# bark-simulator/planner-miqp

Measured on AMD Instinct MI355X. Metric: MIQP solves/sec to 1% gap, 2-agent x 20-step x 32-region, higher is better.
Workload: dtype f64

## Files before the change

### include/miqp_gpu.h

```cpp
#ifndef MIQP_GPU_H
#define MIQP_GPU_H

#include "miqp_types.h"

#ifdef __cplusplus
extern "C" {
#endif

typedef struct miqp_solver miqp_solver_t;

typedef struct miqp_solver_opts {
  int precision;
  int device;
  int nodes_per_round;
  int max_open_nodes;
  double gap_override;
  int verbose;
} miqp_solver_opts;

miqp_solver_t* miqp_solver_create(const miqp_solver_opts* opts);
void miqp_solver_destroy(miqp_solver_t* s);

int miqp_solver_set_params(miqp_solver_t* s, const miqp_model_params_c* p);

int miqp_solver_load_dat(miqp_solver_t* s, const char* path);

int miqp_solver_override_settings(miqp_solver_t* s, double max_solution_time, double relative_mip_gap_tolerance);

int miqp_solver_set_warmstart(miqp_solver_t* s, const miqp_raw_results_c* start, int warmstart_type);

int miqp_solver_solve(miqp_solver_t* s, double timestamp);

int miqp_solver_solve_batch(miqp_solver_t* const* solvers, int n, int* statuses);

int miqp_solver_solve_stream(miqp_solver_t* const* solvers, int n, int inflight, int* statuses);

int miqp_solver_solve_batch_multi(miqp_solver_t* const* solvers, int n, int gpus, int* statuses);

typedef int (*miqp_exchange_fn)(void* user, int op, void* buf, int count, int root);
int miqp_solver_solve_split(miqp_solver_t* s, double timestamp, int world, int rank, miqp_exchange_fn exchange, void* user);

int miqp_comm_unique_id(char* out128);
int miqp_comm_init(int world, int rank, const char* id128, int device);
int miqp_comm_finalize(void);
int miqp_solver_solve_split_rccl(miqp_solver_t* s, double timestamp);
int miqp_comm_selftest(miqp_exchange_fn exchange, void* user, int world, int rank);

int miqp_solver_split_roots(const miqp_solver_t* s, int world, int rank, int* root_of_pair, int* index, int* value, int cap, int* nroots_out, int* ncombos_out);

int miqp_solver_raw_sizes(const miqp_solver_t* s, int* out4);
int miqp_solver_lift_tables(const miqp_solver_t* s, double* out, int cap);

int miqp_solver_get_results(const miqp_solver_t* s, miqp_raw_results_c* out);

int miqp_solver_materialize_results(miqp_solver_t* const* solvers, int n, int threads);

int miqp_solver_get_properties(const miqp_solver_t* s, miqp_solution_properties_c* out);

int miqp_solver_get_dims(const miqp_solver_t* s, int* out6);

int miqp_solver_export_lp(const miqp_solver_t* s, const char* path);

int miqp_solver_write_dat(const miqp_solver_t* s, const char* path);

int miqp_solver_write_solution(const miqp_solver_t* s, const char* path);

int miqp_solver_write_mst(const miqp_solver_t* s, const char* path);

int miqp_solver_read_mst(miqp_solver_t* s, const char* path);

int miqp_solver_solve_fixed(miqp_solver_t* s, const miqp_raw_results_c* fixed, miqp_raw_results_c* out,
                            double* objective, int* iterations);

int miqp_solver_last_timing(const miqp_solver_t* s, double* out6);

int miqp_solver_last_active_set(const miqp_solver_t* s, double* out8);

int miqp_solver_last_fixed_route(const miqp_solver_t* s);

int miqp_solver_solve_fixed_batch(miqp_solver_t* s, const miqp_raw_results_c* const* fixed, int n, miqp_fixed_result_c* out, int* best);

int miqp_solver_fixed_batch_record(miqp_solver_t* s, int k, miqp_raw_results_c* out);

int miqp_gpu_fixed_result_size(void);
int miqp_gpu_fixed_batch_chunk(void);

int miqp_solver_set_pool(miqp_solver_t* s, int capacity);
int miqp_solver_pool_count(const miqp_solver_t* s);
int miqp_solver_pool_found(const miqp_solver_t* s, double* obj, int cap);
int miqp_solver_pool_solve(miqp_solver_t* s, miqp_fixed_result_c* out, int cap);
int miqp_solver_pool_record(miqp_solver_t* s, int k, miqp_raw_results_c* out);
int miqp_gpu_pool_max(void);

int miqp_solver_set_pool_filter(miqp_solver_t* s, int families);
int miqp_gpu_pool_signature(int cars, int steps, int obstacles, int families, const signed char* decisions, signed char* out, int len);
int miqp_solver_pool_signature(const miqp_solver_t* s, const miqp_raw_results_c* rec, int families, signed char* out, int cap);
int miqp_solver_pool_found_decisions(const miqp_solver_t* s, int k, signed char* out, int cap);

int miqp_solver_solve_fixed_multi(miqp_solver_t* const* solvers, int n, const miqp_raw_results_c* const* fixed, const int* first, miqp_fixed_result_c* out, int* best);
int miqp_solver_pool_solve_multi(miqp_solver_t* const* solvers, int n, miqp_fixed_result_c* out, int cap, int* counts);

int miqp_gpu_has_active_set(int num_cars, int num_steps);

int miqp_solver_launch_plan(const miqp_solver_t* s, int bc, int overlap, int par, const int* cls_n3, int cus, double free_gb, int flags, int* out, int cap);

int miqp_solver_last_setup(const miqp_solver_t* s, double* out3);

int miqp_solver_last_admission(const miqp_solver_t* s, double* out1);

const char* miqp_solver_last_error(const miqp_solver_t* s);


int miqp_fraction_parameters(int nr_regions, float max_velocity_fitting, double* out);
int miqp_fitting_polynomial_parameters(int nr_regions, float max_velocity_fitting, float min_velocity_fitting, double* out);
int miqp_mean_angles(const double* fraction_parameters, int nr_regions, double* out);
int miqp_limits_per_region(const double* fraction_parameters, int nr_regions, float long_min, float long_max, float lat_min, float lat_max,
                           double* min_x, double* max_x, double* min_y, double* max_y);
int miqp_calculate_region_idx(const double* fraction_parameters, int nr_regions, float vx, float vy, int* out);
int miqp_reserve_neighbor_regions(int* row, int nr_regions, int expansions);
int miqp_calculate_possible_regions(const double* fraction_parameters, int nr_regions, const double* theta_ref, int n, int* flags);
int miqp_reference_trajectory(const double* ref_xy, int n_ref, const double* state5, double dt, int num_points, double line_interp_inc, double vel_desired,
                              double delta_s_desired, double acc_lat_max, int vel_curve_dep, double* out);
int miqp_update_car(const double* settings12, const double* fraction_parameters, const double* initial_state6, const double* ref_xy, int n_ref, double desired_velocity,
                    double delta_s_desired, double timestep, int track_reference_positions, int is_ego, int num_cars, double* ref4N, int* possible_region, double* weights8);
int miqp_calculate_warmstart(const miqp_raw_results_c* last, miqp_raw_results_c* out, double ts, double minimum_region_change_speed);
int miqp_plan(miqp_solver_t* s, miqp_model_params_c* p, int* initial_region, int* possible_region, const miqp_raw_results_c* warmstart,
              int warmstart_type, double timestamp, int* status_out);

int miqp_initial_pose_check(const miqp_model_params_c* p);
int miqp_select_environment(const double* pieces_xy, const int* piece_off, int n_pieces, const double* traj_xy, const int* traj_off, int n_traj, int* selected);
int miqp_obstacle_intersects_environment(const double* pieces_xy, const int* piece_off, int n_pieces, const double* obstacle_xy, int n_steps, int is_static);
int miqp_bark_trajectory(const miqp_raw_results_c* results, int car, double start_time, double ts, double min_speed, double* out_rows5);
int miqp_obstacles_roi(double x, double y, double theta, double behind_distance, double front_distance, double side_distance, double* roi_xy);
int miqp_obstacle_intersects_environment_roi(const double* pieces_xy, const int* piece_off, int n_pieces, const double* obstacle_xy, int n_steps, int is_static, const double* roi_xy);
int miqp_environment_warmstart(const miqp_raw_results_c* last, miqp_raw_results_c* out, const int* ids_old, int n_old, const int* ids_new, int n_new);

int miqp_solver_certify(miqp_solver_t* s, const miqp_raw_results_c* candidate, miqp_certificate_c* out);
int miqp_solver_certify_batch(miqp_solver_t* const* solvers, int n, miqp_certificate_c* out);
int miqp_gpu_certificate_size(void);
int miqp_gpu_certify_last_timing(double* out4);

const char* miqp_gpu_version(void);

#ifdef __cplusplus
}
#endif
#endif
```

### planner_miqp_amd/csrc/as_onchip.hip

```cpp
namespace miqp {

#ifdef MIQP_PROFILE
#define ASP_T(var) const long long var = clock64()
#define ASP_ACC(k, t0, t1) asp_[k] += (unsigned long long)((t1) - (t0))
#else
#define ASP_T(var)
#define ASP_ACC(k, t0, t1)
#endif
constexpr int AS_MAXSTEP = 220;
constexpr double AS_VTOL = 1.0e-8;
constexpr double AS_DEP = 1.0e-8;
constexpr int AS_MT = 64;
constexpr int AS_MSTR = AS_MT * (AS_MT + 1) / 2;

__host__ __device__ constexpr bool as_shape_ok(int C, int N) { return (C == 1 || C == 2) && N >= 1 && N <= 2 * OC_NSL; }

template <int C> __device__ inline int as_col(int pq) { return C == 2 ? ((pq & 3) << 2) | (pq >> 2) : ((pq & 1) << 2) | (pq >> 1); }
template <int C> __device__ inline int as_pcol(int q) { return C == 2 ? ((q & 3) << 2) | (q >> 2) : ((q & 3) << 1) | (q >> 2); }
template <int C> struct AsDecode {
  static constexpr bool LANE_BOUNDS = true, ROW_IDENTITY = true, MARKS = true;
  static __device__ int col(int l) { return as_col<C>(oc_pcol<C, true>(l)); }
};

template <int C, int NSL, int GCAP = miqp::OC_GCAP>
__global__ void __launch_bounds__(64, (GCAP > 128 ? 1 : 2)) as_onchip_kernel(DevBuf B) {
  static_assert(C == 1 || C == 2, "a stage of 16 columns holds the chains of up to two cars");
  constexpr bool CM = true;
  constexpr bool BIG = GCAP > 128;
  constexpr int OC_GCAP = GCAP, OC_GSLOTS = OC_GCAP / 64, OC_GCOEF = oc_gcoef_of(OC_GCAP);
  constexpr int NX = 6 * C, NZ = 8 * C, NCH = 2 * C;
  const Layout& Y = B.Y;
  const int tid = threadIdx.x, lg = tid >> 4, lc = tid & 15;
  const int par = lg >> 1, side = lg & 1;
  const double bsgn = side ? -1.0 : 1.0;
  WAVE_DUMP(BIG ? 1 : 4);
  const int* const clist = BIG && B.cls_take ? B.cls_list + (size_t)(B.cls_take - 1) * B.batch_cap : nullptr;
  const int nbatch = clist ? (B.cls_count[B.cls_take - 1] < B.batch_cap ? B.cls_count[B.cls_take - 1] : B.batch_cap) : (*B.batch_count < B.batch_cap ? *B.batch_count : B.batch_cap);
  const int N = Y.N, NSLOT = Y.NSLOT;
  extern __shared__ double lds[];
  char* const L0 = (char*)lds;
  const OcLds LL = oc_lds_layout(N, Y.fixlen, OC_GCAP, !BIG);
  double* const Z = (double*)(L0 + LL.z);
  double* const scr = (double*)(L0 + LL.u);
  double* const V = (double*)(L0 + LL.u);
  unsigned long long* const bkey = (unsigned long long*)(L0 + LL.r);
  const int SPAN = LL.gmeta - LL.u;
  double* const kref = (double*)(L0 + LL.u + SPAN - N * 32);
  double* const kff = kref - N * 4;
  double* const KS = kff - N * 16;
  const int STG_CAP = (SPAN - N * 192) / 8;
  uint4* const gmeta = (uint4*)(L0 + LL.gmeta);
  double* const gcoef = (double*)(L0 + LL.gcoef);
  double* const grhs = (double*)(L0 + LL.grhs);
  double* const Wd = (double*)(L0 + LL.wd);
  int* const sstart = (int*)(L0 + LL.sstart);
  unsigned short* const cand = (unsigned short*)(L0 + LL.cand);
  signed char* const fix = (signed char*)(L0 + LL.fix);
  __shared__ int sh_node;
  __shared__ unsigned long long sh_stat[32];
  if (tid < 32) sh_stat[tid] = 0ull;
  const unsigned long long lt = (1ull << tid) - 1ull;

  const int chunk = B.as_chunk > 0 ? B.as_chunk : 1;
  int run_next = 0, run_end = 0;
  const int quota = BIG ? 0 : B.as_quota; int handed = 0;
#ifdef MIQP_PROFILE
  const unsigned long long wv_c0 = __builtin_amdgcn_s_memtime(), wv_r0 = __builtin_amdgcn_s_memrealtime();
  unsigned long long wv_first = 0; int wv_nodes = 0;
  if (!BIG && tid == 0) wv_first = atomicMin(&B.prof[120], wv_r0);
#endif
  for (;;) {
    __syncthreads();
    if (run_next >= run_end) {
      if (quota > 0 && handed >= quota) break;
      ++handed;
      if (tid == 0) sh_node = atomicAdd(B.work_counter, chunk);
      __syncthreads();
      run_next = __builtin_amdgcn_readfirstlane(sh_node); run_end = run_next + chunk;
      if (run_next >= nbatch) break;
    }
    const int slot_ = run_next++;
    if (slot_ >= nbatch) { run_next = run_end; continue; }
    const int node = clist ? __builtin_amdgcn_readfirstlane(clist[slot_]) : slot_;
    {
      const int cls = B.batch_large ? (int)B.batch_large[node] : (is_probe_word(B.batch_depth[node]) ? 1 : 0);
      if (cls != (BIG ? 1 : 0)) continue;
    }
    WAVE_DUMP_NODE();
    const int inst = __builtin_amdgcn_readfirstlane(B.batch_inst[node]);
    const double* D = B.inst_d + (size_t)inst * Y.dstride;
    const int* T = B.inst_i + (size_t)inst * Y.istride;
    const double ts = D[Y.d_glob + 7];
    const double aqs = 2.0 * D[Y.d_misc + 0];
    const double iaq = aqs > 0.0 ? 1.0 / aqs : 0.0;
    {
      const signed char* src = B.pool_fix + (size_t)B.batch_node[node] * Y.fixlen;
      for (int k = tid; k < Y.fixlen; k += 64) fix[k] = src[k];
      if (tid < 16) Wd[tid] = tid < NZ ? D[Y.d_wd + oc_lcol<C, CM>(as_pcol<C>(tid))] : 0.0;
      for (int k = tid; k < N * 32; k += 64) bkey[k] = ~0ull;
      for (int k = tid; k <= N + 1; k += 64) sstart[k] = 0;
    }
    __syncthreads();
    const double* Rf = D + Y.d_ref;
    double cutoff = 1e300;
    {
      const double inc0 = fmin(inc_from_key(*(volatile unsigned long long*)&B.inc_key[inst]), B.inc_ext[inst]);
      const double gap_ = is_probe_word(B.batch_depth[node]) ? 0.0 : B.inst_gap[inst];
      if (B.use_cutoff && inc0 < 1e300) cutoff = inc0 - gap_ * (1e-10 + fabs(inc0)) - B.inst_const[inst];
    }

#ifdef MIQP_PROFILE
    unsigned long long asp_[12] = {0, 0, 0, 0, 0, 0, 0, 0, 0, 0, 0, 0};
#endif
    ASP_T(ta0);
#define OC_DECODE_POLICY AsDecode<C>
#include "oc_decode_body.inc"
#undef OC_DECODE_POLICY
    if (overflow) {
      if (B.batch_A) B.batch_A[(size_t)node * 64 + tid] = 0xFFFFu;
      if (tid == 0) {
        if (B.ring_M) B.batch_Mtag[node] = 0ull;
        B.batch_ok[node] = 5; B.pool_big[B.batch_node[node]] |= (BIG ? 2 : 1); if (B.stats) { atomicAdd(&B.stats[3], 1ull); atomicAdd(&B.stats[8 + (ngen >= 512 ? 15 : ngen / 32)], 1ull); }
      }
      continue;
    }
    const int NM = sstart[N + 1];
    OC_WAVE_SYNC();

    ASP_T(ta1); ASP_ACC(0, ta0, ta1);
#ifdef MIQP_PROFILE
    asp_[9] += (unsigned long long)(ocd_t_sparse - ta0); asp_[11] += (unsigned long long)(ta1 - ocd_t_rows);
#endif
    double brhs[NSL];
    unsigned int bact = 0u, binA = 0u, ginA = 0u;
#pragma unroll
    for (int k = 0; k < NSL; ++k) {
      const int i = 2 * k + par;
      brhs[k] = 1e300;
      if (i < N && lc < NZ) {
        const unsigned long long key = bkey[(i * 2 + side) * 16 + lc];
        if (key != ~0ull) { brhs[k] = key2d(key); bact |= 1u << k; }
      }
    }
    OC_WAVE_SYNC();

    const double h1 = ts, h2 = 0.5 * ts * ts, h3 = ts * ts * ts / 6.0;
    const double* const tb = D + Y.d_astab;
    if constexpr (C == 2) {
      for (int k = tid; k < N * 16; k += 64) KS[k] = tb[k];
      for (int k = tid; k < N * 4; k += 64) kref[k] = tb[N * 16 + k];
    } else {
      for (int k = tid; k < N * 8; k += 64) KS[(k >> 3) * 16 + (k & 7)] = tb[k];
      for (int k = tid; k < N * 2; k += 64) kref[(k >> 1) * 4 + (k & 1)] = tb[N * 8 + k];
    }
    OC_WAVE_SYNC();
    typedef double d2_t __attribute__((ext_vector_type(2)));
    auto subst = [&](const bool fromx0, const int itop, const int iend, double* const out) {
      for (int k = tid; k < (N - 1) * 4; k += 64) if ((k >> 2) > itop) kff[k] = fromx0 ? kref[k] : 0.0;
      if (tid < NCH) {
        const int ch = tid;
        double p0 = 0.0, p1 = 0.0, p2 = 0.0;
        int i0 = itop;
        if (itop >= N - 1) { const d2_t a = *(const d2_t*)(V + (N - 1) * 16 + 4 * ch); p0 = a[0]; p1 = a[1]; p2 = V[(N - 1) * 16 + 4 * ch + 2]; i0 = N - 2; }
        if (i0 >= 0) {
          d2_t va = *(const d2_t*)(V + i0 * 16 + 4 * ch), vb = *(const d2_t*)(V + i0 * 16 + 4 * ch + 2);
          d2_t ka = *(const d2_t*)(KS + (i0 * 4 + ch) * 4), kb = *(const d2_t*)(KS + (i0 * 4 + ch) * 4 + 2);
          double kr = fromx0 ? kref[i0 * 4 + ch] : 0.0;
          for (int i = i0; i >= 0; --i) {
            const int j = i > 0 ? i - 1 : 0;
            const d2_t nva = *(const d2_t*)(V + j * 16 + 4 * ch), nvb = *(const d2_t*)(V + j * 16 + 4 * ch + 2);
            const d2_t nka = *(const d2_t*)(KS + (j * 4 + ch) * 4), nkb = *(const d2_t*)(KS + (j * 4 + ch) * 4 + 2);
            const double nkr = fromx0 ? kref[j * 4 + ch] : 0.0;
            const double su = vb[1] + h3 * p0 + h2 * p1 + h1 * p2;
            const double sx0 = va[0] + p0, sx1 = va[1] + h1 * p0 + p1, sx2 = vb[0] + h2 * p0 + h1 * p1 + p2;
            kff[i * 4 + ch] = fma(su, kb[1], kr);
            p0 = sx0 - ka[0] * su; p1 = sx1 - ka[1] * su; p2 = sx2 - kb[0] * su;
            va = nva; vb = nvb; ka = nka; kb = nkb; kr = nkr;
          }
        }
      }
      OC_WAVE_SYNC();
      if (tid < NCH) {
        const int ch = tid;
        double x0 = 0.0, x1 = 0.0, x2 = 0.0;
        if (fromx0) { const int c = ch >> 1, s = ch & 1; x0 = D[Y.d_x0 + 6 * c + 3 * s]; x1 = D[Y.d_x0 + 6 * c + 3 * s + 1]; x2 = D[Y.d_x0 + 6 * c + 3 * s + 2]; }
        const int ie = iend < N - 1 ? iend : N - 2;
        d2_t ka = *(const d2_t*)(KS + ch * 4), kb = *(const d2_t*)(KS + ch * 4 + 2);
        double kf = kff[ch];
        for (int i = 0; i <= ie; ++i) {
          const int j = i < N - 2 ? i + 1 : N - 2;
          const d2_t nka = *(const d2_t*)(KS + (j * 4 + ch) * 4), nkb = *(const d2_t*)(KS + (j * 4 + ch) * 4 + 2);
          const double nkf = kff[j * 4 + ch];
          const double u = -kf - (ka[0] * x0 + ka[1] * x1 + kb[0] * x2);
          d2_t oa, ob; oa[0] = x0; oa[1] = x1; ob[0] = x2; ob[1] = u;
          *(d2_t*)(out + i * 16 + 4 * ch) = oa; *(d2_t*)(out + i * 16 + 4 * ch + 2) = ob;
          const double n0 = x0 + h1 * x1 + h2 * x2 + h3 * u, n1 = x1 + h1 * x2 + h2 * u, n2 = x2 + h1 * u;
          x0 = n0; x1 = n1; x2 = n2;
          ka = nka; kb = nkb; kf = nkf;
        }
        if (iend >= N - 1 || ie == N - 2) { d2_t oa, ob; oa[0] = x0; oa[1] = x1; ob[0] = x2; ob[1] = 0.0; *(d2_t*)(out + (ie + 1) * 16 + 4 * ch) = oa; *(d2_t*)(out + (ie + 1) * 16 + 4 * ch + 2) = ob; }
      }
      OC_WAVE_SYNC();
    };
    auto row_dot = [&](int id, const double* vec) -> double {
      if (id < 1024) return (((id >> 4) & 1) ? -1.0 : 1.0) * vec[(id >> 5) * 16 + (id & 15)];
      const uint4 m4 = gmeta[id - 1024];
      const int off = (int)(m4.z & 0xFFFFu), nn = (int)((m4.z >> 16) & 7u), i = (int)((m4.z >> 20) & 0x7FFu);
      double a = 0.0;
#pragma unroll
      for (int k = 0; k < 6; ++k) if (k < nn) a += gcoef[off + k] * vec[i * 16 + ((m4.w >> (4 * k)) & 15u)];
      return a;
    };
    auto row_soft = [&](int id) -> bool { return id >= 1024 && (gmeta[id - 1024].z & 0x80000000u) != 0u; };
    auto zeroV = [&]() { for (int k = tid; k < N * 16; k += 64) V[k] = 0.0; OC_WAVE_SYNC(); };
    auto objective = [&]() -> double {
      double o = 0.0;
      for (int k = tid; k < N * 16; k += 64) { const int q = k & 15; if (q < NZ) { const double d = Z[k] - Rf[(k >> 4) * NZ + oc_lcol<C, CM>(as_pcol<C>(q))]; o += Wd[q] * d * d; } }
      return wave_sum(o);
    };

    int arow = -1, astage = -1; double alam = 0.0, arhs = 0.0;
    double M[64];
#pragma unroll
    for (int b = 0; b < 64; ++b) M[b] = 0.0;
    unsigned long long used = 0ull;
    auto rank1 = [&](const double u, const double alpha, const unsigned long long mask) {
#pragma unroll
      for (int g8 = 0; g8 < 8; ++g8) {
        if ((mask >> (8 * g8)) & 0xFFull) {
#pragma unroll
          for (int j = 0; j < 8; ++j) { const int b = 8 * g8 + j; M[b] = fma(u * readlane_d(u, b), alpha, M[b]); }
        }
      }
    };
    auto refresh = [&]() {
      zeroV();
      const double FX = 274877906944.0, IFX = 1.0 / 274877906944.0;
      if (arow >= 0 && alam != 0.0) {
        if (arow < 1024) atomicAdd((unsigned long long*)&V[(arow >> 5) * 16 + (arow & 15)], (unsigned long long)(long long)__double2ll_rn((((arow >> 4) & 1) ? -alam : alam) * FX));
        else {
          const uint4 m4 = gmeta[arow - 1024];
          const int off = (int)(m4.z & 0xFFFFu), nn = (int)((m4.z >> 16) & 7u), i = (int)((m4.z >> 20) & 0x7FFu);
#pragma unroll
          for (int k = 0; k < 6; ++k) if (k < nn) atomicAdd((unsigned long long*)&V[i * 16 + ((m4.w >> (4 * k)) & 15u)], (unsigned long long)(long long)__double2ll_rn(gcoef[off + k] * alam * FX));
        }
      }
      OC_WAVE_SYNC();
      for (int k = tid; k < N * 16; k += 64) V[k] = (double)(long long)__double_as_longlong(V[k]) * IFX;
      const int amax = (int)wave_max((double)astage);
      OC_WAVE_SYNC();
      subst(true, amax, N - 1, Z);
    };
    if constexpr (C == 2) { for (int k = tid; k < N * 16; k += 64) Z[k] = tb[N * 20 + k]; }
    else { for (int k = tid; k < N * 16; k += 64) Z[k] = (k & 15) < NZ ? tb[N * 10 + (k >> 4) * NZ + (k & 15)] : 0.0; }
    OC_WAVE_SYNC();
    ASP_T(ta2); ASP_ACC(1, ta1, ta2);
    int steps = 0, ndrop = 0, ok = 1, nwarm = 0, nfast = 0, ncold = 0;
    bool infeas = false, fail = false;
    int why = 0;
    if (B.pool_A && (B.batch_depth[node] >> 6) >= 1 && B.batch_node[node] < B.z_cap) {
      const int rec = B.batch_node[node];
      const unsigned int pa = B.pool_A[(size_t)rec * 64 + tid];
      int cid = -1;
      int ownl = 0;
      if (pa < 1024u) ownl = (int)((((pa >> 5) & 1u) * 2u + ((pa >> 4) & 1u)) << 4 | (pa & 15u));
      const unsigned int ob = (unsigned int)__shfl((int)bact, ownl);
      if (pa < 1024u) { if ((ob >> (pa >> 6)) & 1u) cid = (int)pa; }
      else if (pa != 0xFFFFu) {
        const int pc = (int)pa - 1024;
        int lo = 0, hi = NM;
        while (lo < hi) { const int mid = (lo + hi) >> 1; if ((int)cand[mid] < pc) lo = mid + 1; else hi = mid; }
        if (lo < NM && (int)cand[lo] == pc) cid = 1024 + lo;
      }
      const unsigned long long u0p = __ballot(pa != 0xFFFFu);
      const unsigned long long u0 = __ballot(cid >= 0);
      if (u0) {
        arow = cid;
        astage = cid < 0 ? -1 : (cid < 1024 ? (cid >> 5) : (int)((gmeta[cid - 1024].z >> 20) & 0x7FFu));
        int nmp = 0; unsigned long long moff = 0ull;
        if (B.ring_M) {
          const unsigned long long tg = B.pool_Mtag[rec];
          const unsigned long long c_ = tg >> 8;
          if (tg != 0ull && *(volatile unsigned long long*)B.ring_head - c_ < B.ring_doubles - B.ring_margin) { nmp = (int)(tg & 255ull); moff = c_ % B.ring_doubles; }
        }
        nmp = __builtin_amdgcn_readfirstlane(nmp);
        if (B.as_stats && tid == 0 && !(nmp > 0 && nmp == __popcll(u0p))) sh_stat[16 + (B.ring_M == nullptr ? 0 : (B.pool_Mtag[rec] == 0ull ? 1 : (nmp == 0 ? 2 : 3)))] += 1ull;
        if (nmp > 0 && nmp == __popcll(u0p)) {
          const double* const rm = B.ring_M; const unsigned long long rd_ = B.ring_doubles;
          const int ra = __popcll(u0p & lt);
          const bool mine = (u0p >> tid) & 1ull;
          const int len = nmp * (nmp + 1) / 2;
          for (int c0 = 0; c0 < len; c0 += STG_CAP) {
            const int c1 = c0 + STG_CAP < len ? c0 + STG_CAP : len;
            OC_WAVE_SYNC();
            for (int k = c0 + tid; k < c1; k += 64) { unsigned long long q_ = moff + (unsigned long long)k; if (q_ >= rd_) q_ -= rd_; V[k - c0] = rm[q_]; }
            OC_WAVE_SYNC();
#pragma unroll
            for (int b8 = 0; b8 < 64; ++b8) {
              if ((u0p >> b8) & 1ull) {
                const int rb = __popcll(u0p & ((1ull << b8) - 1ull));
                const int hi_ = ra > rb ? ra : rb, lo_ = ra > rb ? rb : ra;
                const int ix = hi_ * (hi_ + 1) / 2 + lo_;
                if (mine && ix >= c0 && ix < c1) M[b8] = V[ix - c0];
              }
            }
          }
          OC_WAVE_SYNC();
          used = u0p;
          for (unsigned long long um = u0p & ~u0; um; um &= um - 1ull) {
            const int kd = __builtin_amdgcn_readfirstlane(__ffsll((long long)um) - 1);
            double m = 0.0;
#pragma unroll
            for (int b = 0; b < 64; ++b) m = (b == kd) ? M[b] : m;
            const double mkk = readlane_d(m, kd);
            if (mkk > 0.0) rank1(m, -1.0 / mkk, used);
#pragma unroll
            for (int b = 0; b < 64; ++b) if (b == kd || tid == kd) M[b] = 0.0;
            used &= ~(1ull << kd);
          }
          nfast = 1;
        } else {
          used = u0;
          const int amax0 = (int)wave_max((double)astage);
          double sdiag = 1.0;
          for (unsigned long long um = u0; um; um &= um - 1ull) {
            const int a = __builtin_amdgcn_readfirstlane(__ffsll((long long)um) - 1);
            const int ida = __builtin_amdgcn_readlane(arow, a);
            zeroV();
            if (ida < 1024) { if (tid == 0) V[(ida >> 5) * 16 + (ida & 15)] = ((ida >> 4) & 1) ? -1.0 : 1.0; }
            else {
              const uint4 m4 = gmeta[ida - 1024];
              const int off = (int)(m4.z & 0xFFFFu), nn = (int)((m4.z >> 16) & 7u), i = (int)((m4.z >> 20) & 0x7FFu);
              if (tid < nn) V[i * 16 + ((m4.w >> (4 * tid)) & 15u)] = gcoef[off + tid];
            }
            const int sta = __builtin_amdgcn_readlane(astage, a);
            OC_WAVE_SYNC();
            subst(false, sta, amax0, V);
            double sv = arow >= 0 ? -row_dot(arow, V) : 0.0;
            if (tid == a && row_soft(ida)) sv += iaq;
            if (tid == a) sdiag = sv;
#pragma unroll
            for (int b = 0; b < 64; ++b) M[b] = (b == a) ? sv : M[b];
          }
          for (unsigned long long um = u0; um; um &= um - 1ull) {
            const int k = __builtin_amdgcn_readfirstlane(__ffsll((long long)um) - 1);
            double m = 0.0;
#pragma unroll
            for (int b = 0; b < 64; ++b) m = (b == k) ? M[b] : m;
            const double d = readlane_d(m, k);
            if (!(d > AS_DEP * readlane_d(sdiag, k))) {
#pragma unroll
              for (int b = 0; b < 64; ++b) if (b == k || tid == k) M[b] = 0.0;
              if (tid == k) { arow = -1; astage = -1; }
              used &= ~(1ull << k);
              continue;
            }
            const double invd = 1.0 / d;
#pragma unroll
            for (int g8 = 0; g8 < 8; ++g8) {
              if ((u0 >> (8 * g8)) & 0xFFull) {
#pragma unroll
                for (int j = 0; j < 8; ++j) { const int b = 8 * g8 + j; const double mb = readlane_d(m, b); M[b] = (tid == k) ? M[b] * invd : fma(m * mb, -invd, M[b]); }
              }
            }
#pragma unroll
            for (int b = 0; b < 64; ++b) M[b] = (b == k) ? ((tid == k) ? -invd : m * invd) : M[b];
          }
#pragma unroll
          for (int b = 0; b < 64; ++b) M[b] = (arow < 0) ? 0.0 : -M[b];
        }
        {
          int ol = 0, ok_ = -1;
          if (arow >= 0 && arow < 1024) { ol = (((arow >> 5) & 1) * 2 + ((arow >> 4) & 1)) << 4 | (arow & 15); ok_ = arow >> 6; }
          double rsel = arow >= 1024 ? grhs[arow - 1024] : 0.0;
#pragma unroll
          for (int k = 0; k < NSL; ++k) {
            const double rk = __shfl(brhs[k], ol);
            if (ok_ == k) rsel = rk;
          }
          arhs = rsel;
        }
        double cv = arow >= 0 ? row_dot(arow, Z) - arhs : 0.0;
        for (int guard = 0; guard < 64; ++guard) {
          double l0 = 0.0;
#pragma unroll
          for (int g8 = 0; g8 < 8; ++g8) {
            if ((used >> (8 * g8)) & 0xFFull) {
#pragma unroll
              for (int j = 0; j < 8; ++j) { const int b = 8 * g8 + j; l0 = fma(M[b], readlane_d(cv, b), l0); }
            }
          }
          if (arow < 0) l0 = 0.0;
          alam = l0;
          const double lmin = wave_min(arow >= 0 ? l0 : 1e300);
          if (!(lmin < -1e-10)) break;
          const int kd = __builtin_amdgcn_readfirstlane(__ffsll((long long)__ballot(arow >= 0 && l0 == lmin)) - 1);
          double m = 0.0;
#pragma unroll
          for (int b = 0; b < 64; ++b) m = (b == kd) ? M[b] : m;
          const double mkk = readlane_d(m, kd);
          if (!(mkk > 0.0)) { fail = true; break; }
          rank1(m, -1.0 / mkk, used);
#pragma unroll
          for (int b = 0; b < 64; ++b) if (b == kd || tid == kd) M[b] = 0.0;
          if (tid == kd) { arow = -1; astage = -1; alam = 0.0; cv = 0.0; }
          used &= ~(1ull << kd);
          ndrop++;
        }
        if (alam < 0.0) alam = 0.0;
        nwarm = __popcll(used);
        refresh();
        double resid = arow >= 0 ? fabs(row_dot(arow, Z) - arhs - ((arow >= 1024 && row_soft(arow)) ? alam * iaq : 0.0)) : 0.0;
        resid = wave_max(resid);
        if (!(resid <= 1e-7) || fail) {
          fail = false;
          arow = -1; astage = -1; alam = 0.0; arhs = 0.0; used = 0ull; nwarm = 0; nfast = 0; ncold = 1;
#pragma unroll
          for (int b = 0; b < 64; ++b) M[b] = 0.0;
          refresh();
        } else {
          unsigned int* const inab = C == 2 ? (unsigned int*)fix : (unsigned int*)V;
          inab[tid] = 0u;
          OC_WAVE_SYNC();
          if (arow >= 0) {
            if (arow < 1024) atomicOr(&inab[(((arow >> 5) & 1) * 2 + ((arow >> 4) & 1)) << 4 | (arow & 15)], 1u << (arow >> 6));
            else { const int rr_ = arow - 1024; atomicOr(&inab[rr_ & 63], 1u << (16 + (rr_ >> 6))); }
          }
          OC_WAVE_SYNC();
          { const unsigned int w_ = inab[tid]; binA = w_ & 0xFFFFu; ginA = w_ >> 16; }
        }
      }
    }
    ASP_T(ta3); ASP_ACC(8, ta2, ta3);
    double Dval = objective() + wave_sum((arow >= 1024 && row_soft(arow)) ? 0.5 * alam * alam * iaq : 0.0);

    for (; !fail;) {
      ASP_T(tb0);
      double bv = -1e300, brh = 0.0; int bid = -1;
#pragma unroll
      for (int k = 0; k < NSL; ++k) {
        const int i = 2 * k + par;
        if (((bact >> k) & 1u) && !((binA >> k) & 1u)) { const double v = bsgn * Z[i * 16 + lc] - brhs[k]; if (v > bv) { bv = v; brh = brhs[k]; bid = (i * 2 + side) * 16 + lc; } }
      }
#pragma unroll
      for (int q = 0; q < OC_GSLOTS; ++q) {
        const int r = q * 64 + tid;
        if (r < NM && !((ginA >> q) & 1u)) { const double rh_ = grhs[r]; const double v = row_dot(1024 + r, Z) - rh_; if (v > bv) { bv = v; brh = rh_; bid = 1024 + r; } }
      }
      const double vmax = wave_max(bv);
      if (!(vmax > AS_VTOL)) break;
      if (steps >= AS_MAXSTEP || used == ~0ull || !(vmax < 1e290)) { fail = true; why = used == ~0ull ? 1 : 2; break; }
      const int src = __builtin_amdgcn_readfirstlane(__ffsll((long long)__ballot(bv == vmax)) - 1);
      const int pid = __builtin_amdgcn_readlane(bid, src);
      const bool psoft = row_soft(pid);
      const double prhs = readlane_d(brh, src);
      ASP_T(tb1); ASP_ACC(2, tb0, tb1);
      zeroV();
      if (pid < 1024) { if (tid == 0) V[(pid >> 5) * 16 + (pid & 15)] = ((pid >> 4) & 1) ? -1.0 : 1.0; }
      else {
        const uint4 m4 = gmeta[pid - 1024];
        const int off = (int)(m4.z & 0xFFFFu), nn = (int)((m4.z >> 16) & 7u), i = (int)((m4.z >> 20) & 0x7FFu);
        if (tid < nn) V[i * 16 + ((m4.w >> (4 * tid)) & 15u)] = gcoef[off + tid];
      }
      const int pstage = pid < 1024 ? (pid >> 5) : (int)((gmeta[pid - 1024].z >> 20) & 0x7FFu);
      const int amax_ = (int)wave_max((double)astage);
      OC_WAVE_SYNC();
      subst(false, pstage, amax_ > pstage ? amax_ : pstage, V);
      ASP_T(tb2); ASP_ACC(3, tb1, tb2);
      double q = arow >= 0 ? -row_dot(arow, V) : 0.0;
      const double Spp = -row_dot(pid, V) + (psoft ? iaq : 0.0);
      double vp = vmax, lp = 0.0;
      steps++;
      ASP_T(tb3); ASP_ACC(4, tb2, tb3);
      for (;;) {
        double r = 0.0;
#pragma unroll
        for (int g8 = 0; g8 < 8; ++g8) {
          if ((used >> (8 * g8)) & 0xFFull) {
#pragma unroll
            for (int j = 0; j < 8; ++j) { const int b = 8 * g8 + j; r = fma(M[b], readlane_d(q, b), r); }
          }
        }
        if (arow < 0) r = 0.0;
        const double curv = Spp - wave_sum(q * r);
        const double ratio = (arow >= 0 && r > 1e-13) ? alam / r : 1e300;
        const double td = wave_min(ratio);
        const int kd = td < 1e299 ? __builtin_amdgcn_readfirstlane(__ffsll((long long)__ballot(ratio == td)) - 1) : -1;
        if (!(curv == curv) || !(Spp > 0.0)) { fail = true; why = 3; break; }
        const bool dep = !(curv > AS_DEP * Spp);
        double t; bool full;
        if (dep) { if (kd < 0) { infeas = true; break; } t = td; full = false; }
        else { const double tp = vp / curv; if (tp <= td) { t = tp; full = true; } else { t = td; full = false; } }
        if (arow >= 0) { alam = fma(-t, r, alam); if (alam < 0.0) alam = 0.0; }
        lp += t;
        Dval += t * (vp - 0.5 * t * (dep ? 0.0 : curv));
        if (lp > RHO_EL) { infeas = true; break; }
        if (full) {
          const int s = __builtin_amdgcn_readfirstlane(__ffsll((long long)~used) - 1);
          double u = arow >= 0 ? r : 0.0;
          if (tid == s) u = -1.0;
          const unsigned long long nmask = used | (1ull << s);
          rank1(u, 1.0 / curv, nmask);
          if (tid == s) { arow = pid; alam = lp; astage = pstage; arhs = prhs; }
          used = nmask;
          if (pid < 1024) { if (tid == ((((pid >> 5) & 1) * 2 + ((pid >> 4) & 1)) << 4 | (pid & 15))) binA |= 1u << (pid >> 6); }
          else { const int rr_ = pid - 1024; if (tid == (rr_ & 63)) ginA |= 1u << (rr_ >> 6); }
          break;
        }
        vp -= t * (dep ? 0.0 : curv);
        const int idk = __builtin_amdgcn_readlane(arow, kd);
        if (idk < 1024) { if (tid == ((((idk >> 5) & 1) * 2 + ((idk >> 4) & 1)) << 4 | (idk & 15))) binA &= ~(1u << (idk >> 6)); }
        else { const int rr_ = idk - 1024; if (tid == (rr_ & 63)) ginA &= ~(1u << (rr_ >> 6)); }
        double m = 0.0;
#pragma unroll
        for (int b = 0; b < 64; ++b) m = (b == kd) ? M[b] : m;
        const double mkk = readlane_d(m, kd);
        if (!(mkk > 0.0)) { fail = true; why = 4; break; }
        rank1(m, -1.0 / mkk, used);
#pragma unroll
        for (int b = 0; b < 64; ++b) if (b == kd || tid == kd) M[b] = 0.0;
        if (tid == kd) { arow = -1; astage = -1; alam = 0.0; q = 0.0; }
        used &= ~(1ull << kd);
        ndrop++; steps++;
        if (steps >= AS_MAXSTEP) { fail = true; why = 2; break; }
      }
      ASP_T(tb4); ASP_ACC(5, tb3, tb4);
      if (infeas || fail) break;
      refresh();
      ASP_T(tb5); ASP_ACC(6, tb4, tb5);
      if (Dval - 1e-9 * fabs(Dval) > cutoff + 1e-9 * fabs(cutoff)) { ok = 2; break; }
    }
    ASP_T(tc0);
    double viol = 0.0, scost = 0.0, lres = 0.0;
    if (!fail && !infeas && ok == 1) {
#pragma unroll
      for (int k = 0; k < NSL; ++k) { const int i = 2 * k + par; if ((bact >> k) & 1u) viol = fmax(viol, bsgn * Z[i * 16 + lc] - brhs[k]); }
#pragma unroll
      for (int q = 0; q < OC_GSLOTS; ++q) { const int r = q * 64 + tid; if (r < NM && !(gmeta[r].z & 0x80000000u)) viol = fmax(viol, row_dot(1024 + r, Z) - grhs[r]); }
      if (arow >= 0) {
        const bool sf = arow >= 1024 && row_soft(arow);
        const double res = row_dot(arow, Z) - arhs - (sf ? alam * iaq : 0.0);
        if (sf) { scost = 0.5 * alam * alam * iaq; viol = fmax(viol, res); }
        lres = alam * res;
      }
      viol = wave_max(viol); scost = wave_sum(scost);
      lres = fabs(wave_sum(lres));
    } else if (infeas) viol = 1.0;
    if (!fail && !infeas && ok == 1 && !(viol <= 5.0e-7)) { fail = true; why = 5; }
    if (BIG && infeas && B.as_probe_first && B.pump_max > 0 && is_probe_word(B.batch_depth[node]) && (cutoff > 1e299 || B.pump_inc)) fail = true;
    if (fail) {
      if (B.batch_A) B.batch_A[(size_t)node * 64 + tid] = 0xFFFFu;
      if (B.ring_M && tid == 0) B.batch_Mtag[node] = 0ull;
      if (tid == 0) { B.batch_ok[node] = 5; B.pool_big[B.batch_node[node]] |= 4; if (B.as_stats) { sh_stat[2] += 1ull; sh_stat[10 + (why < 6 ? why : 5)] += 1ull; } }
      continue;
    }
    const double obj = (infeas || ok == 2) ? Dval : objective() + scost;
    double* Zo = B.batch_Z + (size_t)node * N * NZ;
    for (int k = tid; k < N * 16; k += 64) { const int q = k & 15; if (q < NZ) Zo[(k >> 4) * NZ + oc_lcol<C, CM>(as_pcol<C>(q))] = Z[k]; }
    if (B.batch_A) {
      unsigned short enc = 0xFFFFu;
      if (!fail && !infeas && ok == 1 && arow >= 0) enc = arow < 1024 ? (unsigned short)arow : (unsigned short)(1024 + (int)cand[arow - 1024]);
      B.batch_A[(size_t)node * 64 + tid] = enc;
    }
    if (B.ring_M) {
      const int n_ = __popcll(used);
      unsigned long long tg_ = 0ull;
      OC_WAVE_SYNC();
      if (!fail && !infeas && ok == 1 && n_ >= 1 && n_ <= AS_MT && n_ * (n_ + 1) * 4 <= LL.total) {
        double* const stg = (double*)L0;
        const int ra = __popcll(used & lt);
#pragma unroll
        for (int b8 = 0; b8 < 64; ++b8) {
          if ((used >> b8) & 1ull) {
            const int rb = __popcll(used & ((1ull << b8) - 1ull));
            if (arow >= 0 && ra >= rb) stg[ra * (ra + 1) / 2 + rb] = M[b8];
          }
        }
        const int len = n_ * (n_ + 1) / 2;
        unsigned long long cnt_ = 0ull;
        if (tid == 0) cnt_ = atomicAdd(B.ring_head, (unsigned long long)len);
        cnt_ = ((unsigned long long)(unsigned int)__builtin_amdgcn_readfirstlane((int)(cnt_ >> 32)) << 32) | (unsigned int)__builtin_amdgcn_readfirstlane((int)cnt_);
        tg_ = (cnt_ << 8) | (unsigned long long)n_;
        OC_WAVE_SYNC();
        const unsigned long long o_ = cnt_ % B.ring_doubles, rd_ = B.ring_doubles;
        for (int k = tid; k < len; k += 64) { unsigned long long q_ = o_ + (unsigned long long)k; if (q_ >= rd_) q_ -= rd_; B.ring_M[q_] = stg[k]; }
      }
      if (tid == 0) B.batch_Mtag[node] = tg_;
    }
    if (tid == 0) {
      B.batch_obj[node] = obj; B.batch_viol[node] = viol; B.batch_ok[node] = ok;
      B.batch_bound[node] = lres + 1e-9 * (1.0 + fabs(obj));
      B.batch_it[node] = steps;
      atomicAdd((unsigned long long*)&B.inst_nodes[inst], 1ull);
      atomicAdd((unsigned long long*)&B.inst_iters[inst], (unsigned long long)steps);
#ifdef MIQP_PROFILE
      ++wv_nodes;
      { const long long tc1 = clock64(); asp_[7] += (unsigned long long)(tc1 - tc0);
        for (int q_ = 0; q_ < 9; ++q_) atomicAdd(&B.prof[80 + q_], asp_[q_]);
        atomicAdd(&B.prof[92], asp_[9]); atomicAdd(&B.prof[93], asp_[11]);
        atomicAdd(&B.prof[90], 1ull); atomicAdd(&B.prof[91], (unsigned long long)steps); }
#endif
      if (B.as_stats) {
        sh_stat[0] += 1ull; sh_stat[1] += (unsigned long long)steps; sh_stat[3] += (unsigned long long)ndrop;
        sh_stat[4] += infeas ? 1ull : 0ull; sh_stat[5] += ok == 2 ? 1ull : 0ull; sh_stat[6] += (unsigned long long)__popcll(used); sh_stat[7] += (unsigned long long)nwarm; sh_stat[8] += (unsigned long long)nfast; sh_stat[9] += (unsigned long long)ncold;
        if (BIG) { const int og_ = B.pool_origin ? (int)B.pool_origin[B.batch_node[node]] : 0; sh_stat[20] += 1ull; sh_stat[21] += (unsigned long long)steps; if (og_ == 14) { sh_stat[22] += 1ull; sh_stat[23] += (unsigned long long)steps; }
          sh_stat[24 + (ngen <= 64 ? 0 : ngen <= 96 ? 1 : ngen <= 128 ? 2 : ngen <= 192 ? 3 : 4)] += 1ull; if (is_probe_word(B.batch_depth[node]) && og_ != 14) sh_stat[29] += 1ull; }
      }
    }
  }
  __syncthreads();
  if (B.as_stats && tid < 32 && sh_stat[tid] != 0ull) atomicAdd(&B.as_stats[tid], sh_stat[tid]);
#ifdef MIQP_PROFILE
  if (!BIG && tid == 0) {
    const unsigned long long wv_c1 = __builtin_amdgcn_s_memtime(), wv_r1 = __builtin_amdgcn_s_memrealtime();
    atomicAdd(&B.prof[94], wv_c1 - wv_c0); atomicAdd(&B.prof[95], wv_r1 - wv_r0); atomicAdd(&B.prof[96], 1ull);
    atomicMin(&B.prof[122], wv_r1); atomicMax(&B.prof[121], wv_r1);
    const unsigned long long dl = wv_r0 > wv_first ? wv_r0 - wv_first : 0ull;
    const int hb = dl < 5000 ? 0 : dl < 20000 ? 1 : dl < 50000 ? 2 : dl < 100000 ? 3 : dl < 200000 ? 4 : dl < 400000 ? 5 : dl < 800000 ? 6 : 7;
    atomicAdd(&B.prof[128 + hb], 1ull);
    const int nb = wv_nodes == 0 ? 0 : wv_nodes <= 4 ? 1 : wv_nodes <= 16 ? 2 : wv_nodes <= 32 ? 3 : wv_nodes <= 64 ? 4 : 5;
    atomicAdd(&B.prof[136 + nb], 1ull);
    if (B.prof[125] == 300 && blockIdx.x < 4096) {
      unsigned int hw, xcc;
      asm volatile("s_getreg_b32 %0, hwreg(HW_REG_HW_ID)" : "=s"(hw));
      asm volatile("s_getreg_b32 %0, hwreg(HW_REG_XCC_ID)" : "=s"(xcc));
      unsigned long long* const w = B.prof + 160 + 4 * blockIdx.x;
      w[0] = wv_r0; w[1] = wv_r1; w[2] = ((unsigned long long)xcc << 32) | hw; w[3] = (unsigned long long)wv_nodes;
    }
  }
#endif
}

}
```

### planner_miqp_amd/csrc/miqp_gpu.hip

```cpp
#include <hip/hip_runtime.h>
#include <dlfcn.h>

#include <algorithm>
#include <chrono>
#include <cmath>
#include <cstdio>
#include <cstdlib>
#include <cstring>
#include <map>
#include <memory>
#include <atomic>
#include <mutex>
#include <string>
#include <thread>
#include <vector>

#include "../../include/miqp_gpu.h"
#include "kernels.hip"
#include "wire_formats.hpp"
#include "planner_core.hpp"
#include "lp_export.hpp"

__attribute__((constructor)) static void miqp_gpu_hw_queues() { setenv("GPU_MAX_HW_QUEUES", "8", 0); }

// ... 1122 lines not shown
    unsigned long long kinc = ~0ull; double lbl = 1e300;
    HIP_OK(hipMemcpy(&kinc, B.inc_key, 8, hipMemcpyDeviceToHost)); HIP_OK(hipMemcpy(&lbl, B.lower_bound, 8, hipMemcpyDeviceToHost));
    local_done = bc <= 0;
    unsigned long long w[4];
    w[0] = kinc >= 0xFFF0000000000000ull ? ~0ull : ((kinc & ~0xFFFFFull) | (unsigned long long)split->rank);
    w[1] = host_d2key(local_done && kinc >= 0xFFF0000000000000ull ? 1e300 : (local_done ? std::min(lbl, 1e300) : lbl));
    w[2] = local_done ? ~0ull : 0ull;
    w[3] = (wall_s() - t0 > tlim) ? 0ull : ~0ull;
    if (split->fn(split->user, 0, w, 4, 0) != 0) { std::fprintf(stderr, "[miqp_gpu] incumbent exchange failed\n"); return false; }
    sp.inc = w[0] >= 0xFFF0000000000000ull ? 1e300 : host_key2d(w[0] & ~0xFFFFFull); sp.owner = (int)(w[0] & 0xFFFFFull);
    sp.lb = host_key2d(w[1]); sp.timeup = w[3] == 0ull;
    HIP_OK(hipMemcpyAsync(B.inc_ext, &sp.inc, 8, hipMemcpyHostToDevice, st));
    const bool all_done = w[2] == ~0ull;
    const bool gap_ok = sp.inc < 1e299 && (sp.inc - sp.lb) <= H.h_gap[0] * (1e-10 + std::fabs(sp.inc));
    stop = all_done || sp.timeup || gap_ok;
    if (stop) sp.finished = all_done || gap_ok;
    return true;
  }

  void adapt_width() {
    if (kinc_now != width_key) { width_key = kinc_now; width_since = rounds; }
    else if (kinc_now < 0xFFF0000000000000ull && rounds - width_since >= 32 && demand_now >= 8 * width_now && width_now < sh.width_max) {
      const double io_ = host_key2d(kinc_now & ~0xFFFFFull);
      if (lb_now > -1e299 && io_ - lb_now <= 0.05 * std::fabs(io_)) { width_now *= 2; width_since = rounds; }
    }
  }

  bool run() {
    const ProcessSwitches& ps = process_switches(); const CallSwitches& sw = X.sw; const Layout& Y = X.Y;
    t0 = wall_s();
    for (int k = 0; k < n; ++k) tlim = std::max(tlim, H.h_tlim[k]);
    HIP_OK(hipEventRecord(X.ev0, st));
    if (!admit(0.0, 0)) return false;
    use_par = X.ctr && X.oc_grid > 0 && X.ocb_grid > 0 && X.concurrent_big && X.stream2 && X.probe_grid > 0 && !sw.memsets;
    if (use_par) HIP_OK(hipMemsetAsync(X.ctr, 0, 2 * CTR_SET * 4, st));
    use_cls = use_par && X.as_on && X.cls_list && sw.cls_lists;
    B.cls_list = use_cls ? X.cls_list : nullptr; B.cls_take = 0; X.cls_n[0] = X.cls_n[1] = X.cls_n[2] = -1;
    width_now = sh.adaptive_width ? sh.width0 : 0;
    const bool share_aside = B.lns_mode > 0 && NS >= 64 && X.stream2 && X.ev_sfork && !sw.debug_sync;
    for (;;) {
      const int par = rounds & 1;
      B.width_cap = width_now;
      if (use_par) { B.batch_count = X.ctr + CTR_SET * par; B.cls_count = B.batch_count + 8; } else HIP_OK(hipMemsetAsync(B.batch_count, 0, 4, st));
      B.open_sel = rounds & 1;
      B.prev_bc = prev_bc;
      hipLaunchKernelGGL(select_kernel, dim3(NS), dim3(SEL_THREADS), 0, st, B, rounds);
      if (share_aside) { (void)hipEventRecord(X.ev_sfork, st); (void)hipStreamWaitEvent(X.stream2, X.ev_sfork, 0); hipLaunchKernelGGL(share_kernel, dim3(1), dim3(1024), 0, X.stream2, B); (void)hipEventRecord(X.ev_sjoin, X.stream2); }
      if (B.lns_mode > 0) hipLaunchKernelGGL(lns_kernel, dim3(NS), dim3(64), 0, st, B);
      if (sw.debug_sync) debug_sync(st, rounds, "select");
      hipLaunchKernelGGL(roll_kernel, dim3(1), dim3(CTR_SET), 0, st, B, use_par ? X.ctr + CTR_SET * (par ^ 1) : (int*)nullptr);
      if (share_aside) (void)hipStreamWaitEvent(st, X.ev_sjoin, 0); else hipLaunchKernelGGL(share_kernel, dim3(1), dim3(1024), 0, st, B);
      int bc = 0; int hctr[CTR_SET] = {0};
      HIP_OK(hipMemcpyAsync(use_cls ? hctr : &bc, B.batch_count, use_cls ? CTR_SET * 4 : 4, hipMemcpyDeviceToHost, st));
      HIP_OK(hipMemcpyAsync(done_now.data(), B.inst_done, (size_t)n * 4, hipMemcpyDeviceToHost, st));
      if (sh.adaptive_width) { HIP_OK(hipMemcpyAsync(&kinc_now, B.inc_key, 8, hipMemcpyDeviceToHost, st)); HIP_OK(hipMemcpyAsync(&demand_now, B.slot_demand, 4, hipMemcpyDeviceToHost, st)); HIP_OK(hipMemcpyAsync(&lb_now, B.lower_bound, 8, hipMemcpyDeviceToHost, st)); }
      HIP_OK(hipStreamSynchronize(st));
      if (use_cls) { bc = hctr[0]; for (int q = 0; q < 3; ++q) X.cls_n[q] = std::min(hctr[8 + q], X.batch_cap); }
      if (sh.adaptive_width) adapt_width();
      const double tnow = wall_s() - t0;
      for (int sl = 0; sl < NS; ++sl) { const int k = slot_inst[sl]; if (k >= 0 && done_now[k] && t_done[k] < 0) t_done[k] = tnow - t_admit[k]; }
      if (split) {
        bool stop = false, local_done = false;
        if (!exchange(bc, stop, local_done)) return false;
        if (stop) break;
        if (local_done) { rounds++; continue; }
      } else {
        if (!kill_timed_out(tnow)) return false;
        if (!admit(tnow, 1 - (rounds & 1))) return false;
        if (in_flight == 0 && next_q >= n) break;
        if (tnow > tlim * (double)((n + NS - 1) / NS + 1) + 30.0) { abandoned = true; break; }
        if (bc <= 0) {
          if (!empty_round()) return false;
          if (abandoned) break;
          rounds++; prev_bc = 0; continue;
        }
        stuck_once = false;
        empty_rounds = 0;
      }
      if (bc > X.batch_cap) bc = X.batch_cap;
      if (sw.trace && bc > 0 && bc <= 256 && !trace_selection(X, rounds, bc)) return false;
      if (X.ipm_ev.size() < nev + 2) { hipEvent_t a, b; HIP_OK(hipEventCreate(&a)); HIP_OK(hipEventCreate(&b)); X.ipm_ev.push_back(a); X.ipm_ev.push_back(b); }
      if (ps.launch_trace && !X.ev_mid) HIP_OK(hipEventCreate(&X.ev_mid));
      if (X.std_ev.size() < nev / 2 + 1) { hipEvent_t a_; HIP_OK(hipEventCreate(&a_)); X.std_ev.push_back(a_); }
      HIP_OK(hipEventRecord(X.ipm_ev[nev], st));
      launch_ipm_batch(X, B, bc, st, true, use_par ? par : -1, X.std_ev[nev / 2]);
      HIP_OK(hipEventRecord(X.ipm_ev[nev + 1], st));
      if (ps.launch_trace && !trace_launches(X, rounds, bc, nev)) return false;
      nev += 2;
      if (bc >= X.batch_cap / 2 && rounds >= ps.replay_round && !replay_batch(X, bc)) return false;
      if (sw.debug_sync) debug_sync(st, rounds, "ipm", bc);
      if (sw.trace && !trace_batch(X, rounds, bc)) return false;
      { DevBuf Be = B; Be.open_sel = 1 - (rounds & 1); launch_eval_c(Y.C, Be, bc, l_eval, st); }
      if (X.pool.on && !pool_capture(X, bc)) return false;
      if (sw.debug_sync) debug_sync(st, rounds, "eval");
      launched_nodes += bc; rounds++; prev_bc = bc;
      if (ps.round_log) round_bc.push_back(bc);
      if (verbose > 1) std::fprintf(stderr, "[miqp_gpu] round %d: %d nodes\n", rounds, bc);
      if (verbose == 1 && rounds % 25 == 0 && !print_progress(X, wall_s() - t0, rounds, launched_nodes, H.h_const[0])) return false;
    }
    return true;
  }
};

struct Polished { std::vector<double> obj, viol; std::vector<int> ok, it; };
bool polish(DevCtx& X, int n, Polished& P, float& ms_all) {
  const DevBuf& B = X.B; const Layout& Y = X.Y; hipStream_t st = X.stream;
  P.obj.assign(n, 0.0); P.viol.assign(n, 1.0); P.ok.assign(n, 0); P.it.assign(n, 0);
  HIP_OK(hipMemcpyAsync(B.pool_fix, B.inc_fix, (size_t)n * Y.fixlen, hipMemcpyDeviceToDevice, st));
  std::vector<int> ids(n); for (int k = 0; k < n; ++k) ids[k] = k;
  HIP_OK(hipMemcpyAsync(B.batch_node, ids.data(), n * 4, hipMemcpyHostToDevice, st));
  HIP_OK(hipMemcpyAsync(B.batch_inst, ids.data(), n * 4, hipMemcpyHostToDevice, st));
  HIP_OK(hipMemcpyAsync(B.batch_count, &n, 4, hipMemcpyHostToDevice, st));
  HIP_OK(hipStreamSynchronize(st));
  DevBuf Bp = B; Bp.qp_tol = QP_TOL_FINAL; Bp.use_cutoff = 0; Bp.batch_cap = X.batch_alloc;
  Bp.ws_on = (B.ws_on && !X.sw.polish_cold) ? 2 : 0; Bp.ws_mu = X.sw.polish_mu; Bp.ws_delta = X.sw.polish_delta;
  int nb = std::min(n, X.batch_alloc);
  launch_ipm_batch(X, Bp, nb, st);
  HIP_OK(hipMemcpyAsync(P.obj.data(), B.batch_obj, nb * 8, hipMemcpyDeviceToHost, st));
  HIP_OK(hipMemcpyAsync(P.viol.data(), B.batch_viol, nb * 8, hipMemcpyDeviceToHost, st));
  HIP_OK(hipMemcpyAsync(P.ok.data(), B.batch_ok, nb * 4, hipMemcpyDeviceToHost, st));
  HIP_OK(hipMemcpyAsync(P.it.data(), B.batch_it, nb * 4, hipMemcpyDeviceToHost, st));
  HIP_OK(hipEventRecord(X.ev1, st));
  HIP_OK(hipStreamSynchronize(st));
  HIP_OK(hipGetLastError());
  HIP_OK(hipEventElapsedTime(&ms_all, X.ev0, X.ev1));
  return true;
}

struct Results {
  std::vector<double> inc, lb, Z; std::vector<int> flags, ninc, oc, dn; std::vector<long long> nodes, iters;
  std::vector<signed char> fix; unsigned long long rowiters = 0, as[32] = {0};
};
bool read_back(const DevCtx& X, int n, Results& R) {
  const DevBuf& B = X.B; const Layout& Y = X.Y;
  R.inc.resize(n); R.lb.resize(n); R.flags.resize(n); R.ninc.resize(n); R.oc.resize(n); R.dn.resize(n); R.nodes.resize(n); R.iters.resize(n);
  HIP_OK(hipMemcpy(R.inc.data(), B.inc_obj, n * 8, hipMemcpyDeviceToHost));
  HIP_OK(hipMemcpy(R.lb.data(), B.lower_bound, n * 8, hipMemcpyDeviceToHost));
  HIP_OK(hipMemcpy(R.flags.data(), B.inst_flags, n * 4, hipMemcpyDeviceToHost));
  HIP_OK(hipMemcpy(R.ninc.data(), B.inst_ninc, n * 4, hipMemcpyDeviceToHost));
  HIP_OK(hipMemcpy(R.oc.data(), B.open_count, n * 4, hipMemcpyDeviceToHost));
  HIP_OK(hipMemcpy(R.dn.data(), B.inst_done, n * 4, hipMemcpyDeviceToHost));
  HIP_OK(hipMemcpy(R.nodes.data(), B.inst_nodes, n * 8, hipMemcpyDeviceToHost));
  HIP_OK(hipMemcpy(R.iters.data(), B.inst_iters, n * 8, hipMemcpyDeviceToHost));
  HIP_OK(hipMemcpy(&R.rowiters, B.stat_rowiters, 8, hipMemcpyDeviceToHost));
  HIP_OK(hipMemcpy(R.as, B.as_stats, 256, hipMemcpyDeviceToHost));
  if (B.stats && R.as[0] + R.as[2] > 0) print_as_stats(R.as);
  R.fix.resize((size_t)n * Y.fixlen); R.Z.resize((size_t)n * Y.N * Y.nz);
  HIP_OK(hipMemcpy(R.fix.data(), B.inc_fix, R.fix.size(), hipMemcpyDeviceToHost));
  HIP_OK(hipMemcpy(R.Z.data(), B.inc_Z, R.Z.size() * 8, hipMemcpyDeviceToHost));
  return true;
}
bool take_polished(const DevCtx& X, miqp_solver_t* const* S, int n, const HostTables& H, const Polished& P, Results& R) {
  const DevBuf& B = X.B; const Layout& Y = X.Y;
  std::vector<double> h_pZ((size_t)n * Y.N * Y.nz);
  HIP_OK(hipMemcpy(h_pZ.data(), B.batch_Z, h_pZ.size() * 8, hipMemcpyDeviceToHost));
  for (int k = 0; k < n; ++k) {
    if (!(R.inc[k] < 1e299)) continue;
    if (P.viol[k] <= FEAS_TOL && (P.ok[k] || P.it[k] >= 10)) {
      int nign = 0; for (int q = 0; q < Y.C * Y.O * Y.N * 5; ++q) nign += R.fix[(size_t)k * Y.fixlen + Y.f_obs + q] >= Y.L;
      R.inc[k] = P.obj[k] + H.h_const[k] + nign * S[k]->inst.w_slack_obs;
      std::copy(h_pZ.begin() + (size_t)k * Y.N * Y.nz, h_pZ.begin() + (size_t)(k + 1) * Y.N * Y.nz, R.Z.begin() + (size_t)k * Y.N * Y.nz);
    }
  }
  return true;
}

bool split_broadcast(const SplitCtx* split, const SplitState& sp, Results& R) {
  std::vector<unsigned char> buf(8 + R.Z.size() * 8 + R.fix.size());
  unsigned long long w[2] = {R.inc[0] < 1e299 ? ((host_d2key(R.inc[0]) & ~0xFFFFFull) | (unsigned long long)split->rank) : ~0ull, ~0ull};
  if (split->fn(split->user, 0, w, 2, 0) != 0) { std::fprintf(stderr, "[miqp_gpu] incumbent exchange failed\n"); return false; }
  if (w[0] < 0xFFF0000000000000ull) {
    const int owner = (int)(w[0] & 0xFFFFFull);
    if (owner == split->rank) { std::memcpy(buf.data(), &R.inc[0], 8); std::memcpy(buf.data() + 8, R.Z.data(), R.Z.size() * 8); std::memcpy(buf.data() + 8 + R.Z.size() * 8, R.fix.data(), R.fix.size()); }
    if (split->fn(split->user, 1, buf.data(), (int)buf.size(), owner) != 0) { std::fprintf(stderr, "[miqp_gpu] solution broadcast failed\n"); return false; }
    std::memcpy(&R.inc[0], buf.data(), 8); std::memcpy(R.Z.data(), buf.data() + 8, R.Z.size() * 8); std::memcpy(R.fix.data(), buf.data() + 8 + R.Z.size() * 8, R.fix.size());
    R.lb[0] = std::min(sp.lb, R.inc[0]);
  }
  R.flags[0] = sp.finished ? 0 : 1; R.oc[0] = 0; R.dn[0] = 1;
  return true;
}

struct CallTimes { double t_setup = 0, t_ctx = 0, t_tables = 0, t_solve = 0, ms_ipm = 0, ms_std = 0; float ms_all = 0; bool ctx_built = false, std_timed = false; };

void report(miqp_solver_t* const* S, int* statuses, const Layout& Y, const HostTables& H, const Rounds& L, const Results& R, const CallTimes& T, bool split) {
  const int n = L.n;
  long long tot_iters = 0; for (int k = 0; k < n; ++k) tot_iters += R.iters[k];
  for (int k = 0; k < n; ++k) {
    miqp_solver* s = S[k];
    bool have = R.inc[k] < 1e299;
    bool unfinished = (R.flags[k] & 3) || R.oc[k] > 0 || !R.dn[k];
    if (!split && k >= L.next_q && !H.h_done[k]) {
      s->status = MIQP_STATUS_FAILED_SEG_FAULT; s->has_sol = false; s->props.objective = NAN; s->props.gap = NAN; s->props.best_bound = NAN; s->props.status = 0; s->props.time = 0.0;
      s->err = "the queue was abandoned before this instance was admitted";
      statuses[k] = s->status; continue;
    }
    s->props.time = L.t_done[k] >= 0 ? L.t_done[k] : std::max(0.0, T.t_solve - L.t_admit[k]);
    s->admit_s = L.t_admit[k];
    s->props.NrIterations = (int)std::min<long long>(R.iters[k], 2147483647LL); s->props.nodes = R.nodes[k];
    s->props.NrSolutionPool = R.ninc[k];
    s->timing[0] = T.ms_all * 1e-3; s->timing[1] = T.ms_ipm * 1e-3; s->timing[2] = (double)(L.nev / 2); s->timing[3] = (double)L.launched_nodes;
    s->timing[4] = (double)tot_iters; s->timing[5] = (double)R.rowiters;
    s->as_timing[0] = (double)R.as[0]; s->as_timing[1] = (double)R.as[1]; s->as_timing[2] = (double)R.as[2]; s->as_timing[3] = (double)R.as[3];
    s->as_timing[4] = (double)R.as[6]; s->as_timing[5] = (double)R.as[7]; s->as_timing[6] = T.ms_std * 1e-3; s->as_timing[7] = T.std_timed ? (double)(L.nev / 2) : 0.0;
    s->setup[0] = T.t_setup; s->setup[1] = T.t_ctx; s->setup[2] = T.ctx_built ? 1.0 : 0.0;
    s->err.clear();
    if (L.stalled[k] && unfinished) s->err = "retired without a proof: no progress for 64 branch-and-bound rounds (not a time-limit verdict)";
    if (have) {
      s->status = MIQP_STATUS_SUCCESS; s->has_sol = true;
      s->props.objective = R.inc[k];
      double lb = std::min(R.lb[k], R.inc[k]);
      const double lb_tol = R.inc[k] - H.h_gap[k] * std::fabs(R.inc[k]);
      lb = std::min(lb, lb_tol);
      s->props.best_bound = lb; s->props.gap = std::fabs(lb - R.inc[k]) / (1e-10 + std::fabs(R.inc[k]));
      if (lb == lb_tol && s->props.gap > H.h_gap[k]) s->props.gap = H.h_gap[k];
      s->props.status = unfinished ? MIQP_CPX_STAT_TIME_LIM_FEAS : (s->props.gap <= 1e-9 ? MIQP_CPX_STAT_OPTIMAL : MIQP_CPX_STAT_OPTIMAL_TOL);
      s->Z.assign(R.Z.begin() + (size_t)k * Y.N * Y.nz, R.Z.begin() + (size_t)(k + 1) * Y.N * Y.nz);
      s->comp.assign(R.fix.begin() + (size_t)k * Y.fixlen, R.fix.begin() + (size_t)(k + 1) * Y.fixlen);
    } else {
      s->status = unfinished ? (L.stalled[k] ? MIQP_STATUS_FAILED_SEG_FAULT : MIQP_STATUS_FAILED_TIMEOUT) : MIQP_STATUS_FAILED_NO_SOLUT;
      s->props.objective = NAN; s->props.gap = NAN; s->props.best_bound = R.lb[k];
      s->props.status = unfinished ? MIQP_CPX_STAT_TIME_LIM_INFEAS : MIQP_CPX_STAT_INFEASIBLE;
    }
    statuses[k] = s->status;
  }
  if (L.abandoned) std::fprintf(stderr, "[miqp_gpu] the round loop was abandoned with %d of %d instances never admitted: they report FAILED_SEG_FAULT, the call fails\n", n - L.next_q, n);
}

bool pool_prepare(DevCtx& X, miqp_solver_t* const* S, int n);
bool pool_read_back(const DevCtx& X, miqp_solver_t* const* S, int n, const Results& R);

bool solve_batch_impl(miqp_solver_t* const* S, int n, int* statuses, const SplitCtx* split = nullptr, int inflight = 0, int lane = 0, int lanes = 1) {
  for (int k = 0; k < n; ++k) { statuses[k] = MIQP_STATUS_FAILED_SEG_FAULT; if (S[k]) { S[k]->status = MIQP_STATUS_FAILED_SEG_FAULT; S[k]->has_sol = false; S[k]->rescache.reset(); S[k]->drop_pool(); } }
  if (split && n != 1) return false;
  BatchShape bs = batch_layout(S, n);
  if (!bs.ok) { for (int k = 0; k < n; ++k) { if (S[k]) S[k]->err = bs.err; statuses[k] = MIQP_STATUS_FAILED_SEG_FAULT; } std::fprintf(stderr, "[miqp_gpu] %s\n", bs.err.c_str()); return false; }
  const Layout& Y = bs.Y;
  const miqp_solver_opts& O0 = S[0]->opts;
  auto fail_all = [&](const char* why) { if (why) std::fprintf(stderr, "[miqp_gpu] %s\n", why); for (int k = 0; k < n; ++k) statuses[k] = MIQP_STATUS_FAILED_SEG_FAULT; return false; };
  for (int k = 1; k < n; ++k) if (S[k]->opts.device != O0.device) return fail_all("instances of one batch must name the same device (use miqp_solver_solve_batch_multi to span devices)");
  const double t_enter = wall_s();
  DevCtx* Xp = ctx_for_device(O0.device, lane);
  if (!Xp) return fail_all(nullptr);
  warn_ignored_switches();
  DevCtx& X = *Xp;
  std::lock_guard<std::mutex> ctx_lock(X.mu);
  if (hipSetDevice(X.device) != hipSuccess) return fail_all("hipSetDevice failed");
  const CallSwitches sw = read_call_switches();
  const CallShape sh = plan_call(Y, O0, n, inflight, lanes, split != nullptr, sw);
  const size_t l_ipm = ipm_lds_bytes(Y), l_eval = eval_lds_bytes(Y, sw.seq_kinds);
  CallTimes T;
  {
    bool setup_ok = ctx_prepare(X, Y, n, sh.NS, sh.open_cap, sh.npr, sh.MAXR, sh.clamp_open, lanes, &T.ctx_built);
    if (setup_ok && (l_ipm > 160 * 1024 || l_eval > 160 * 1024)) { std::fprintf(stderr, "[miqp_gpu] instance too large for LDS (%zu bytes)\n", l_ipm); setup_ok = false; }
    if (setup_ok && !set_kernel_lds(Y, l_ipm, l_eval)) setup_ok = false;
    if (setup_ok && !pool_prepare(X, S, n)) setup_ok = false;
    if (split) {
      unsigned long long w = setup_ok ? 1ull : 0ull;
      if (split->fn(split->user, 0, &w, 1, 0) != 0) return fail_all("set-up exchange failed");
      if (setup_ok && w == 0ull) return fail_all("another rank of the tree split failed its set-up");
    }
    if (!setup_ok) return fail_all(nullptr);
  }
  T.t_ctx = wall_s() - t_enter;
  HostTables H;
  prepare_instances(S, Y, sh, split, H);
  T.t_tables = wall_s() - t_enter - T.t_ctx;
  apply_call_switches(X, sh, sw, H.h_gap);
  if (!upload_and_reset(X, H, sh)) return fail_all(nullptr);

  Rounds L(X, sh, H, split, O0.verbose, l_eval);
  if (!L.run()) return fail_all(nullptr);
  T.t_setup = L.t0 - t_enter;
  if (sw.dump_open && !dump_open_list(X, sw.dump_open, L.rounds, sh.NS, H.h_const[0])) return fail_all(nullptr);

  Polished P;
  if (!polish(X, n, P, T.ms_all)) return fail_all(nullptr);
#ifdef MIQP_PROFILE
  if (!print_profile(X)) return fail_all(nullptr);
#endif
  if (X.B.stats && !print_stats(X)) return fail_all(nullptr);
  if (process_switches().round_log) { std::fprintf(stderr, "[rounds]"); for (int v : L.round_bc) std::fprintf(stderr, " %d", v); std::fprintf(stderr, "\n"); }
  for (size_t e = 0; e + 1 < L.nev; e += 2) { float ms = 0; HIP_OK(hipEventElapsedTime(&ms, X.ipm_ev[e], X.ipm_ev[e + 1])); T.ms_ipm += ms; }
  T.std_timed = L.use_par;
  if (T.std_timed) for (size_t e = 0; e + 1 < L.nev; e += 2) { float ms = 0; if (hipEventElapsedTime(&ms, X.ipm_ev[e], X.std_ev[e / 2]) == hipSuccess) T.ms_std += ms; }
  T.t_solve = wall_s() - L.t0;

  Results R;
  if (!read_back(X, n, R) || !take_polished(X, S, n, H, P, R)) return fail_all(nullptr);
  if (X.pool.on && !pool_read_back(X, S, n, R)) return fail_all(nullptr);
  if (split && !split_broadcast(split, L.sp, R)) return fail_all(nullptr);
  report(S, statuses, Y, H, L, R, T, split != nullptr);
  for (int k = 0; k < n; ++k) if (!S[k]->has_sol) S[k]->drop_pool();
  if (sw.stats) std::fprintf(stderr, "[miqp_gpu stats] reachable-set diameter (L1) of instance 0: %.1f\n", H.D[Y.d_misc + 2]);
  if (sw.stats) std::fprintf(stderr, "[miqp_gpu stats] host: setup %.3f s (device context %.3f, instance tables and presolve %.3f, upload %.3f), rounds %.3f s (%d), results %.3f s\n", T.t_setup, T.t_ctx, T.t_tables, T.t_setup - T.t_ctx - T.t_tables, T.t_solve, L.rounds, wall_s() - L.t0 - T.t_solve);
  return !L.abandoned;
}

}

#include "certify.hip"
#include "fixed_batch.hip"
#include "solution_pool.hip"
#include "fixed_multi.hip"

extern "C" {

const char* miqp_gpu_version(void) { return "miqp_gpu 0.1 (gfx950)"; }

miqp_solver_t* miqp_solver_create(const miqp_solver_opts* opts) {
  miqp_solver* s = new miqp_solver();
  if (opts) s->opts = *opts; else { s->opts.precision = 12; s->opts.device = -1; s->opts.gap_override = -1; }
  if (s->opts.precision <= 0) s->opts.precision = 12;
  return s;
}

void miqp_solver_destroy(miqp_solver_t* s) { delete s; }

int miqp_solver_set_params(miqp_solver_t* s, const miqp_model_params_c* p) {
  if (!s || !p) return -1;
  s->has_inst = inst_from_params(p, s->opts.precision - 2, s->inst, s->err);
  s->rescache.reset(); s->drop_fixed_batch(); s->drop_pool();
  s->has_sol = false;
  if (!s->has_inst) std::fprintf(stderr, "[miqp_gpu] %s\n", s->err.c_str());
  return s->has_inst ? 0 : -2;
}

int miqp_solver_load_dat(miqp_solver_t* s, const char* path) {
  if (!s || !path) return -1;
  s->has_inst = inst_from_dat(path, s->inst, s->err);
  s->has_sol = false; s->rescache.reset(); s->drop_fixed_batch(); s->drop_pool();
  if (!s->has_inst) std::fprintf(stderr, "[miqp_gpu] %s\n", s->err.c_str());
  return s->has_inst ? 0 : -2;
}

int miqp_solver_override_settings(miqp_solver_t* s, double max_solution_time, double relative_mip_gap_tolerance) {
  if (!s || !s->has_inst) return -1;
  s->inst.tilim = max_solution_time; s->inst.gap = relative_mip_gap_tolerance;
  return 0;
}

int miqp_solver_get_dims(const miqp_solver_t* s, int* o) {
  if (!s || !s->has_inst) return -1;
  o[0] = s->inst.C; o[1] = s->inst.N; o[2] = s->inst.R; o[3] = s->inst.E; o[4] = s->inst.O; o[5] = s->inst.L;
  return 0;
}

int miqp_solver_set_warmstart(miqp_solver_t* s, const miqp_raw_results_c* start, int warmstart_type) {
  if (!s) return -1;
  if (warmstart_type == MIQP_WARMSTART_NONE || !start) { s->ws[0].reset(); s->ws[1].reset(); return 0; }
  const int slot = warmstart_type == MIQP_WARMSTART_LAST_SOLUTION ? 1 : 0;
  if (start->N < 2 || start->NrCars < 1 || start->NrRegions < 1 || start->NrEnvironments < 0 || start->NrObstacles < 0 || start->MaxLinesObstacles < 0 ||
      start->NrCarToCarCollisions != start->NrCars - 1) return -2;
  if (s->has_inst && !dims_match(*start, s->inst)) { s->ws[slot].reset(); return -3; }
  s->ws[slot].reset(new OwnedResults(start->NrCars, start->N, start->NrRegions, start->NrEnvironments, start->NrObstacles, start->MaxLinesObstacles));
  s->ws[slot]->copy_from(*start);
  return 0;
}

int miqp_solver_solve_batch(miqp_solver_t* const* solvers, int n, int* statuses) {
  if (!solvers || n < 1 || !statuses) return -1;
  return solve_batch_impl(solvers, n, statuses) ? 0 : -2;
}

int miqp_solver_solve_stream(miqp_solver_t* const* solvers, int n, int inflight, int* statuses) {
  if (!solvers || n < 1 || !statuses) return -1;
  int lanes = knob_int(KNOB_P("MIQP_LANES"), 1);
  if (lanes > 8) lanes = 8;
  while (lanes > 1 && (inflight <= 0 || inflight >= n || inflight / lanes < 128)) lanes--;
  if (lanes <= 1) return solve_batch_impl(solvers, n, statuses, nullptr, inflight) ? 0 : -2;
  for (int b = 0; b < n; ++b) { if (!solvers[b]) return -1; if (solvers[b]->opts.device != solvers[0]->opts.device) lanes = 1; }
  if (lanes <= 1) return solve_batch_impl(solvers, n, statuses, nullptr, inflight) ? 0 : -2;
  std::vector<std::vector<miqp_solver_t*>> sub(lanes); std::vector<std::vector<int>> st(lanes);
  for (int b = 0; b < n; ++b) sub[b % lanes].push_back(solvers[b]);
  std::vector<char> ok(lanes, 0);
  std::vector<std::thread> th;
  for (int l = 0; l < lanes; ++l) {
    st[l].assign(sub[l].size(), MIQP_STATUS_FAILED_SEG_FAULT);
    const int infl = (inflight + lanes - 1 - l) / lanes;
    th.emplace_back([&, l, infl] { ok[l] = solve_batch_impl(sub[l].data(), (int)sub[l].size(), st[l].data(), nullptr, infl, l, lanes) ? 1 : 0; });
  }
  for (auto& t : th) t.join();
  int rc = 0;
  for (int b = 0; b < n; ++b) statuses[b] = st[b % lanes][b / lanes];
  for (int l = 0; l < lanes; ++l) if (!ok[l]) rc = -2;
  return rc;
}

int miqp_solver_solve_batch_multi(miqp_solver_t* const* solvers, int n, int gpus, int* statuses) {
  if (!solvers || n < 1 || !statuses) return -1;
  int ndev = 0;
  if (hipGetDeviceCount(&ndev) != hipSuccess || ndev < 1) { std::fprintf(stderr, "[miqp_gpu] no HIP device: the solver has no CPU path\n"); for (int k = 0; k < n; ++k) statuses[k] = MIQP_STATUS_FAILED_SEG_FAULT; return -2; }
  if (gpus <= 0 || gpus > ndev) gpus = ndev;
  if (gpus > n) gpus = n;
  std::vector<std::vector<miqp_solver_t*>> shard(gpus); std::vector<std::vector<int>> st(gpus);
  for (int b = 0; b < n; ++b) { if (!solvers[b]) return -1; solvers[b]->opts.device = b % gpus; shard[b % gpus].push_back(solvers[b]); }
  std::vector<char> ok(gpus, 0);
  std::vector<std::thread> th;
  for (int g = 0; g < gpus; ++g) {
    st[g].assign(shard[g].size(), MIQP_STATUS_FAILED_SEG_FAULT);
    th.emplace_back([&, g] { ok[g] = solve_batch_impl(shard[g].data(), (int)shard[g].size(), st[g].data()) ? 1 : 0; });
  }
  for (auto& t : th) t.join();
  int rc = 0;
  for (int b = 0; b < n; ++b) statuses[b] = st[b % gpus][b / gpus];
  for (int g = 0; g < gpus; ++g) if (!ok[g]) rc = -2;
  return rc;
}

int miqp_solver_solve_split(miqp_solver_t* s, double timestamp, int world, int rank, miqp_exchange_fn exchange, void* user) {
  (void)timestamp;
  if (!s || !s->has_inst || world < 1 || rank < 0 || rank >= world || !exchange) return MIQP_STATUS_FAILED_SEG_FAULT;
  SplitCtx sc{world, rank, exchange, user};
  miqp_solver_t* one[1] = {s}; int st = MIQP_STATUS_FAILED_SEG_FAULT;
  if (!solve_batch_impl(one, 1, &st, &sc)) return MIQP_STATUS_FAILED_SEG_FAULT;
  return st;
}

int miqp_solver_split_roots(const miqp_solver_t* s, int world, int rank, int* root_of_pair, int* index, int* value, int cap, int* nroots_out, int* ncombos_out) {
  if (!s || !s->has_inst || world < 1 || rank < 0 || rank >= world) return -1;
  miqp_solver_t* one[1] = {const_cast<miqp_solver_t*>(s)};
  BatchShape bs = batch_layout(one, 1);
  if (!bs.ok) return -2;
  std::vector<double> D(bs.Y.dstride); std::vector<int> T(bs.Y.istride);
  compile_instance(s->inst, bs.Y, D.data(), T.data());
  std::vector<std::vector<std::pair<int, int>>> combos; split_roots(bs.Y, T.data(), combos, world);
  int np = 0, nr = 0;
  for (size_t q = 0; q < combos.size(); ++q) {
    if ((int)(q % (size_t)world) != rank) continue;
    for (auto& d : combos[q]) { if (np < cap) { if (root_of_pair) root_of_pair[np] = nr; if (index) index[np] = d.first; if (value) value[np] = d.second; } np++; }
    nr++;
  }
  if (nroots_out) *nroots_out = nr;
  if (ncombos_out) *ncombos_out = (int)combos.size();
  return np;
}

struct Id128 { char b[128]; };
namespace {
struct Rccl {
  void* lib = nullptr; void* comm = nullptr; int world = 0, rank = 0, device = -1; void* dbuf = nullptr; size_t dcap = 0; hipStream_t stream = nullptr;
  int (*GetUniqueId)(void*) = nullptr;
  int (*CommInitRank)(void**, int, Id128, int) = nullptr;
  int (*CommDestroy)(void*) = nullptr;
  int (*AllReduce)(const void*, void*, size_t, int, int, void*, hipStream_t) = nullptr;
  int (*Broadcast)(const void*, void*, size_t, int, int, void*, hipStream_t) = nullptr;
};
Rccl g_rccl; std::mutex g_rccl_mu;
bool rccl_load() {
  if (g_rccl.lib) return true;
  for (const char* nm : {"librccl.so.1", "librccl.so", "/opt/rocm/lib/librccl.so.1"}) { g_rccl.lib = dlopen(nm, RTLD_NOW | RTLD_LOCAL); if (g_rccl.lib) break; }
  if (!g_rccl.lib) { std::fprintf(stderr, "[miqp_gpu] librccl not found: %s\n", dlerror()); return false; }
  g_rccl.GetUniqueId = (int (*)(void*))dlsym(g_rccl.lib, "ncclGetUniqueId");
  g_rccl.CommInitRank = (int (*)(void**, int, Id128, int))dlsym(g_rccl.lib, "ncclCommInitRank");
  g_rccl.CommDestroy = (int (*)(void*))dlsym(g_rccl.lib, "ncclCommDestroy");
  g_rccl.AllReduce = (int (*)(const void*, void*, size_t, int, int, void*, hipStream_t))dlsym(g_rccl.lib, "ncclAllReduce");
  g_rccl.Broadcast = (int (*)(const void*, void*, size_t, int, int, void*, hipStream_t))dlsym(g_rccl.lib, "ncclBroadcast");
  return g_rccl.GetUniqueId && g_rccl.CommInitRank && g_rccl.CommDestroy && g_rccl.AllReduce && g_rccl.Broadcast;
}
int rccl_exchange(void*, int op, void* buf, int count, int root) {
  Rccl& R = g_rccl;
  if (!R.comm) return -1;
  const size_t bytes = op == 0 ? (size_t)count * 8 : (size_t)count;
  if (hipSetDevice(R.device) != hipSuccess) return -2;
  if (bytes > R.dcap) { if (R.dbuf) (void)hipFree(R.dbuf); R.dcap = std::max<size_t>(bytes, 1 << 16); if (hipMalloc(&R.dbuf, R.dcap) != hipSuccess) { R.dbuf = nullptr; R.dcap = 0; return -2; } }
  if (hipMemcpyAsync(R.dbuf, buf, bytes, hipMemcpyHostToDevice, R.stream) != hipSuccess) return -2;
  const int rc = op == 0 ? R.AllReduce(R.dbuf, R.dbuf, (size_t)count,  5,  3, R.comm, R.stream)
                         : R.Broadcast(R.dbuf, R.dbuf, bytes,  1, root, R.comm, R.stream);
  if (rc != 0) return -3;
  if (hipMemcpyAsync(buf, R.dbuf, bytes, hipMemcpyDeviceToHost, R.stream) != hipSuccess) return -2;
  return hipStreamSynchronize(R.stream) == hipSuccess ? 0 : -2;
}
}

int miqp_comm_unique_id(char* out128) {
  std::lock_guard<std::mutex> lk(g_rccl_mu);
  if (!out128 || !rccl_load()) return -1;
  return g_rccl.GetUniqueId(out128) == 0 ? 0 : -2;
}
int miqp_comm_init(int world, int rank, const char* id128, int device) {
  std::lock_guard<std::mutex> lk(g_rccl_mu);
  if (!id128 || world < 1 || rank < 0 || rank >= world || !rccl_load()) return -1;
  if (g_rccl.comm) return -4;
  int ndev = 0; if (hipGetDeviceCount(&ndev) != hipSuccess || ndev < 1) { std::fprintf(stderr, "[miqp_gpu] no HIP device\n"); return -2; }
  if (device < 0) { if (hipGetDevice(&device) != hipSuccess) device = 0; }
  if (hipSetDevice(device) != hipSuccess) return -2;
  Id128 id; std::memcpy(id.b, id128, 128);
  if (g_rccl.CommInitRank(&g_rccl.comm, world, id, rank) != 0) { g_rccl.comm = nullptr; return -3; }
  if (hipStreamCreate(&g_rccl.stream) != hipSuccess) return -2;
  g_rccl.world = world; g_rccl.rank = rank; g_rccl.device = device;
  return 0;
}
int miqp_comm_finalize(void) {
  std::lock_guard<std::mutex> lk(g_rccl_mu);
  if (g_rccl.comm) { g_rccl.CommDestroy(g_rccl.comm); g_rccl.comm = nullptr; }
  if (g_rccl.dbuf) { (void)hipFree(g_rccl.dbuf); g_rccl.dbuf = nullptr; g_rccl.dcap = 0; }
  if (g_rccl.stream) { (void)hipStreamDestroy(g_rccl.stream); g_rccl.stream = nullptr; }
  return 0;
}
int miqp_comm_selftest(miqp_exchange_fn exchange, void* user, int world, int rank) {
  if (!exchange) { if (!g_rccl.comm) return -1; exchange = rccl_exchange; world = g_rccl.world; rank = g_rccl.rank; }
  unsigned long long w[3] = {1000ull - (unsigned long long)rank, 5ull + (unsigned long long)rank, 0x8000000000000000ull + (unsigned long long)(world - rank)};
  if (exchange(user, 0, w, 3, 0) != 0) return -2;
  if (w[0] != 1000ull - (unsigned long long)(world - 1) || w[1] != 5ull || w[2] != 0x8000000000000001ull) return -3;
  for (int root = 0; root < world; ++root) {
    unsigned char b[37]; for (int k = 0; k < 37; ++k) b[k] = (unsigned char)(rank == root ? (7 * k + root) & 255 : 0xEE);
    if (exchange(user, 1, b, 37, root) != 0) return -4;
    for (int k = 0; k < 37; ++k) if (b[k] != (unsigned char)((7 * k + root) & 255)) return -5;
  }
  return 0;
}
int miqp_solver_solve_split_rccl(miqp_solver_t* s, double timestamp) {
  if (!g_rccl.comm || !s) return MIQP_STATUS_FAILED_SEG_FAULT;
  s->opts.device = g_rccl.device;
  return miqp_solver_solve_split(s, timestamp, g_rccl.world, g_rccl.rank, rccl_exchange, nullptr);
}

int miqp_solver_raw_sizes(const miqp_solver_t* s, int* out4) {
  if (!s || !s->has_inst || !out4) return -1;
  raw_sizes(s->inst, out4[0], out4[1], out4[2], out4[3]);
  return 0;
}

int miqp_solver_lift_tables(const miqp_solver_t* s, double* out, int cap) {
  if (!s || !s->has_inst || !out) return -1;
  miqp_solver_t* one[1] = {const_cast<miqp_solver_t*>(s)};
  BatchShape bs = batch_layout(one, 1);
  if (!bs.ok) return -2;
  const int n = bs.Y.C * 2 * bs.Y.N * 16;
  if (cap < n) return -3;
  std::vector<double> D(bs.Y.dstride, 0.0);
  lift_tables(s->inst, bs.Y, D.data());
  std::copy(D.begin() + bs.Y.d_lift, D.begin() + bs.Y.d_lift + n, out);
  return n;
}

int miqp_solver_solve(miqp_solver_t* s, double timestamp) {
  (void)timestamp;
  if (!s || !s->has_inst) return MIQP_STATUS_FAILED_SEG_FAULT;
  miqp_solver_t* one[1] = {s}; int st = MIQP_STATUS_FAILED_SEG_FAULT;
  if (!solve_batch_impl(one, 1, &st)) return MIQP_STATUS_FAILED_SEG_FAULT;
  return st;
}

int miqp_solver_last_admission(const miqp_solver_t* s, double* out1) { if (!s || !out1) return -1; out1[0] = s->admit_s; return 0; }

const char* miqp_solver_last_error(const miqp_solver_t* s) { return s ? s->err.c_str() : "null handle"; }

int miqp_solver_get_results(const miqp_solver_t* s, miqp_raw_results_c* out) {
  if (!s || !out || !s->has_sol) return -1;
  if (!dims_match(*out, s->inst)) return -2;
  if (s->rescache) { out->N = s->rescache->r.N; out->NrEnvironments = s->rescache->r.NrEnvironments; out->NrRegions = s->rescache->r.NrRegions; out->NrObstacles = s->rescache->r.NrObstacles;
                     out->MaxLinesObstacles = s->rescache->r.MaxLinesObstacles; out->NrCarToCarCollisions = s->rescache->r.NrCarToCarCollisions; out->NrCars = s->rescache->r.NrCars;
                     s->rescache->copy_to(*out); return 0; }
  std::vector<double> D(s->lay.dstride); std::vector<int> T(s->lay.istride);
  compile_instance(s->inst, s->lay, D.data(), T.data());
  fill_results(s->inst, s->lay, D.data(), T.data(), s->comp.data(), s->Z.data(), out);
  return 0;
}

int miqp_solver_materialize_results(miqp_solver_t* const* solvers, int n, int threads) {
  if (!solvers || n < 0) return -1;
  int nth = threads > 0 ? threads : std::min((int)std::thread::hardware_concurrency(), 32);
  nth = std::max(1, std::min(nth, std::max(1, n / 4)));
  std::atomic<int> next{0}, made{0};
  auto work = [&] {
    std::vector<double> D; std::vector<int> T;
    for (int k = next.fetch_add(1); k < n; k = next.fetch_add(1)) {
      miqp_solver* s = solvers[k];
      if (!s || !s->has_sol || s->rescache) continue;
      std::unique_ptr<OwnedResults> R(new OwnedResults(s->inst));
      D.resize(s->lay.dstride); T.resize(s->lay.istride);
      compile_instance(s->inst, s->lay, D.data(), T.data());
      fill_results(s->inst, s->lay, D.data(), T.data(), s->comp.data(), s->Z.data(), &R->r);
      s->rescache = std::move(R); made.fetch_add(1);
    }
  };
  if (nth <= 1) work();
  else { std::vector<std::thread> th; for (int t = 0; t < nth; ++t) th.emplace_back(work); for (auto& t : th) t.join(); }
  return made.load();
}

int miqp_solver_get_properties(const miqp_solver_t* s, miqp_solution_properties_c* out) {
  if (!s || !out) return -1;
  *out = s->props;
  return 0;
}

int miqp_solver_last_timing(const miqp_solver_t* s, double* out6) {
  if (!s || !out6) return -1;
  for (int k = 0; k < 6; ++k) out6[k] = s->timing[k];
  return 0;
}

int miqp_solver_last_active_set(const miqp_solver_t* s, double* out8) {
  if (!s || !out8) return -1;
  for (int k = 0; k < 8; ++k) out8[k] = s->as_timing[k];
  return 0;
}

int miqp_solver_last_fixed_route(const miqp_solver_t* s) { return s ? s->fixed_route : -1; }

int miqp_gpu_has_active_set(int num_cars, int num_steps) { return miqp::as_shape_ok(num_cars, num_steps) ? 1 : 0; }

int miqp_solver_launch_plan(const miqp_solver_t* s, int bc, int overlap, int par, const int* cls_n3, int cus, double free_gb, int flags, int* out, int cap) {
  if (!s || !s->has_inst || !cls_n3 || !out || bc < 1 || cus < 1 || free_gb <= 0) return -1;
  miqp_solver_t* one[1] = {const_cast<miqp_solver_t*>(s)};
// ... 238 lines not shown
```

### planner_miqp_amd/csrc/oc_decode.hip

```cpp
namespace miqp {

constexpr int OC_GCAP = 128;
constexpr int OC_SCR = 32;
constexpr int OC_SSTR = 17;
constexpr int OC_KL0 = 6;

struct OcLds { int z, u, r, gmeta, gcoef, grhs, wd, sstart, cand, fix, total; };
constexpr int OC_GCAP_BIG = 320;
__host__ __device__ constexpr int oc_gcoef_of(int gcap) { return gcap == 128 ? 432 : gcap * 7 / 2; }
__host__ __device__ inline OcLds oc_lds_layout(int N, int fixlen, int OC_GCAP = miqp::OC_GCAP, bool as_std = false) {
  const int OC_GCOEF = oc_gcoef_of(OC_GCAP);
  OcLds L; int o = 0;
  L.z = o; o += N * 16 * 8;
  L.u = o; { int a = as_std ? N * 16 * 8 : N * 32 * 8, b = OC_SCR * OC_SSTR * 8; o += a > b ? a : b; }
  L.r = o; { int a = N * 32 * 8, b = as_std ? 0 : OC_GCAP * 16 + OC_KL0 * 64 * 8; o += a > b ? a : b; }
  L.gmeta = o; o += OC_GCAP * 16;
  L.gcoef = o; o += OC_GCOEF * 8;
  L.grhs = o; o += OC_GCAP * 8;
  L.wd = o; o += 16 * 8;
  L.sstart = o; o += ((N + 2) * 4 + 7) & ~7;
  L.cand = o; o += (OC_GCAP + 64) * 2;
  L.fix = o; o += (fixlen + 15) & ~15;
  L.total = (o + 15) & ~15;
  return L;
}

#define OC_WAVE_SYNC() do { __builtin_amdgcn_fence(__ATOMIC_RELEASE, "wavefront"); __builtin_amdgcn_wave_barrier(); __builtin_amdgcn_fence(__ATOMIC_ACQUIRE, "wavefront"); } while (0)

template <int C>
__device__ inline bool box_of_slot(const Layout& Y, const double* D, const int* T, const signed char* fix, int i, int slot, int& col, double& sgn, double& rhs) {
  if (slot >= C * Y.SC) return false;
  const int N = Y.N;
  const double* G = D + Y.d_glob;
  const int c = slot / Y.SC, rr = slot - c * Y.SC;
  const int code = i >= 1 ? (int)fix[Y.f_reg + c * N + i] : -1;
  const double* rt = code >= 0 ? D + Y.d_reg + (c * Y.P + (code >> 2)) * REGSZ : nullptr;
  if (rr < 7) {
    const double* Hc = (rt || rr < 3) ? D : region_hull(Y, D, T, fix, c, i);
    switch (rr) {
      case 0: col = 6 * c + 1; sgn = -1; rhs = -G[0]; break;
      case 1: col = 6 * c + 4; sgn = -1; rhs = -G[0]; break;
      case 2: col = 6 * c + 1; sgn = 1; rhs = G[1]; break;
      case 3: col = 6 * c + 2; sgn = 1; rhs = rt ? rt[12] : Hc[1]; break;
      case 4: col = 6 * c + 2; sgn = -1; rhs = -(rt ? rt[11] : Hc[0]); break;
      case 5: col = 6 * c + 5; sgn = 1; rhs = rt ? rt[14] : Hc[3]; break;
      default: col = 6 * c + 5; sgn = -1; rhs = -(rt ? rt[13] : Hc[2]); break;
    }
    return true;
  }
  if (rr < 11) {
    const int s = (rr - 7) >> 1; const bool up = ((rr - 7) & 1) == 0;
    double lo, hi;
    if (i == 0) { lo = D[Y.d_u0box + c * 4 + 2 * s]; hi = D[Y.d_u0box + c * 4 + 2 * s + 1]; }
    else if (rt) { lo = rt[15 + 2 * s]; hi = rt[16 + 2 * s]; }
    else { const double* Hc = region_hull(Y, D, T, fix, c, i); lo = Hc[4 + 2 * s]; hi = Hc[5 + 2 * s]; }
    col = 6 * C + 2 * c + s; sgn = up ? 1.0 : -1.0; rhs = up ? hi : -lo;
    return true;
  }
  if (rr < 16) {
    if (code < 0) return false;
    const int h = code & 3, k = rr - 11;
    if (h == 3) { col = 6 * c + (k < 2 ? 1 : 4); sgn = (k & 1) ? -1.0 : 1.0; rhs = G[6]; return true; }
    if (k == 2) {
      const int* hs = T + Y.i_hs + ((c * Y.P + (code >> 2)) * 2 + h) * 2;
      col = 6 * c + (hs[0] == 0 ? 1 : 4); sgn = -(double)hs[1]; rhs = -G[6];
      return true;
    }
    return false;
  }
  int q = rr - 16;
  const double* ed;
  if (q < 5 * Y.EL) {
    const int pt = q / Y.EL, k = q - pt * Y.EL;
    if (pt != 0) return false;
    const int e = Y.E == 1 ? 0 : (int)fix[Y.f_env + (c * N + i) * 5];
    ed = D + Y.d_env + (e * Y.EL + k) * 3;
  } else {
    q -= 5 * Y.EL;
    const int o = q / 5, pt = q - o * 5;
    if (pt != 0) return false;
    const int kk = (int)fix[Y.f_obs + ((c * Y.O + o) * N + i) * 5];
    ed = D + Y.d_obs + ((o * N + i) * Y.L + kk) * 3;
  }
  if (ed[1] == 0.0 && fabs(ed[0]) == 1.0) { col = 6 * c; sgn = ed[0]; rhs = ed[2]; return true; }
  if (ed[0] == 0.0 && fabs(ed[1]) == 1.0) { col = 6 * c + 3; sgn = ed[1]; rhs = ed[2]; return true; }
  return false;
}

template <int C>
__device__ inline bool slot_maybe(const Layout& Y, const signed char* fix, int i, int slot) {
  const int N = Y.N;
  if (slot < C * Y.SC) {
    const int c = slot / Y.SC, rr = slot - c * Y.SC;
    if (rr < 11) return true;
    if (i < 1) return false;
    const int code = (int)fix[Y.f_reg + c * N + i];
    if (rr < 16) return code >= 0 ? ((code & 3) != 3 || rr - 11 <= 3) : rr - 11 <= 1;
    int q = rr - 16;
    if (q < 5 * Y.EL) {
      if (Y.E < 1) return false;
      const int pt = q / Y.EL;
      const int e = Y.E == 1 ? 0 : (int)fix[Y.f_env + (c * N + i) * 5 + pt];
      return e >= 0 && (pt == 0 || code >= 0);
    }
    q -= 5 * Y.EL;
    const int o = q / 5, pt = q - o * 5;
    const int kk = (int)fix[Y.f_obs + ((c * Y.O + o) * N + i) * 5 + pt];
    return kk >= 0 && kk < Y.L && (pt == 0 || code >= 0);
  }
  if (C < 2 || i < 1) return false;
  const int q = slot - C * Y.SC;
  if (q < Y.NP * 8) { const int p = q >> 3, grp = (q & 7) >> 1; return (int)fix[Y.f_c2c + (p * N + i) * 4 + grp] >= 0; }
  const int q2 = q - Y.NP * 8, p = q2 >> 4, grp = (q2 >> 2) & 3, alt = q2 & 3;
  const int m = (int)fix[Y.f_c2n + (p * N + i) * 4 + grp];
  return m > 0 && ((m >> alt) & 1);
}

}
```

### planner_miqp_amd/csrc/solve_diag.hpp

```cpp
#pragma once

inline void debug_sync(hipStream_t st, int round, const char* stage, int nodes = -1) {
  hipError_t e_ = hipStreamSynchronize(st);
  if (nodes >= 0) std::fprintf(stderr, "[dbg] round %d %s (%d nodes): %s\n", round, stage, nodes, hipGetErrorString(e_));
  else std::fprintf(stderr, "[dbg] round %d %s: %s\n", round, stage, hipGetErrorString(e_));
}

inline bool trace_selection(const DevCtx& X, int rounds, int bc) {
  const DevBuf& B = X.B;
  std::vector<double> sb(bc); std::vector<int> sd(bc); double io_ = 0; int md_ = 0;
  HIP_OK(hipMemcpy(sb.data(), B.batch_bound, (size_t)bc * 8, hipMemcpyDeviceToHost)); HIP_OK(hipMemcpy(sd.data(), B.batch_depth, (size_t)bc * 4, hipMemcpyDeviceToHost));
  HIP_OK(hipMemcpy(&io_, B.inc_obj, 8, hipMemcpyDeviceToHost)); HIP_OK(hipMemcpy(&md_, B.inst_mode, 4, hipMemcpyDeviceToHost));
  std::vector<int> ord(bc); for (int k = 0; k < bc; ++k) ord[k] = k;
  std::sort(ord.begin(), ord.end(), [&](int a, int b) { return sd[a] != sd[b] ? sd[a] > sd[b] : sb[a] < sb[b]; });
  std::fprintf(stderr, "[sel] r%d mode %d incumbent %a:", rounds, md_, io_);
  for (int k : ord) std::fprintf(stderr, " %d.%d/%a", sd[k] >> 6, sd[k] & 63, sb[k]);
  std::fprintf(stderr, "\n");
  return true;
}

inline bool trace_batch(const DevCtx& X, int rounds, int bc) {
  const DevBuf& B = X.B; hipStream_t st = X.stream;
  HIP_OK(hipStreamSynchronize(st));
  if (X.stream2) HIP_OK(hipStreamSynchronize(X.stream2));
  std::vector<int> hd(bc), hi(bc), hk(bc); std::vector<double> ho(bc), hb(bc), hv(bc);
  HIP_OK(hipMemcpy(hd.data(), B.batch_depth, bc * 4, hipMemcpyDeviceToHost)); HIP_OK(hipMemcpy(hi.data(), B.batch_it, bc * 4, hipMemcpyDeviceToHost));
  HIP_OK(hipMemcpy(hk.data(), B.batch_ok, bc * 4, hipMemcpyDeviceToHost)); HIP_OK(hipMemcpy(ho.data(), B.batch_obj, bc * 8, hipMemcpyDeviceToHost));
  HIP_OK(hipMemcpy(hb.data(), B.batch_bound, bc * 8, hipMemcpyDeviceToHost)); HIP_OK(hipMemcpy(hv.data(), B.batch_viol, bc * 8, hipMemcpyDeviceToHost));
  std::vector<int> ord(bc); for (int k = 0; k < bc; ++k) ord[k] = k;
  std::sort(ord.begin(), ord.end(), [&](int a, int b) { return hd[a] != hd[b] ? hd[a] < hd[b] : (ho[a] != ho[b] ? ho[a] < ho[b] : hi[a] < hi[b]); });
  { int oc_ = 0, fc_ = 0, tk_ = 0, dm_ = 0; double nt_ = 0;
    HIP_OK(hipMemcpy(&oc_, B.open_count, 4, hipMemcpyDeviceToHost)); if (B.far_cap > 0) HIP_OK(hipMemcpy(&fc_, B.far_count, 4, hipMemcpyDeviceToHost));
    HIP_OK(hipMemcpy(&nt_, B.near_thr, 8, hipMemcpyDeviceToHost)); HIP_OK(hipMemcpy(&tk_, B.slot_take, 4, hipMemcpyDeviceToHost)); HIP_OK(hipMemcpy(&dm_, B.slot_demand, 4, hipMemcpyDeviceToHost));
    std::fprintf(stderr, "[lists] r%d batch %d: near list after selection %d, far tier %d, near_thr %g, share of the next round %d, demand %d\n", rounds, bc, oc_, fc_, nt_, tk_, dm_); }
  for (int k : ord) std::fprintf(stderr, "[trace] r%d depth %d.%d ok %d it %d obj %a bound %a viol %.3e\n", rounds, hd[k] >> 6, hd[k] & 63, hk[k], hi[k], ho[k], hb[k], hv[k]);
  return true;
}

inline bool trace_launches(const DevCtx& X, int rounds, int bc, size_t nev) {
  const DevBuf& B = X.B; hipStream_t st = X.stream;
  HIP_OK(hipStreamSynchronize(st));
  float m1 = 0, m2 = 0; HIP_OK(hipEventElapsedTime(&m1, X.ipm_ev[nev], X.ev_mid)); HIP_OK(hipEventElapsedTime(&m2, X.ev_mid, X.ipm_ev[nev + 1]));
  int oc = 0; HIP_OK(hipMemcpy(&oc, B.ovf_count, 4, hipMemcpyDeviceToHost));
  std::vector<int> ol(std::max(oc, 1)), hit(bc), hdw(bc), hok(bc);
  if (oc > 0) HIP_OK(hipMemcpy(ol.data(), B.ovf_list, (size_t)oc * 4, hipMemcpyDeviceToHost));
  HIP_OK(hipMemcpy(hit.data(), B.batch_it, (size_t)bc * 4, hipMemcpyDeviceToHost)); HIP_OK(hipMemcpy(hdw.data(), B.batch_depth, (size_t)bc * 4, hipMemcpyDeviceToHost));
  HIP_OK(hipMemcpy(hok.data(), B.batch_ok, (size_t)bc * 4, hipMemcpyDeviceToHost));
  int np = 0, mxp = 0, mxo = 0, mxc = 0; long long sp = 0, so = 0, sc = 0;
  for (int q = 0; q < oc; ++q) { const int k = ol[q]; if ((hdw[k] & 63) == 63 && (hdw[k] >> 6) >= 1) { np++; sp += hit[k]; mxp = std::max(mxp, hit[k]); } else { so += hit[k]; mxo = std::max(mxo, hit[k]); } }
  std::vector<char> isov(bc, 0); for (int q = 0; q < oc; ++q) isov[ol[q]] = 1;
  for (int k = 0; k < bc; ++k) if (!isov[k]) { sc += hit[k]; mxc = std::max(mxc, hit[k]); }
  std::fprintf(stderr, "[launch] round %d nodes %d: on-chip %.2f ms (%d nodes, mean it %.1f, max %d); behind it %.2f ms: %d probes (mean it %.1f, max %d), %d others (mean it %.1f, max %d)\n",
               rounds, bc, m1, bc - oc, (double)sc / std::max(1, bc - oc), mxc, m2, np, (double)sp / std::max(1, np), mxp, oc - np, (double)so / std::max(1, oc - np), mxo);
  return true;
}

inline bool replay_batch(DevCtx& X, int bc) {
  static int replay = process_switches().replay;
  if (replay <= 0) return true;
  const DevBuf& B = X.B; hipStream_t st = X.stream; const Layout& Y = X.Y; (void)Y;
  hipEvent_t e0, e1; HIP_OK(hipEventCreate(&e0)); HIP_OK(hipEventCreate(&e1));
  HIP_OK(hipEventRecord(e0, st));
  for (int r = 0; r < replay; ++r) launch_ipm_batch(X, B, bc, st);
  HIP_OK(hipEventRecord(e1, st)); HIP_OK(hipStreamSynchronize(st));
  float ms = 0; HIP_OK(hipEventElapsedTime(&ms, e0, e1));
  std::vector<int> its(bc); HIP_OK(hipMemcpy(its.data(), B.batch_it, (size_t)bc * 4, hipMemcpyDeviceToHost));
  long long tot = 0; for (int v : its) tot += v;
  std::fprintf(stderr, "[miqp_gpu replay] %d nodes, %lld node-iterations: %.3f ms per pass, %.1f ns per node-iteration\n", bc, tot, ms / replay, 1e6 * ms / replay / (double)tot);
#ifdef MIQP_ABLATE
  if (X.oc_grid > 0 && Y.C == 2) {
    const size_t l_oc = (size_t)oc_lds_layout(Y.N, Y.fixlen).total;
    auto run = [&](auto kern, int mask) {
      HIP_OK(hipFuncSetAttribute((const void*)kern, hipFuncAttributeMaxDynamicSharedMemorySize, (int)l_oc));
      auto once = [&] { (void)hipMemsetAsync(B.work_counter, 0, 4, st); (void)hipMemsetAsync(B.ovf_count, 0, 4, st); hipLaunchKernelGGL(kern, dim3(std::min(bc, X.oc_grid)), dim3(64), l_oc, st, B); };
      once(); HIP_OK(hipEventRecord(e0, st)); for (int r = 0; r < 3; ++r) once(); HIP_OK(hipEventRecord(e1, st)); HIP_OK(hipStreamSynchronize(st));
      float m2 = 0; HIP_OK(hipEventElapsedTime(&m2, e0, e1));
      std::fprintf(stderr, "[miqp_gpu ablate] mask %4d: %.3f ms per pass of %d nodes x 15 iterations = %.1f ns per node-iteration\n", mask, m2 / 3, bc, 1e6 * m2 / 3 / (bc * 15.0));
      return true;
    };
    run(ipm_onchip_kernel<2, OC_NSL, 1>, 1); run(ipm_onchip_kernel<2, OC_NSL, 3>, 3); run(ipm_onchip_kernel<2, OC_NSL, 5>, 5); run(ipm_onchip_kernel<2, OC_NSL, 9>, 9);
    run(ipm_onchip_kernel<2, OC_NSL, 17>, 17); run(ipm_onchip_kernel<2, OC_NSL, 33>, 33); run(ipm_onchip_kernel<2, OC_NSL, 65>, 65); run(ipm_onchip_kernel<2, OC_NSL, 129>, 129);
    run(ipm_onchip_kernel<2, OC_NSL, 257>, 257); run(ipm_onchip_kernel<2, OC_NSL, 513>, 513); run(ipm_onchip_kernel<2, OC_NSL, 1023>, 1023);
    run(ipm_onchip_kernel<2, OC_NSL, 1025>, 1025);
    launch_ipm_batch(X, B, bc, st);
  }
#endif
  replay = 0;
  return true;
}

inline bool print_progress(const DevCtx& X, double t, int rounds, long long launched_nodes, double const0) {
  const DevBuf& B = X.B; hipStream_t st = X.stream;
  double lb0 = 0, io0 = 0; int oc0 = 0; unsigned long long k0 = 0;
  HIP_OK(hipMemcpyAsync(&lb0, B.lower_bound, 8, hipMemcpyDeviceToHost, st)); HIP_OK(hipMemcpyAsync(&io0, B.inc_obj, 8, hipMemcpyDeviceToHost, st));
  HIP_OK(hipMemcpyAsync(&oc0, B.open_count, 4, hipMemcpyDeviceToHost, st)); HIP_OK(hipMemcpyAsync(&k0, B.inc_key, 8, hipMemcpyDeviceToHost, st));
  int fc0 = 0; HIP_OK(hipMemcpyAsync(&fc0, B.far_count, 4, hipMemcpyDeviceToHost, st));
  HIP_OK(hipStreamSynchronize(st));
  std::fprintf(stderr, "[miqp_gpu] t %.2f s round %d nodes %lld: instance 0 bound %.4f incumbent %.4f open %d + %d\n", t, rounds, launched_nodes, lb0, k0 >= 0xFFF0000000000000ull ? INFINITY : io0 + const0, oc0, fc0);
  return true;
}

inline bool dump_open_list(const DevCtx& X, const char* dp, int rounds, int NS, double const0) {
  const DevBuf& B = X.B; const Layout& Y = X.Y; const int open_cap = X.open_cap;
  int oc0 = 0; HIP_OK(hipMemcpy(&oc0, B.open_count, 4, hipMemcpyDeviceToHost)); oc0 = std::min(oc0, open_cap);
  const size_t src = ((size_t)(rounds & 1) * NS + 0) * open_cap;
  std::vector<double> hb(oc0); std::vector<int> hn(oc0), hd(oc0);
  if (oc0 > 0) { HIP_OK(hipMemcpy(hb.data(), B.open_bound + src, (size_t)oc0 * 8, hipMemcpyDeviceToHost)); HIP_OK(hipMemcpy(hn.data(), B.open_node + src, (size_t)oc0 * 4, hipMemcpyDeviceToHost));
    HIP_OK(hipMemcpy(hd.data(), B.open_depth + src, (size_t)oc0 * 4, hipMemcpyDeviceToHost)); }
  std::vector<int> ord(oc0); for (int k = 0; k < oc0; ++k) ord[k] = k;
  std::sort(ord.begin(), ord.end(), [&](int x, int y) { return hb[x] < hb[y]; });
  if (FILE* f = std::fopen(dp, "w")) {
    std::fprintf(f, "%d %d %d %d %d %d %d\n", oc0, Y.fixlen, Y.f_reg, Y.f_env, Y.f_obs, Y.f_c2c, Y.N);
    std::vector<signed char> rec(Y.fixlen);
    for (int q = 0; q < std::min(oc0, 400); ++q) {
      int k = ord[q]; HIP_OK(hipMemcpy(rec.data(), B.pool_fix + (size_t)hn[k] * Y.fixlen, Y.fixlen, hipMemcpyDeviceToHost));
      std::fprintf(f, "%.9g %d", hb[k] + const0, hd[k] >> 6); for (int x = 0; x < Y.fixlen; ++x) std::fprintf(f, " %d", (int)rec[x]); std::fprintf(f, "\n");
    }
    std::fclose(f);
  }
  return true;
}

#ifdef MIQP_PROFILE
inline bool print_profile(const DevCtx& X) {
  const DevBuf& B = X.B;
  { unsigned long long pf[64]; HIP_OK(hipMemcpy(pf, B.prof + 64, 64 * 8, hipMemcpyDeviceToHost));
    const char* nm[10] = {"decode", "rowpass", "bw.phi", "bw.TS+p", "bw.readlane+LDL", "bw.Ksolve", "bw.update", "forward", "step", "update"};
    double tot = 0; for (int q = 0; q < 10; ++q) tot += (double)pf[q];
    { unsigned long long po[16]; HIP_OK(hipMemcpy(po, B.prof, 16 * 8, hipMemcpyDeviceToHost));
      const char* no[9] = {"build", "bw.rows/assemble", "bw.mfma", "bw.TS", "bw.cholK", "bw.P", "forward", "step", "update"};
      double to = 0; for (int q = 0; q < 9; ++q) to += (double)po[q];
      if (po[10]) { std::fprintf(stderr, "[miqp_gpu profile] memory-backed kernel nodes %llu iters %llu cycles/node-iter %.0f :", po[10], po[9], to / std::max(1ull, po[9]));
        for (int q = 0; q < 9; ++q) std::fprintf(stderr, " %s %.1f%% (%.0f)", no[q], 100.0 * po[q] / to, (double)po[q] / std::max(1ull, po[9]));
        std::fprintf(stderr, "; inside bw.TS, the stage-Hessian chain: weights + staging %.0f, single-entry rows %.0f, MFMA loop %.0f, reductions + diagonal %.0f", (double)po[12] / std::max(1ull, po[9]), (double)po[13] / std::max(1ull, po[9]), (double)po[14] / std::max(1ull, po[9]), (double)po[15] / std::max(1ull, po[9]));
        std::fprintf(stderr, "\n"); } }
    std::fprintf(stderr, "[miqp_gpu profile] on-chip nodes %llu iters %llu cycles/node-iter %.0f :", pf[11], pf[10], tot / std::max(1ull, pf[10]));
    for (int q = 0; q < 10; ++q) std::fprintf(stderr, " %s %.1f%% (%.0f)", nm[q], 100.0 * pf[q] / tot, (double)pf[q] / std::max(1ull, pf[10]));
    std::fprintf(stderr, "\n");
    { unsigned long long pa[14]; HIP_OK(hipMemcpy(pa, B.prof + 80, 14 * 8, hipMemcpyDeviceToHost));
      const char* na[9] = {"decode", "gains + first iterate", "scan", "response of the row", "q", "directions + ratio test + M update", "iterate refresh", "results", "warm start"};
      double ta = 0; for (int q = 0; q < 9; ++q) ta += (double)pa[q];
      if (pa[10]) { std::fprintf(stderr, "[miqp_gpu profile] active-set kernel nodes %llu steps %llu cycles/node %.0f :", pa[10], pa[11], ta / (double)pa[10]);
        for (int q = 0; q < 9; ++q) std::fprintf(stderr, " %s %.1f%% (%.0f)", na[q], 100.0 * pa[q] / ta, (double)pa[q] / (double)pa[10]);
        std::fprintf(stderr, "; inside the decode: bound classes %.0f, general-row pass %.0f", (double)pa[12] / (double)pa[10], (double)pa[13] / (double)pa[10]);
        std::fprintf(stderr, "\n");
        unsigned long long pw[3], pl[6]; HIP_OK(hipMemcpy(pw, B.prof + 94, 3 * 8, hipMemcpyDeviceToHost)); HIP_OK(hipMemcpy(pl, B.prof + 120, 6 * 8, hipMemcpyDeviceToHost));
        if (pw[2] && pw[1] && pl[5]) std::fprintf(stderr, "[miqp_gpu profile] standard active-set launches: %llu wavefronts resident %.0f shader cycles = %.1f us each (shader clock %.0f MHz); per launch (%llu folded): span %.3f ms, from the first wavefront out of work to the last end %.3f ms, wavefronts %.0f, resident wavefront time / (span x wavefronts) %.3f\n",
          pw[2], (double)pw[0] / pw[2], (double)pw[1] / pw[2] / 100.0, 100.0 * (double)pw[0] / (double)pw[1], pl[5], (double)pl[3] / pl[5] / 1e5, (double)pl[4] / pl[5] / 1e5, (double)pw[2] / pl[5], ((double)pw[1]) / ((double)pl[3] * ((double)pw[2] / pl[5])));
        unsigned long long ph[16]; HIP_OK(hipMemcpy(ph, B.prof + 128, 16 * 8, hipMemcpyDeviceToHost));
        if (pw[2]) { std::fprintf(stderr, "[miqp_gpu profile] standard active-set wavefronts by their start after the launch's first (< 0.05 / 0.2 / 0.5 / 1 / 2 / 4 / 8 ms / later), %% :");
          for (int q = 0; q < 8; ++q) std::fprintf(stderr, " %.1f", 100.0 * ph[q] / pw[2]);
          std::fprintf(stderr, "; by the nodes they solved (0 / <= 4 / <= 16 / <= 32 / <= 64 / more), %% :");
          for (int q = 8; q < 14; ++q) std::fprintf(stderr, " %.1f", 100.0 * ph[q] / pw[2]);
          std::fprintf(stderr, "\n"); }
        if (const char* wd = X.sw.wave_dump) {
          std::vector<unsigned long long> w(4 * 4 * 4096); HIP_OK(hipMemcpy(w.data(), B.prof + 160, w.size() * 8, hipMemcpyDeviceToHost));
          if (FILE* f = std::fopen(wd, "w")) { for (int q = 0; q < 4 * 4096; ++q) if (w[4 * q]) std::fprintf(f, "%d %llu %llu %u %u %llu %d\n", q & 4095, w[4 * q], w[4 * q + 1], (unsigned)(w[4 * q + 2] >> 32), (unsigned)w[4 * q + 2], w[4 * q + 3], q >> 12); std::fclose(f); } } } }
    { unsigned long long pe[8]; HIP_OK(hipMemcpy(pe, B.prof + 100, 8 * 8, hipMemcpyDeviceToHost));
      const char* ne[6] = {"load", "regions", "leaf disjunctions", "branching", "lifting + reservation", "records"};
      double te = 0; for (int q = 0; q < 6; ++q) te += (double)pe[q];
      if (pe[6]) { std::fprintf(stderr, "[miqp_gpu profile] eval_kernel, %llu branched nodes, cycles/node %.0f :", pe[6], te / (double)pe[6]);
        for (int q = 0; q < 6; ++q) std::fprintf(stderr, " %s %.1f%% (%.0f)", ne[q], 100.0 * pe[q] / te, (double)pe[q] / (double)pe[6]);
        std::fprintf(stderr, "\n"); } }
    { unsigned long long ps[10]; HIP_OK(hipMemcpy(ps, B.prof + 110, 10 * 8, hipMemcpyDeviceToHost));
      const char* ns[8] = {"incumbent copy / kill", "setup", "pass 1 (prune, keys)", "far refill", "bound reduce + spill select", "focus + window + share", "radix select + ties", "pass 3 (emit, compact)"};
      double ts = 0; for (int q = 0; q < 8; ++q) ts += (double)ps[q];
      if (ps[8]) { std::fprintf(stderr, "[miqp_gpu profile] select_kernel, %llu workgroups that reached the end (thread 0's clock), mean list %.0f entries, cycles each %.0f :", ps[8], (double)ps[9] / (double)ps[8], ts / (double)ps[8]);
        for (int q = 0; q < 8; ++q) std::fprintf(stderr, " %s %.1f%% (%.0f)", ns[q], 100.0 * ps[q] / ts, (double)ps[q] / (double)ps[8]);
        std::fprintf(stderr, "\n"); } }
    HIP_OK(hipMemset(B.prof, 0, 160 * 8)); }
  return true;
}
#endif

inline bool print_stats(const DevCtx& X) {
  const DevBuf& B = X.B; const Layout& Y = X.Y;
  unsigned long long hs[256]; HIP_OK(hipMemcpy(hs, B.stats, sizeof(hs), hipMemcpyDeviceToHost)); HIP_OK(hipMemset(B.stats, 0, sizeof(hs)));
  const double nn_ = (double)std::max(1ull, hs[0]);
  std::fprintf(stderr, "[miqp_gpu stats] on-chip nodes %llu (general rows %.1f, coefficients %.1f, box keys %.1f, iterations %.1f per node), handed over %llu; general rows / 32 histogram:", hs[0], hs[1] / nn_, hs[4] / nn_, hs[2] / nn_, hs[5] / nn_, hs[3]);
  for (int q = 0; q < 16; ++q) std::fprintf(stderr, " %llu", hs[8 + q]);
  std::fprintf(stderr, "\n");
  std::fprintf(stderr, "[miqp_gpu stats] node outcomes: infeasible %llu (%.1f it), cut off %llu (%.1f it), not converged %llu (%.1f it), solved %llu (%.1f it) of which: bound >= incumbent %llu, within gap %llu, integer feasible %llu, branched %llu (%.2f children; by kind region/env/obstacle/car-car: %llu x %.1f, %llu x %.1f, %llu x %.1f, %llu x %.1f)\n",
               hs[32], hs[36] / (double)std::max(1ull, hs[32]), hs[33], hs[37] / (double)std::max(1ull, hs[33]), hs[34], hs[38] / (double)std::max(1ull, hs[34]), hs[35], hs[39] / (double)std::max(1ull, hs[35]),
               hs[40], hs[41], hs[42], hs[43], hs[44] / (double)std::max(1ull, hs[43]), hs[48], hs[52] / (double)std::max(1ull, hs[48]), hs[49], hs[53] / (double)std::max(1ull, hs[49]),
               hs[50], hs[54] / (double)std::max(1ull, hs[50]), hs[51], hs[55] / (double)std::max(1ull, hs[51]));
  std::fprintf(stderr, "[miqp_gpu stats] region sets: tightened at %llu (car, step) sites, %llu nodes closed because a step had no region left; children not created because of their lifted bound %llu (multi-row lift larger than the single-row one: %llu), car/car sets tightened at %llu groups\n", hs[58], hs[59], hs[56], hs[57], hs[61]);
  std::fprintf(stderr, "[miqp_gpu stats] region branchings flagged by: own rows %llu (worst class acc box %llu, jerk box %llu, sector %llu, half-plane %llu, curvature %llu, slow square %llu), environment front rows %llu, obstacle front rows %llu, car/car front rows %llu; by step:",
               hs[64], hs[70], hs[71], hs[72], hs[73], hs[74], hs[75], hs[65], hs[66], hs[67]);
  for (int q = 0; q < 32 && q < Y.N; ++q) std::fprintf(stderr, " %llu", hs[160 + q]);
  std::fprintf(stderr, "\n[miqp_gpu stats] node outcomes by origin (processed: infeasible / cut off / not converged / solved):");
  const char* on_[16] = {"root|reg-ref", "reg-adjacent", "reg-other", "reg-slow", "env-ref", "env-other", "-", "-", "obs-ref", "obs-other", "-", "-", "c2c-ref", "c2c-other", "-", "probe"};
  for (int q = 0; q < 16; ++q) if (hs[80 + q]) std::fprintf(stderr, " %s %llu: %llu / %llu / %llu / %llu;", on_[q], hs[80 + q], hs[96 + q], hs[112 + q], hs[128 + q], hs[144 + q]);
  std::fprintf(stderr, "\n[miqp_gpu stats] infeasible rounding probes re-rounded: %llu", hs[62]);
  std::fprintf(stderr, "\n[miqp_gpu stats] handed-over nodes with >= 480 general rows: %llu, mean %.0f, most %llu general rows", hs[7], (double)hs[6] / std::max(1ull, hs[7]), hs[5]);
  std::fprintf(stderr, "\n[miqp_gpu stats] rounding probes by iterations / 3 (0-2, 3-5, ..., 45+):");
  { const char* oc_n[4] = {"infeasible", "cut off", "not converged", "solved"};
    for (int o = 0; o < 4; ++o) { std::fprintf(stderr, " %s", oc_n[o]); for (int q = 0; q < 16; ++q) std::fprintf(stderr, " %llu", hs[192 + 16 * o + q]); std::fprintf(stderr, ";"); } }
  std::fprintf(stderr, "\n");
  return true;
}

inline void print_as_stats(const unsigned long long* h_as) {
  std::fprintf(stderr, "[miqp_gpu stats] active-set launch: %llu nodes (%.1f steps, %.1f drops, %.1f rows from the parent's active set, %.1f active rows at the end per node; %llu infeasible, %llu cut off; %llu started from the parent's M, %llu fell back to a cold start), %llu handed to the interior point (no free slot %llu, step cap %llu, curvature %llu, down-date pivot %llu, rows off their equalities %llu, other %llu); M rebuilt because: the parent left none %llu, the ring had come round %llu, another row count %llu; in the larger block %llu nodes (%.1f steps), of them leaves of the local search %llu (%.1f steps), rounding probes %llu; by their general rows (<= 64 / 96 / 128 / 192 / more) %llu / %llu / %llu / %llu / %llu\n",
               h_as[0], h_as[1] / (double)std::max(1ull, h_as[0]), h_as[3] / (double)std::max(1ull, h_as[0]), h_as[7] / (double)std::max(1ull, h_as[0]), h_as[6] / (double)std::max(1ull, h_as[0]), h_as[4], h_as[5], h_as[8], h_as[9], h_as[2], h_as[11], h_as[12], h_as[13], h_as[14], h_as[15], h_as[10], h_as[17], h_as[18], h_as[19], h_as[20], h_as[21] / (double)std::max(1ull, h_as[20]), h_as[22], h_as[23] / (double)std::max(1ull, h_as[22]), h_as[29], h_as[24], h_as[25], h_as[26], h_as[27], h_as[28]);
}
```

### planner_miqp_amd/wrapper.py

```python
import ctypes as C
import enum
import os
import subprocess

import numpy as np

os.environ.setdefault("GPU_MAX_HW_QUEUES", "8")

from .ctypes_types import (Certificate, CertificateC, FixedResultC, ModelParameters, ModelParamsC, RawResults, RawResultsC, SolutionPropertiesC, SolverOptsC,
                           c_double_p)

_HERE = os.path.dirname(os.path.abspath(__file__))
_LIB = None
EXCHANGE_FN = C.CFUNCTYPE(C.c_int, C.c_void_p, C.c_int, C.c_void_p, C.c_int, C.c_int)


def library_path():
    return os.environ.get("MIQP_GPU_LIB", os.path.join(_HERE, "libmiqp_gpu.so"))


def build_library(force=False):
    src = os.path.join(_HERE, "csrc", "miqp_gpu.hip")
    out = library_path()
    deps = [os.path.join(_HERE, "csrc", f) for f in os.listdir(os.path.join(_HERE, "csrc"))]
    deps += [os.path.join(_HERE, "..", "include", f) for f in ("miqp_gpu.h", "miqp_types.h")]
    if not force and os.path.exists(out) and all(os.path.getmtime(out) >= os.path.getmtime(d) for d in deps):
        return out
    hipcc = os.environ.get("HIPCC", "/opt/rocm/bin/hipcc")
    cmd = [hipcc, "--offload-arch=gfx950", "-O3", "-fno-math-errno", "-fno-trapping-math",
           "-Xarch_device", "-freciprocal-math", "-Xarch_device", "-fno-signed-zeros",
           "-fPIC", "-shared", "-std=c++17", "-o", out, src]
    subprocess.check_call(cmd)
    return out


def load_library():
    global _LIB
    if _LIB is not None:
        return _LIB
    path = library_path()
    if not os.path.exists(path):
        raise RuntimeError("libmiqp_gpu.so is not built (run __graft_entry__.build()); the solver has no CPU fallback")
    L = C.CDLL(path)
    vp = C.c_void_p
    L.miqp_solver_create.restype = vp; L.miqp_solver_create.argtypes = [C.POINTER(SolverOptsC)]
    L.miqp_solver_destroy.restype = None; L.miqp_solver_destroy.argtypes = [vp]
    L.miqp_solver_set_params.restype = C.c_int; L.miqp_solver_set_params.argtypes = [vp, C.POINTER(ModelParamsC)]
    L.miqp_solver_load_dat.restype = C.c_int; L.miqp_solver_load_dat.argtypes = [vp, C.c_char_p]
    L.miqp_solver_override_settings.restype = C.c_int; L.miqp_solver_override_settings.argtypes = [vp, C.c_double, C.c_double]
    L.miqp_solver_set_warmstart.restype = C.c_int; L.miqp_solver_set_warmstart.argtypes = [vp, C.POINTER(RawResultsC), C.c_int]
    L.miqp_solver_solve.restype = C.c_int; L.miqp_solver_solve.argtypes = [vp, C.c_double]
    L.miqp_solver_solve_batch.restype = C.c_int; L.miqp_solver_solve_batch.argtypes = [C.POINTER(vp), C.c_int, C.POINTER(C.c_int)]
    L.miqp_solver_solve_stream.restype = C.c_int; L.miqp_solver_solve_stream.argtypes = [C.POINTER(vp), C.c_int, C.c_int, C.POINTER(C.c_int)]
    L.miqp_solver_solve_batch_multi.restype = C.c_int; L.miqp_solver_solve_batch_multi.argtypes = [C.POINTER(vp), C.c_int, C.c_int, C.POINTER(C.c_int)]
    L.miqp_solver_raw_sizes.restype = C.c_int; L.miqp_solver_raw_sizes.argtypes = [vp, C.POINTER(C.c_int)]
    L.miqp_solver_lift_tables.restype = C.c_int; L.miqp_solver_lift_tables.argtypes = [vp, c_double_p, C.c_int]
    L.miqp_solver_solve_split.restype = C.c_int; L.miqp_solver_solve_split.argtypes = [vp, C.c_double, C.c_int, C.c_int, EXCHANGE_FN, vp]
    L.miqp_solver_solve_split_rccl.restype = C.c_int; L.miqp_solver_solve_split_rccl.argtypes = [vp, C.c_double]
    L.miqp_solver_split_roots.restype = C.c_int
    L.miqp_solver_split_roots.argtypes = [vp, C.c_int, C.c_int, C.POINTER(C.c_int), C.POINTER(C.c_int), C.POINTER(C.c_int), C.c_int, C.POINTER(C.c_int), C.POINTER(C.c_int)]
    L.miqp_comm_unique_id.restype = C.c_int; L.miqp_comm_unique_id.argtypes = [C.c_char_p]
    L.miqp_comm_init.restype = C.c_int; L.miqp_comm_init.argtypes = [C.c_int, C.c_int, C.c_char_p, C.c_int]
    L.miqp_comm_finalize.restype = C.c_int; L.miqp_comm_finalize.argtypes = []
    L.miqp_comm_selftest.restype = C.c_int; L.miqp_comm_selftest.argtypes = [EXCHANGE_FN, vp, C.c_int, C.c_int]
    L.miqp_solver_get_results.restype = C.c_int; L.miqp_solver_get_results.argtypes = [vp, C.POINTER(RawResultsC)]
    L.miqp_solver_materialize_results.restype = C.c_int; L.miqp_solver_materialize_results.argtypes = [C.POINTER(vp), C.c_int, C.c_int]
    L.miqp_solver_get_properties.restype = C.c_int; L.miqp_solver_get_properties.argtypes = [vp, C.POINTER(SolutionPropertiesC)]
    L.miqp_solver_get_dims.restype = C.c_int; L.miqp_solver_get_dims.argtypes = [vp, C.POINTER(C.c_int)]
    L.miqp_solver_export_lp.restype = C.c_int; L.miqp_solver_export_lp.argtypes = [vp, C.c_char_p]
    for fn in (L.miqp_solver_write_dat, L.miqp_solver_write_solution, L.miqp_solver_write_mst, L.miqp_solver_read_mst):
        fn.restype = C.c_int; fn.argtypes = [vp, C.c_char_p]
    L.miqp_solver_solve_fixed.restype = C.c_int
    L.miqp_solver_solve_fixed.argtypes = [vp, C.POINTER(RawResultsC), C.POINTER(RawResultsC), C.POINTER(C.c_double), C.POINTER(C.c_int)]
    L.miqp_solver_last_timing.restype = C.c_int; L.miqp_solver_last_timing.argtypes = [vp, C.POINTER(C.c_double)]
    L.miqp_solver_last_setup.restype = C.c_int; L.miqp_solver_last_setup.argtypes = [vp, C.POINTER(C.c_double)]
    L.miqp_solver_last_active_set.restype = C.c_int; L.miqp_solver_last_active_set.argtypes = [vp, C.POINTER(C.c_double)]
    L.miqp_solver_last_fixed_route.restype = C.c_int; L.miqp_solver_last_fixed_route.argtypes = [vp]
    L.miqp_solver_last_error.restype = C.c_char_p; L.miqp_solver_last_error.argtypes = [vp]
    L.miqp_solver_last_admission.restype = C.c_int; L.miqp_solver_last_admission.argtypes = [vp, C.POINTER(C.c_double)]
    L.miqp_solver_certify.restype = C.c_int; L.miqp_solver_certify.argtypes = [vp, C.POINTER(RawResultsC), C.POINTER(CertificateC)]
    L.miqp_solver_certify_batch.restype = C.c_int; L.miqp_solver_certify_batch.argtypes = [C.POINTER(vp), C.c_int, C.POINTER(CertificateC)]
    L.miqp_gpu_certificate_size.restype = C.c_int; L.miqp_gpu_certificate_size.argtypes = []
    L.miqp_gpu_certify_last_timing.restype = C.c_int; L.miqp_gpu_certify_last_timing.argtypes = [C.POINTER(C.c_double)]
    L.miqp_gpu_has_active_set.restype = C.c_int; L.miqp_gpu_has_active_set.argtypes = [C.c_int, C.c_int]
    L.miqp_solver_launch_plan.restype = C.c_int
    L.miqp_solver_launch_plan.argtypes = [vp, C.c_int, C.c_int, C.c_int, C.POINTER(C.c_int), C.c_int, C.c_double, C.c_int, C.POINTER(C.c_int), C.c_int]
    L.miqp_solver_solve_fixed_batch.restype = C.c_int
    L.miqp_solver_solve_fixed_batch.argtypes = [vp, C.POINTER(C.POINTER(RawResultsC)), C.c_int, C.POINTER(FixedResultC), C.POINTER(C.c_int)]
    L.miqp_solver_fixed_batch_record.restype = C.c_int; L.miqp_solver_fixed_batch_record.argtypes = [vp, C.c_int, C.POINTER(RawResultsC)]
    L.miqp_gpu_fixed_result_size.restype = C.c_int; L.miqp_gpu_fixed_result_size.argtypes = []
    L.miqp_gpu_fixed_batch_chunk.restype = C.c_int; L.miqp_gpu_fixed_batch_chunk.argtypes = []
    L.miqp_solver_set_pool.restype = C.c_int; L.miqp_solver_set_pool.argtypes = [vp, C.c_int]
    L.miqp_solver_pool_count.restype = C.c_int; L.miqp_solver_pool_count.argtypes = [vp]
    L.miqp_solver_pool_found.restype = C.c_int; L.miqp_solver_pool_found.argtypes = [vp, c_double_p, C.c_int]
    L.miqp_solver_pool_solve.restype = C.c_int; L.miqp_solver_pool_solve.argtypes = [vp, C.POINTER(FixedResultC), C.c_int]
    L.miqp_solver_pool_record.restype = C.c_int; L.miqp_solver_pool_record.argtypes = [vp, C.c_int, C.POINTER(RawResultsC)]
    L.miqp_gpu_pool_max.restype = C.c_int; L.miqp_gpu_pool_max.argtypes = []
    L.miqp_solver_set_pool_filter.restype = C.c_int; L.miqp_solver_set_pool_filter.argtypes = [vp, C.c_int]
    L.miqp_gpu_pool_signature.restype = C.c_int
    L.miqp_gpu_pool_signature.argtypes = [C.c_int, C.c_int, C.c_int, C.c_int, C.POINTER(C.c_byte), C.POINTER(C.c_byte), C.c_int]
    L.miqp_solver_pool_signature.restype = C.c_int; L.miqp_solver_pool_signature.argtypes = [vp, C.POINTER(RawResultsC), C.c_int, C.POINTER(C.c_byte), C.c_int]
    L.miqp_solver_pool_found_decisions.restype = C.c_int; L.miqp_solver_pool_found_decisions.argtypes = [vp, C.c_int, C.POINTER(C.c_byte), C.c_int]
    L.miqp_solver_solve_fixed_multi.restype = C.c_int
    L.miqp_solver_solve_fixed_multi.argtypes = [C.POINTER(vp), C.c_int, C.POINTER(C.POINTER(RawResultsC)), C.POINTER(C.c_int), C.POINTER(FixedResultC), C.POINTER(C.c_int)]
    L.miqp_solver_pool_solve_multi.restype = C.c_int
    L.miqp_solver_pool_solve_multi.argtypes = [C.POINTER(vp), C.c_int, C.POINTER(FixedResultC), C.c_int, C.POINTER(C.c_int)]
    if L.miqp_gpu_fixed_result_size() != C.sizeof(FixedResultC):
        raise RuntimeError("libmiqp_gpu.so and ctypes_types.FixedResultC disagree on miqp_fixed_result_c (%d / %d bytes): rebuild the library"
                           % (L.miqp_gpu_fixed_result_size(), C.sizeof(FixedResultC)))
    L.miqp_gpu_version.restype = C.c_char_p
    _LIB = L
    return L


EXPORTED_SYMBOLS = ["miqp_solver_create", "miqp_solver_destroy", "miqp_solver_set_params", "miqp_solver_load_dat",
                    "miqp_solver_override_settings", "miqp_solver_set_warmstart", "miqp_solver_solve",
                    "miqp_solver_solve_batch", "miqp_solver_get_results", "miqp_solver_get_properties",
                    "miqp_solver_get_dims", "miqp_solver_export_lp", "miqp_solver_solve_fixed",
                    "miqp_solver_last_timing", "miqp_solver_last_active_set", "miqp_solver_last_setup", "miqp_solver_last_error", "miqp_solver_last_admission", "miqp_gpu_version", "miqp_solver_write_dat", "miqp_solver_write_solution",
                    "miqp_solver_write_mst", "miqp_solver_read_mst", "miqp_fraction_parameters", "miqp_mean_angles",
                    "miqp_limits_per_region", "miqp_calculate_region_idx", "miqp_reserve_neighbor_regions",
                    "miqp_calculate_possible_regions", "miqp_calculate_warmstart", "miqp_plan",
                    "miqp_solver_solve_batch_multi", "miqp_solver_raw_sizes", "miqp_solver_lift_tables", "miqp_reference_trajectory", "miqp_update_car", "miqp_fitting_polynomial_parameters",
                    "miqp_solver_solve_split", "miqp_solver_solve_split_rccl", "miqp_solver_split_roots", "miqp_comm_unique_id",
                    "miqp_comm_init", "miqp_comm_finalize", "miqp_comm_selftest", "miqp_solver_solve_stream", "miqp_solver_materialize_results",
                    "miqp_initial_pose_check", "miqp_select_environment", "miqp_obstacle_intersects_environment", "miqp_obstacles_roi", "miqp_bark_trajectory", "miqp_obstacle_intersects_environment_roi", "miqp_environment_warmstart",
                    "miqp_solver_certify", "miqp_solver_certify_batch", "miqp_gpu_certificate_size", "miqp_gpu_certify_last_timing",
                    "miqp_gpu_has_active_set", "miqp_solver_last_fixed_route", "miqp_solver_launch_plan",
                    "miqp_solver_solve_fixed_batch", "miqp_solver_fixed_batch_record", "miqp_gpu_fixed_result_size", "miqp_gpu_fixed_batch_chunk",
                    "miqp_solver_set_pool", "miqp_solver_pool_count", "miqp_solver_pool_found", "miqp_solver_pool_solve", "miqp_solver_pool_record", "miqp_gpu_pool_max",
                    "miqp_solver_solve_fixed_multi", "miqp_solver_pool_solve_multi",
                    "miqp_solver_set_pool_filter", "miqp_gpu_pool_signature", "miqp_solver_pool_signature", "miqp_solver_pool_found_decisions"]


LAUNCH_PLAN_FIELDS = ("kernel", "stream", "grid", "lds", "ovf_mode", "cls_take", "as_split", "skip_probes", "bounce", "work", "from_ovf2", "bufs", "zero")


_FIXED_RESULT_DTYPE = np.dtype([("status", "<i4"), ("route", "<i4"), ("iterations", "<i4"), ("reserved", "<i4"), ("objective", "<f8"), ("violation", "<f8")])


POOL_BY_REGION, POOL_BY_ENVIRONMENT, POOL_BY_OBSTACLE, POOL_BY_CAR_CAR, POOL_EXACT_TIMING = 1, 2, 4, 8, 16


def _decision_len(cars, steps, obstacles):
    return cars * steps * 6 + cars * obstacles * steps * 5 + cars * (cars - 1) // 2 * steps * 4


def pool_signature(cars, steps, obstacles, families, decisions):
    d = np.ascontiguousarray(decisions, dtype=np.int8)
    D = _decision_len(int(cars), int(steps), int(obstacles))
    if d.ndim != 1 or d.size < D or D <= 0:
        raise ValueError("%d decision bytes given, the shape has %d" % (d.size, D))
    out = np.empty(D, dtype=np.int8)
    bp = C.POINTER(C.c_byte)
    rc = load_library().miqp_gpu_pool_signature(int(cars), int(steps), int(obstacles), int(families), d.ctypes.data_as(bp), out.ctypes.data_as(bp), D)
    if rc != D:
        raise ValueError("miqp_gpu_pool_signature refused the arguments (%d)" % rc)
    return out


def pool_max():
    return int(load_library().miqp_gpu_pool_max())


def fixed_batch_chunk():
    return int(load_library().miqp_gpu_fixed_batch_chunk())


def has_active_set(cars, steps):
    return int(load_library().miqp_gpu_has_active_set(int(cars), int(steps)))


class OptimizationStatus(enum.IntEnum):
    SUCCESS = 0
    FAILED_NO_SOLUT = 1
    FAILED_SEG_FAULT = 2
    FAILED_TIMEOUT = 3


class WarmstartType(enum.IntEnum):
    NO_WARMSTART = 0
    RECEDING_HORIZON_WARMSTART = 1
    LAST_SOLUTION_WARMSTART = 2
    BOTH_WARMSTART_STRATEGIES = 3


class ParameterSource(enum.IntEnum):
    DATFILE = 0
    CPPINPUTS = 1
    MIXED = 2


class SolutionProperties:
    def __init__(self, c=None):
        for n, _ in SolutionPropertiesC._fields_:
            setattr(self, n, getattr(c, n) if c is not None else 0)

    def __repr__(self):
        return "SolutionProperties(" + ", ".join("%s=%r" % (n, getattr(self, n)) for n, _ in SolutionPropertiesC._fields_) + ")"


class CplexWrapper:

    def __init__(self, modfile="cplexmodel.mod", parameterSource=ParameterSource.CPPINPUTS, precision=12, modpath="cplexmodel/",
                 nodes_per_round=0, max_open_nodes=0, gap_override=-1.0, verbose=0, device=-1):
        self._L = load_library()
        self._opts = SolverOptsC(int(precision), int(device), int(nodes_per_round), int(max_open_nodes), float(gap_override), int(verbose))
        self._h = self._L.miqp_solver_create(C.byref(self._opts))
        self.parameterSource_ = ParameterSource(parameterSource)
        self.modfile_ = modpath + modfile
        self.datfile_ = ""
        self._params = None
        self._keep = None
        self._results = None
        self._warm = None
        self.useSpecialOrderedSets_ = False
        self.useBranchingPriorities_ = False
        self.doWarmstart_ = WarmstartType.NO_WARMSTART
        self.debugOutputFilePath_ = ""
        self.debugOutputFilePrefix_ = ""
        self.print_debug_outputs_ = False
        self.debugOutputParameterFilePath_ = ""
        self.tmpWarmstartFile_ = "/tmp/warmstart_debug_res.mst"

    def __del__(self):
        try:
            if self._h:
                self._L.miqp_solver_destroy(self._h)
                self._h = None
        except Exception:
            pass

    def setParameterDatFileRelative(self, datfile):
        self.datfile_ = "cplexmodel/" + datfile

    def setParameterDatFileAbsolute(self, datfile):
        self.datfile_ = datfile

    def resetParameters(self, parameters: ModelParameters):
        self._params = parameters

    def overrideSolverSettingsDataSource(self, parameters: ModelParameters):
        if self._params is not None:
            for n in ["max_solution_time", "relative_mip_gap_tolerance", "mipdisplay", "mipemphasis", "relobjdif", "cutpass",
                      "probe", "repairtries", "rinsheur", "varsel", "mircuts", "parallelmode"]:
                setattr(self._params, n, getattr(parameters, n))

    def setSpecialOrderedSets(self, v):
        self.useSpecialOrderedSets_ = bool(v)

    def setUseBranchingPriorities(self, v):
        self.useBranchingPriorities_ = bool(v)

    def setBranchingPriorityValueExtent(self, value, extent):
        self.branchingPriority_ = (value, extent)

    def setBufferCplexOutputsToStream(self, v):
        pass

    def setDebugOutputPrint(self, v):
        self.print_debug_outputs_ = bool(v)

    def setDebugOutputFilePath(self, p):
        self.debugOutputFilePath_ = p

    def setDebugOutputFilePrefix(self, p):
        self.debugOutputFilePrefix_ = p

    def addRecedingHorizonWarmstart(self, warmstart: RawResults, wt=WarmstartType.RECEDING_HORIZON_WARMSTART):
        self.doWarmstart_ = wt if wt == WarmstartType.RECEDING_HORIZON_WARMSTART else WarmstartType.BOTH_WARMSTART_STRATEGIES
        self._warm = warmstart

    def setLastSolutionWarmstart(self, wt=WarmstartType.LAST_SOLUTION_WARMSTART):
        self.doWarmstart_ = wt if wt == WarmstartType.LAST_SOLUTION_WARMSTART else WarmstartType.BOTH_WARMSTART_STRATEGIES

    def deleteLastSolutionWarmstartFile(self):
        self._last = None
        if os.path.exists(self.tmpWarmstartFile_):
            os.remove(self.tmpWarmstartFile_)

    def _push_inputs(self):
        if self.parameterSource_ == ParameterSource.DATFILE:
            rc = self._L.miqp_solver_load_dat(self._h, self.datfile_.encode())
        elif self.parameterSource_ == ParameterSource.MIXED and self._params is None:
            rc = self._L.miqp_solver_load_dat(self._h, self.datfile_.encode())
        else:
            if self._params is None:
                return -1
            s, self._keep = self._params.to_c()
            rc = self._L.miqp_solver_set_params(self._h, C.byref(s))
        if rc != 0:
            return rc
        self._L.miqp_solver_set_warmstart(self._h, None, int(WarmstartType.NO_WARMSTART))
        if self.doWarmstart_ in (WarmstartType.RECEDING_HORIZON_WARMSTART, WarmstartType.BOTH_WARMSTART_STRATEGIES) and self._warm is not None:
            wc = self._warm.to_c()
            self._L.miqp_solver_set_warmstart(self._h, C.byref(wc), int(WarmstartType.RECEDING_HORIZON_WARMSTART))
        if self.doWarmstart_ in (WarmstartType.LAST_SOLUTION_WARMSTART, WarmstartType.BOTH_WARMSTART_STRATEGIES):
            if os.path.exists(self.tmpWarmstartFile_):
                self._L.miqp_solver_read_mst(self._h, self.tmpWarmstartFile_.encode())
        return 0

    def _stamp(self, timestamp):
        return "%.15g" % float(timestamp)

    def _debug_before(self, timestamp):
        if not self.print_debug_outputs_:
            return
        base = os.path.join(self.debugOutputFilePath_, self.debugOutputFilePrefix_)
        self.debugOutputParameterFilePath_ = base + "parameters_" + self._stamp(timestamp) + ".txt"
        self._L.miqp_solver_write_dat(self._h, self.debugOutputParameterFilePath_.encode())
        self._L.miqp_solver_export_lp(self._h, (base + "lpexport_" + self._stamp(timestamp) + ".lp").encode())

    def _debug_after(self, timestamp, status):
        if status != OptimizationStatus.SUCCESS:
            return
        last = self.doWarmstart_ in (WarmstartType.LAST_SOLUTION_WARMSTART, WarmstartType.BOTH_WARMSTART_STRATEGIES)
        if last:
            self._L.miqp_solver_write_mst(self._h, self.tmpWarmstartFile_.encode())
        if self.print_debug_outputs_:
            base = os.path.join(self.debugOutputFilePath_, self.debugOutputFilePrefix_)
            self._L.miqp_solver_write_solution(self._h, (base + "solution_" + self._stamp(timestamp) + ".txt").encode())
            if last:
                self._L.miqp_solver_write_mst(self._h, (base + "warmstartsolution_" + self._stamp(timestamp) + ".mst").encode())

    def _collect(self, status, lazy=False):
        self._stale = status == OptimizationStatus.SUCCESS
        if not self._stale:
            return OptimizationStatus(status)
        if not lazy:
            self._fetch()
        return OptimizationStatus(status)

    def _fetch(self):
        if getattr(self, "_stale", False):
            d = (C.c_int * 6)()
            self._L.miqp_solver_get_dims(self._h, d)
            res = RawResults(*list(d))
            rc = res.to_c()
            if self._L.miqp_solver_get_results(self._h, C.byref(rc)) != 0:
                raise RuntimeError("miqp_solver_get_results failed: the library holds no solution for this handle")
            self._results = res
            self._last = res
            self._stale = False

    def callCplex(self, timestamp=0.0):
        if self._push_inputs() != 0:
            return OptimizationStatus.FAILED_SEG_FAULT
        self._debug_before(timestamp)
        st = self._collect(self._L.miqp_solver_solve(self._h, float(timestamp)))
        self._debug_after(timestamp, st)
        return st

    def callCplexSplit(self, world, rank, exchange=None, timestamp=0.0):
        if self._push_inputs() != 0:
            return OptimizationStatus.FAILED_SEG_FAULT
        if exchange is None:
            st = self._L.miqp_solver_solve_split_rccl(self._h, float(timestamp))
        else:
            st = self._L.miqp_solver_solve_split(self._h, float(timestamp), int(world), int(rank), exchange, None)
        return self._collect(st)

    def splitRoots(self, world, rank):
        if self._push_inputs() != 0:
            return None
        cap = 4096
        ro, ix, va = (C.c_int * cap)(), (C.c_int * cap)(), (C.c_int * cap)()
        nr, nc = C.c_int(0), C.c_int(0)
        n = self._L.miqp_solver_split_roots(self._h, int(world), int(rank), ro, ix, va, cap, C.byref(nr), C.byref(nc))
        if n < 0:
            return None
        roots = [[] for _ in range(nr.value)]
        for k in range(min(n, cap)):
            roots[ro[k]].append((ix[k], va[k]))
        return roots, nc.value

    def getRawResults(self):
        self._fetch()
        return self._results

    def getSolutionProperties(self):
        p = SolutionPropertiesC()
        self._L.miqp_solver_get_properties(self._h, C.byref(p))
        return SolutionProperties(p)

    def getTmpWarmstartFile(self):
        return self.tmpWarmstartFile_

    def getDebugOutputParameterFilePath(self):
        return self.debugOutputParameterFilePath_

    def writeDat(self, path):
        if self._push_inputs() != 0:
            return -1
        return self._L.miqp_solver_write_dat(self._h, path.encode())

    def solveFixed(self, fixed: RawResults):
        if self._push_inputs() != 0:
            return None
        d = (C.c_int * 6)()
        self._L.miqp_solver_get_dims(self._h, d)
        out = RawResults(*list(d))
        oc = out.to_c()
        fc = fixed.to_c()
        obj = C.c_double(0)
        it = C.c_int(0)
        rc = self._L.miqp_solver_solve_fixed(self._h, C.byref(fc), C.byref(oc), C.byref(obj), C.byref(it))
        return rc, out, obj.value, it.value

    def lastFixedRoute(self):
        return int(self._L.miqp_solver_last_fixed_route(self._h))

    def launchPlan(self, bc, overlap=0, par=-1, cls_n=(-1, -1, -1), cus=256, free_gb=256.0, as_on=1, concurrent=True):
        if self._push_inputs() != 0:
            return None
        out = (C.c_int * (5 * len(LAUNCH_PLAN_FIELDS)))()
        n = self._L.miqp_solver_launch_plan(self._h, int(bc), int(overlap), int(par), (C.c_int * 3)(*cls_n), int(cus), float(free_gb),
                                            (1 if as_on else 0) | (0 if concurrent else 2), out, len(out))
        if n < 0:
            raise RuntimeError("miqp_solver_launch_plan failed (%d)" % n)
        k = len(LAUNCH_PLAN_FIELDS)
        return [tuple(out[i * k:(i + 1) * k]) for i in range(n)]

    def solveFixedBatch(self, records):
        if self._push_inputs() != 0:
            raise RuntimeError("invalid parameters")
        n = len(records)
        keep = [r.to_c() if r is not None else None for r in records]
        ptrs = (C.POINTER(RawResultsC) * max(n, 1))(*[C.pointer(c) if c is not None else None for c in keep])
        out = (FixedResultC * max(n, 1))()
        best = C.c_int(-1)
        rc = self._L.miqp_solver_solve_fixed_batch(self._h, ptrs, n, out, C.byref(best))
        if rc != 0:
            raise RuntimeError("miqp_solver_solve_fixed_batch failed (%d)" % rc)
        a = np.frombuffer(out, dtype=np.dtype([("status", "<i4"), ("route", "<i4"), ("iterations", "<i4"), ("reserved", "<i4"),
                                               ("objective", "<f8"), ("violation", "<f8")]), count=n)
        return (a["status"].copy(), a["objective"].copy(), a["violation"].copy(), a["iterations"].copy(), a["route"].copy(), best.value)

    def fixedBatchRecord(self, k):
        d = (C.c_int * 6)()
        if self._L.miqp_solver_get_dims(self._h, d) != 0:
            return -1, None
        out = RawResults(*list(d))
        oc = out.to_c()
        rc = self._L.miqp_solver_fixed_batch_record(self._h, int(k), C.byref(oc))
        return rc, (out if rc == 0 else None)

    def setSolutionPool(self, capacity):
        return int(self._L.miqp_solver_set_pool(self._h, int(capacity)))

    def setSolutionPoolFilter(self, families):
        return int(self._L.miqp_solver_set_pool_filter(self._h, int(families)))

    def solutionPoolFoundDecisions(self, k):
        d = (C.c_int * 6)()
        if self._L.miqp_solver_get_dims(self._h, d) != 0:
            return None
        out = np.empty(_decision_len(d[0], d[1], d[4]), dtype=np.int8)
        rc = self._L.miqp_solver_pool_found_decisions(self._h, int(k), out.ctypes.data_as(C.POINTER(C.c_byte)), out.size)
        return out if rc == out.size else None

    def poolSignature(self, record, families):
        d = (C.c_int * 6)()
        if self._L.miqp_solver_get_dims(self._h, d) != 0 and (self._push_inputs() != 0 or self._L.miqp_solver_get_dims(self._h, d) != 0):
            raise ValueError("invalid parameters")
        out = np.empty(_decision_len(d[0], d[1], d[4]), dtype=np.int8)
        rc = self._L.miqp_solver_pool_signature(self._h, C.byref(record.to_c()), int(families), out.ctypes.data_as(C.POINTER(C.c_byte)), out.size)
        if rc != out.size:
            raise ValueError("miqp_solver_pool_signature refused the arguments (%d)" % rc)
        return out

    def solutionPoolCount(self):
        return int(self._L.miqp_solver_pool_count(self._h))

    def solutionPoolFound(self):
        n = self.solutionPoolCount()
        o = np.zeros(max(n, 1))
        m = self._L.miqp_solver_pool_found(self._h, o.ctypes.data_as(c_double_p), n)
        return o[:max(m, 0)].copy()

    def solveSolutionPool(self):
        n = max(self.solutionPoolCount(), 1)
        out = (FixedResultC * n)()
        m = self._L.miqp_solver_pool_solve(self._h, out, n)
        if m < 0:
            raise RuntimeError("miqp_solver_pool_solve failed (%d)" % m)
        a = np.frombuffer(out, dtype=np.dtype([("status", "<i4"), ("route", "<i4"), ("iterations", "<i4"), ("reserved", "<i4"),
                                               ("objective", "<f8"), ("violation", "<f8")]), count=m)
        return (a["status"].copy(), a["objective"].copy(), a["violation"].copy(), a["iterations"].copy(), a["route"].copy())

    def solutionPoolRecord(self, k):
        d = (C.c_int * 6)()
        if self._L.miqp_solver_get_dims(self._h, d) != 0:
            return -1, None
        out = RawResults(*list(d))
        oc = out.to_c()
        rc = self._L.miqp_solver_pool_record(self._h, int(k), C.byref(oc))
        return rc, (out if rc == 0 else None)

    def liftTables(self):
        if self._push_inputs() != 0:
            raise RuntimeError("invalid parameters")
        p = self._params
        out = np.zeros((p.NumCars, 2, p.NumSteps, 4, 4))
        n = self._L.miqp_solver_lift_tables(self._h, out.ctypes.data_as(c_double_p), out.size)
        if n != out.size:
            raise RuntimeError("miqp_solver_lift_tables failed (%d)" % n)
        return out

    def rawSizes(self):
        if self._push_inputs() != 0:
            return None
        o = (C.c_int * 4)()
        if self._L.miqp_solver_raw_sizes(self._h, o) != 0:
            return None
        return dict(rows=o[0], bin=o[1], cont=o[2], nnz=o[3])

    def certify(self, candidate: RawResults = None, use_real_slack=True):
        out = CertificateC()
        if candidate is None:
            rc = self._L.miqp_solver_certify(self._h, None, C.byref(out))
        else:
            d = (C.c_int * 6)()
            if self._L.miqp_solver_get_dims(self._h, d) != 0 and self._push_inputs() != 0:
                raise RuntimeError("invalid parameters")
            cc = candidate.to_c()
            if not use_real_slack:
                cc.slackvars_real = None
            rc = self._L.miqp_solver_certify(self._h, C.byref(cc), C.byref(out))
        if rc != 0:
            raise RuntimeError("miqp_solver_certify failed (%d): %s" % (rc, self.lastError()))
        return Certificate(out)

    def lastAdmission(self):
        o = (C.c_double * 1)()
        self._L.miqp_solver_last_admission(self._h, o)
        return o[0]

    def lastError(self):
        return (self._L.miqp_solver_last_error(self._h) or b"").decode()

    def lastTiming(self):
        t = (C.c_double * 6)()
        self._L.miqp_solver_last_timing(self._h, t)
        u = (C.c_double * 3)()
        self._L.miqp_solver_last_setup(self._h, u)
        v = (C.c_double * 8)()
        self._L.miqp_solver_last_active_set(self._h, v)
        return dict(solve_s=t[0], ipm_s=t[1], ipm_launches=int(t[2]), nodes=int(t[3]), ipm_iters=int(t[4]), row_iters=int(t[5]),
                    setup_s=u[0], context_s=u[1], context_built=bool(u[2]),
                    as_nodes=int(v[0]), as_steps=int(v[1]), as_unfinished=int(v[2]), as_drops=int(v[3]), as_rows_end=int(v[4]), as_rows_parent=int(v[5]),
                    std_launch_s=v[6], std_launches=int(v[7]))


def prepare_batch(wrappers):
    for w in wrappers:
        if w._push_inputs() != 0:
            raise RuntimeError("invalid parameters")


def solve_batch(wrappers, gpus=None, inflight=None, prepared=False):
    L = load_library()
    if not prepared:
        prepare_batch(wrappers)
    n = len(wrappers)
    hs = (C.c_void_p * n)(*[w._h for w in wrappers])
    st = (C.c_int * n)(*([int(OptimizationStatus.FAILED_SEG_FAULT)] * n))
    if inflight is not None and gpus is None:
        rc = L.miqp_solver_solve_stream(hs, n, int(inflight), st)
    else:
        rc = L.miqp_solver_solve_batch(hs, n, st) if gpus is None else L.miqp_solver_solve_batch_multi(hs, n, int(gpus), st)
    if rc not in (0, -2):
        return [OptimizationStatus.FAILED_SEG_FAULT] * n
    return [w._collect(st[k], lazy=True) for k, w in enumerate(wrappers)]


def certify_batch(wrappers):
    L = load_library()
    n = len(wrappers)
    if n == 0:
        return []
    hs = (C.c_void_p * n)(*[w._h for w in wrappers])
    out = (CertificateC * n)()
    rc = L.miqp_solver_certify_batch(hs, n, out)
    if rc != 0:
        raise RuntimeError("miqp_solver_certify_batch failed (%d): %s" % (rc, wrappers[0].lastError()))
    return [Certificate(out[k]) for k in range(n)]


def solve_fixed_multi(wrappers, records_per_wrapper):
    L = load_library()
    n = len(wrappers)
    if n != len(records_per_wrapper):
        raise ValueError("one list of records per wrapper")
    d = (C.c_int * 6)()
    for w in wrappers:
        if L.miqp_solver_get_dims(w._h, d) != 0 and w._push_inputs() != 0:
            raise RuntimeError("invalid parameters")
    first = [0]
    for recs in records_per_wrapper:
        first.append(first[-1] + len(recs))
    total = first[-1]
    keep = [r.to_c() if r is not None else None for recs in records_per_wrapper for r in recs]
    ptrs = (C.POINTER(RawResultsC) * max(total, 1))(*[C.pointer(c) if c is not None else None for c in keep])
    out = (FixedResultC * max(total, 1))()
    best = (C.c_int * max(n, 1))(*([-1] * max(n, 1)))
    hs = (C.c_void_p * max(n, 1))(*[w._h for w in wrappers])
    rc = L.miqp_solver_solve_fixed_multi(hs, n, ptrs, (C.c_int * (n + 1))(*first), out, best)
    if rc != 0:
        raise RuntimeError("miqp_solver_solve_fixed_multi failed (%d)%s" % (rc, ": " + wrappers[0].lastError() if n and rc == -2 else ""))
    a = np.frombuffer(out, dtype=_FIXED_RESULT_DTYPE, count=total)
    return [(a["status"][first[h]:first[h + 1]].copy(), a["objective"][first[h]:first[h + 1]].copy(), a["violation"][first[h]:first[h + 1]].copy(),
             a["iterations"][first[h]:first[h + 1]].copy(), a["route"][first[h]:first[h + 1]].copy(), int(best[h])) for h in range(n)]


def solve_solution_pools(wrappers):
    L = load_library()
    n = len(wrappers)
    cap = max([w.solutionPoolCount() for w in wrappers] + [1])
    out = (FixedResultC * (max(n, 1) * cap))()
    counts = (C.c_int * max(n, 1))()
    hs = (C.c_void_p * max(n, 1))(*[w._h for w in wrappers])
    m = L.miqp_solver_pool_solve_multi(hs, n, out, cap, counts)
    if m < 0:
        raise RuntimeError("miqp_solver_pool_solve_multi failed (%d)%s" % (m, ": " + wrappers[0].lastError() if n and m == -2 else ""))
    a = np.frombuffer(out, dtype=_FIXED_RESULT_DTYPE, count=n * cap)
    res = []
    for h in range(n):
        b = a[h * cap:h * cap + counts[h]]
        res.append((b["status"].copy(), b["objective"].copy(), b["violation"].copy(), b["iterations"].copy(), b["route"].copy()))
    return res


def certify_last_timing():
    t = (C.c_double * 4)()
    load_library().miqp_gpu_certify_last_timing(t)
    return dict(pack_s=t[0], upload_s=t[1], kernel_s=t[2], call_s=t[3])


def materialize_results(wrappers, threads=0):
    L = load_library()
    n = len(wrappers)
    hs = (C.c_void_p * n)(*[w._h for w in wrappers])
    return L.miqp_solver_materialize_results(hs, n, int(threads))
```

Measured before the change: 1091.

## Replace active-set decode with compacted candidate-list enumeration and bitmap prefix

The active-set kernel now uses a new decode body. Bound classes are written directly with atomicMin. Sparse row candidates are compacted into an LDS list via wavefront ballots, then classified in batched flushes, and survivors go into a bitmap that a prefix scan turns into the candidate array. This is meant to avoid classifying every slot of every step, cutting decode cycles per node. It also adds a decode-compare kernel and API that check the new decode against the old one, plus profiling counters, at the cost of more code and LDS pressure for the list.

```diff
diff --git a/include/miqp_gpu.h b/include/miqp_gpu.h
--- a/include/miqp_gpu.h
+++ b/include/miqp_gpu.h
@@ -104,6 +104,9 @@
 
 int miqp_solver_launch_plan(const miqp_solver_t* s, int bc, int overlap, int par, const int* cls_n3, int cus, double free_gb, int flags, int* out, int cap);
 
+int miqp_solver_decode_compare(miqp_solver_t* s, const signed char* fix, int n, int gcap, int* out, int* layout16, signed char* fix_out);
+int miqp_gpu_decode_compare_words(void);
+
 int miqp_solver_last_setup(const miqp_solver_t* s, double* out3);
 
 int miqp_solver_last_admission(const miqp_solver_t* s, double* out1);
diff --git a/planner_miqp_amd/csrc/as_decode_body.inc b/planner_miqp_amd/csrc/as_decode_body.inc
--- /dev/null
+++ b/planner_miqp_amd/csrc/as_decode_body.inc
@@ -0,0 +1,215 @@
+#ifdef MIQP_PROFILE
+    long long ocd_t_sparse = 0, ocd_t_rows = 0, ocd_c_class = 0, ocd_c_prefix = 0, ocd_c_build = 0;
+#endif
+    int ngen = 0;
+    {
+      unsigned long long* const bmp = (unsigned long long*)scr;
+      const int nw = (N * NSLOT + 63) >> 6;
+      unsigned short* const pre = (unsigned short*)(bmp + nw);
+      for (int k = tid; k < nw; k += 64) bmp[k] = 0ull;
+      OC_WAVE_SYNC();
+      const unsigned int nslot_magic = oc_magic16(NSLOT);
+      unsigned short* const plist = pre + ((nw + 1 + 3) & ~3);
+      const int LCAP = (int)(((char*)(L0 + LL.r) - (char*)plist) / 2) - 64;
+      int nlist = 0;
+      auto flush = [&]() {
+        OC_WAVE_SYNC();
+#ifdef MIQP_PROFILE
+        const long long tf0 = clock64();
+#endif
+        for (int j0 = 0; j0 < nlist; j0 += 64) if (j0 + tid < nlist) {
+          const int pc = plist[j0 + tid]; const int i = oc_div16(pc, nslot_magic);
+          int col; double sg, rh;
+          const int kind = as_classify<C>(Y, D, T, fix, i, pc - i * NSLOT, col, sg, rh);
+          if (kind == 1) atomicMin(&bkey[(i * 2 + (sg < 0.0 ? 1 : 0)) * 16 + OC_DECODE_POLICY::col(col)], d2key(rh));
+          else if (kind == 2) atomicOr(&bmp[pc >> 6], 1ull << (pc & 63));
+        }
+        OC_WAVE_SYNC();
+#ifdef MIQP_PROFILE
+        ocd_c_class += clock64() - tf0;
+#endif
+        nlist = 0;
+      };
+      for (int e0 = 0; e0 < C * N; e0 += 64) {
+        const int e = e0 + tid;
+        if (e < C * N) {
+          const int c = e / N, i = e - c * N;
+          const double* G = D + Y.d_glob;
+          const int code = i >= 1 ? (int)fix[Y.f_reg + c * N + i] : -1;
+          const unsigned int skip = i >= 1 ? (unsigned int)T[Y.i_boxskip + c * N + i] : 0x7Fu;
+          const double* rt = code >= 0 ? D + Y.d_reg + (c * Y.P + (code >> 2)) * REGSZ : nullptr;
+          const double* Hc = (!rt && i >= 1) ? region_hull(Y, D, T, fix, c, i) : nullptr;
+          auto put = [&](int col, bool neg, double rh) { atomicMin(&bkey[(i * 2 + (neg ? 1 : 0)) * 16 + OC_DECODE_POLICY::col(col)], d2key(rh)); };
+          if (i >= 1) {
+            const double a_lo_x = rt ? rt[11] : Hc[0], a_hi_x = rt ? rt[12] : Hc[1], a_lo_y = rt ? rt[13] : Hc[2], a_hi_y = rt ? rt[14] : Hc[3];
+            if (!(skip & 1u)) put(6 * c + 1, true, -G[0]);
+            if (!(skip & 2u)) put(6 * c + 4, true, -G[0]);
+            if (!(skip & 4u)) put(6 * c + 1, false, G[1]);
+            if (!(skip & 8u)) put(6 * c + 2, false, a_hi_x);
+            if (!(skip & 16u)) put(6 * c + 2, true, -a_lo_x);
+            if (!(skip & 32u)) put(6 * c + 5, false, a_hi_y);
+            if (!(skip & 64u)) put(6 * c + 5, true, -a_lo_y);
+          }
+          if (i <= N - 2) {
+#pragma unroll
+            for (int s_ = 0; s_ < 2; ++s_) {
+              double lo, hi;
+              if (i == 0) { lo = D[Y.d_u0box + c * 4 + 2 * s_]; hi = D[Y.d_u0box + c * 4 + 2 * s_ + 1]; }
+              else if (rt) { lo = rt[15 + 2 * s_]; hi = rt[16 + 2 * s_]; }
+              else { lo = Hc[4 + 2 * s_]; hi = Hc[5 + 2 * s_]; }
+              put(6 * C + 2 * c + s_, false, hi); put(6 * C + 2 * c + s_, true, -lo);
+            }
+          }
+        }
+      }
+#ifdef MIQP_PROFILE
+      if (OC_DECODE_POLICY::MARKS) ocd_t_sparse = clock64();
+#endif
+      {
+        const int SC = Y.SC, EL = Y.EL, NPN = Y.NP * N;
+        const int env_end = 16 + 5 * EL;
+        for (int e0 = 0; e0 < C * N; e0 += 64) {
+          const int e = e0 + tid;
+          const int c = (C == 2 && e >= N) ? 1 : 0, i = e - c * N;
+          const bool site = e < C * N && i >= 1;
+          const int code = site ? (int)fix[Y.f_reg + e] : -1;
+          const int base = i * NSLOT + c * SC;
+          const signed char* const fe = fix + Y.f_env + e * 5;
+          const bool psite = C == 2 && e < NPN && e >= 1;
+          const int pbase = e * NSLOT + C * SC;
+          int nstep = SC - 11;
+          if constexpr (C == 2) {
+            bool anym = false;
+            if (psite) { const signed char* fm = fix + Y.f_c2n + e * 4; anym = fm[0] > 0 || fm[1] > 0 || fm[2] > 0 || fm[3] > 0; }
+            nstep += __ballot(anym) ? 20 : 4;
+          }
+          int pt = 0, kq = 0, ob = 0;
+#pragma unroll 1
+          for (int st = 0; st < nstep; ++st) {
+            const int rr = 11 + st;
+            bool cnd = false; int pc = 0, two = 0;
+            if (rr < SC) {
+              pc = base + rr;
+              if (rr < 16) cnd = site && (code >= 0 ? ((code & 3) != 3 || rr <= 14) : rr <= 12);
+              else if (rr < env_end) {
+                if (kq == EL) { kq = 0; ++pt; }
+                ++kq;
+                if (Y.E >= 1) { const int ev = (site && Y.E > 1) ? (int)fe[pt] : 0; cnd = site && ev >= 0 && (pt == 0 || code >= 0); }
+                if (rr + 1 == env_end) pt = 0;
+              } else {
+                if (pt == 5) { pt = 0; ++ob; }
+                if (site) { const int kk = (int)fix[Y.f_obs + ((c * Y.O + ob) * N + i) * 5 + pt]; cnd = kk >= 0 && kk < Y.L && (pt == 0 || code >= 0); }
+                ++pt;
+              }
+            } else if constexpr (C == 2) {
+              const int s2 = rr - SC;
+              if (s2 < 4) { two = 1; pc = pbase + 2 * s2; cnd = psite && (int)fix[Y.f_c2c + e * 4 + s2] >= 0; }
+              else {
+                const int g_ = (s2 - 4) >> 2, a_ = (s2 - 4) & 3;
+                pc = pbase + 8 + g_ * 4 + a_;
+                if (psite) { const int m = (int)fix[Y.f_c2n + e * 4 + g_]; cnd = m > 0 && ((m >> a_) & 1); }
+              }
+            }
+            const unsigned long long mk = __ballot(cnd);
+            if (mk) {
+              if (cnd) {
+                const int at = nlist + (__popcll(mk & lt) << two);
+                plist[at] = (unsigned short)pc;
+                if (two) plist[at + 1] = (unsigned short)(pc + 1);
+              }
+              nlist += __popcll(mk) << two;
+              if (nlist > LCAP - 64) flush();
+            }
+          }
+        }
+      }
+      flush();
+#ifdef MIQP_PROFILE
+      const long long ocd_t_listed = clock64();
+#endif
+      {
+        int carry = 0;
+        for (int k0 = 0; k0 < nw; k0 += 64) {
+          const int k = k0 + tid;
+          const int cnt = k < nw ? __popcll(bmp[k]) : 0;
+          int x = cnt;
+#pragma unroll
+          for (int d = 1; d < 64; d <<= 1) { const int y = __shfl_up(x, d); if (tid >= d) x += y; }
+          const int a = carry + x - cnt;
+          if (k < nw) pre[k] = (unsigned short)(a < 65535 ? a : 65535);
+          carry += __shfl(x, 63);
+        }
+        if (tid == 0) pre[nw] = (unsigned short)(carry < 65535 ? carry : 65535);
+        ngen = carry < 65535 ? carry : 65535;
+      }
+      OC_WAVE_SYNC();
+      if (ngen <= OC_GCAP)
+        for (int k = tid; k < nw; k += 64) {
+          unsigned long long bits = bmp[k]; int pos = pre[k];
+          while (bits) { const int b = __ffsll((long long)bits) - 1; cand[pos++] = (unsigned short)(k * 64 + b); bits &= bits - 1ull; }
+        }
+      OC_WAVE_SYNC();
+#ifdef MIQP_PROFILE
+      ocd_c_prefix = clock64() - ocd_t_listed;
+#endif
+    }
+#ifdef MIQP_PROFILE
+    if (OC_DECODE_POLICY::MARKS) ocd_t_rows = clock64();
+#endif
+    bool overflow = ngen > OC_GCAP;
+    int ncoef = 0;
+    {
+      const unsigned int nslot_magic_b = oc_magic16(NSLOT);
+      for (int c0 = 0; c0 < ngen && !overflow; c0 += 64) {
+#ifdef MIQP_PROFILE
+        const long long tb0_ = clock64();
+#endif
+        RowOut r; r.active = false; r.rhs = 0; r.aq = 0;
+        int i = 0, nn = 0;
+        const bool mine = c0 + tid < ngen;
+        int slot_ = 0, car0 = 0, car1 = 0; bool regpat = false;
+        double v8[8];
+#pragma unroll
+        for (int k = 0; k < 8; ++k) v8[k] = 0.0;
+        if (mine) { const int pcode = cand[c0 + tid]; i = oc_div16(pcode, nslot_magic_b); slot_ = pcode - i * NSLOT; r = as_sparse_row<C>(Y, D, T, fix, i, slot_, v8, car0, car1, regpat); }
+#ifdef MIQP_PROFILE
+        ocd_c_build += clock64() - tb0_;
+#endif
+        unsigned long long map = 0ull; unsigned int cols = 0u;
+        double v6[6];
+#pragma unroll
+        for (int k = 0; k < 6; ++k) v6[k] = 0.0;
+        if (mine) {
+#pragma unroll
+          for (int j = 0; j < (C == 2 ? 8 : 4); ++j) {
+            const double v = v8[j];
+            if (v != 0.0 && nn < 6) {
+#pragma unroll
+              for (int k = 0; k < 6; ++k) if (k == nn) v6[k] = v;
+              const int q = 6 * (j < 4 ? car0 : car1) + (j & 3) + ((j & 3) >= 2 ? 1 : 0) + (regpat ? 1 : 0);
+              const int pq = OC_DECODE_POLICY::col(q);
+              map |= (unsigned long long)(nn + 1) << (4 * pq); cols |= (unsigned int)pq << (4 * nn); nn++;
+            }
+          }
+        }
+        const bool keep = mine && nn > 0;
+        const unsigned long long mk = __ballot(keep);
+        const unsigned long long b0 = __ballot(keep && (nn & 1)), b1 = __ballot(keep && (nn & 2)), b2 = __ballot(keep && (nn & 4));
+        const int tot = __popcll(b0) + 2 * __popcll(b1) + 4 * __popcll(b2);
+        if (ncoef + tot > OC_GCOEF) { overflow = true; break; }
+        if (keep) {
+          const int idx = sstart[N + 1] + __popcll(mk & lt);
+          const int off = ncoef + __popcll(b0 & lt) + 2 * __popcll(b1 & lt) + 4 * __popcll(b2 & lt);
+#pragma unroll
+          for (int k = 0; k < 6; ++k) if (k < nn) gcoef[off + k] = v6[k];
+          uint4 m4; m4.x = (unsigned int)map; m4.y = (unsigned int)(map >> 32);
+          m4.z = (unsigned int)off | ((unsigned int)nn << 16) | ((unsigned int)i << 20) | (r.aq > 0.0 ? 0x80000000u : 0u); m4.w = cols;
+          gmeta[idx] = m4; grhs[idx] = r.rhs;
+          cand[idx] = (unsigned short)(i * NSLOT + slot_);
+        }
+        OC_WAVE_SYNC();
+        if (tid == 0) sstart[N + 1] += __popcll(mk);
+        ncoef += tot;
+        OC_WAVE_SYNC();
+      }
+    }
diff --git a/planner_miqp_amd/csrc/as_onchip.hip b/planner_miqp_amd/csrc/as_onchip.hip
--- a/planner_miqp_amd/csrc/as_onchip.hip
+++ b/planner_miqp_amd/csrc/as_onchip.hip
@@ -110,11 +110,11 @@
     }
 
 #ifdef MIQP_PROFILE
-    unsigned long long asp_[12] = {0, 0, 0, 0, 0, 0, 0, 0, 0, 0, 0, 0};
+    unsigned long long asp_[15] = {0, 0, 0, 0, 0, 0, 0, 0, 0, 0, 0, 0, 0, 0, 0};
 #endif
     ASP_T(ta0);
 #define OC_DECODE_POLICY AsDecode<C>
-#include "oc_decode_body.inc"
+#include "as_decode_body.inc"
 #undef OC_DECODE_POLICY
     if (overflow) {
       if (B.batch_A) B.batch_A[(size_t)node * 64 + tid] = 0xFFFFu;
@@ -130,6 +130,7 @@
     ASP_T(ta1); ASP_ACC(0, ta0, ta1);
 #ifdef MIQP_PROFILE
     asp_[9] += (unsigned long long)(ocd_t_sparse - ta0); asp_[11] += (unsigned long long)(ta1 - ocd_t_rows);
+    asp_[12] += (unsigned long long)ocd_c_class; asp_[13] += (unsigned long long)ocd_c_prefix; asp_[14] += (unsigned long long)ocd_c_build;
 #endif
     double brhs[NSL];
     unsigned int bact = 0u, binA = 0u, ginA = 0u;
@@ -598,6 +599,7 @@
       { const long long tc1 = clock64(); asp_[7] += (unsigned long long)(tc1 - tc0);
         for (int q_ = 0; q_ < 9; ++q_) atomicAdd(&B.prof[80 + q_], asp_[q_]);
         atomicAdd(&B.prof[92], asp_[9]); atomicAdd(&B.prof[93], asp_[11]);
+        atomicAdd(&B.prof[97], asp_[12]); atomicAdd(&B.prof[98], asp_[13]); atomicAdd(&B.prof[99], asp_[14]);
         atomicAdd(&B.prof[90], 1ull); atomicAdd(&B.prof[91], (unsigned long long)steps); }
 #endif
       if (B.as_stats) {
diff --git a/planner_miqp_amd/csrc/decode_compare.hip b/planner_miqp_amd/csrc/decode_compare.hip
--- /dev/null
+++ b/planner_miqp_amd/csrc/decode_compare.hip
@@ -0,0 +1,201 @@
+namespace miqp {
+
+constexpr int DC_WORDS = 16;
+enum DcKind { DC_NONE = 0, DC_OVERFLOW = 1, DC_NGEN = 2, DC_BKEY = 3, DC_SSTART = 4, DC_NCOEF = 5, DC_GMETA = 6, DC_GRHS = 7, DC_CAND = 8, DC_GCOEF = 9 };
+
+struct DecodeCompareArgs { Layout Y; const double* D; const int* T; const signed char* fix; int n; int* out; };
+
+template <int C, int GCAP>
+__global__ void __launch_bounds__(64) decode_compare_kernel(DecodeCompareArgs A) {
+  constexpr bool BIG = GCAP > 128;
+  constexpr int OC_GCAP = GCAP, OC_GCOEF = oc_gcoef_of(OC_GCAP);
+  constexpr int NZ = 8 * C;
+  const Layout& Y = A.Y;
+  const double* const D = A.D; const int* const T = A.T;
+  const int tid = threadIdx.x;
+  const int N = Y.N, NSLOT = Y.NSLOT;
+  const unsigned long long lt = (1ull << tid) - 1ull;
+  extern __shared__ double lds[];
+  const OcLds LL = oc_lds_layout(N, Y.fixlen, OC_GCAP, !BIG);
+  __shared__ unsigned int sh_mis, sh_cnt[10];
+  for (int rec = blockIdx.x; rec < A.n; rec += gridDim.x) {
+    __syncthreads();
+    if (tid == 0) sh_mis = ~0u;
+    if (tid < 10) sh_cnt[tid] = 0u;
+    int res_ngen[2], res_ovf[2], res_ncoef[2];
+#pragma unroll 1
+    for (int which = 0; which < 2; ++which) {
+      char* const L0 = (char*)lds + (size_t)which * LL.total;
+      double* const scr = (double*)(L0 + LL.u);
+      unsigned long long* const bkey = (unsigned long long*)(L0 + LL.r);
+      uint4* const gmeta = (uint4*)(L0 + LL.gmeta);
+      double* const gcoef = (double*)(L0 + LL.gcoef);
+      double* const grhs = (double*)(L0 + LL.grhs);
+      int* const sstart = (int*)(L0 + LL.sstart);
+      unsigned short* const cand = (unsigned short*)(L0 + LL.cand);
+      signed char* const fix = (signed char*)(L0 + LL.fix);
+      {
+        const signed char* src = A.fix + (size_t)rec * Y.fixlen;
+        for (int k = tid; k < Y.fixlen; k += 64) fix[k] = src[k];
+        for (int k = tid; k < N * 32; k += 64) bkey[k] = ~0ull;
+        for (int k = tid; k <= N + 1; k += 64) sstart[k] = 0;
+        for (int k = tid; k < OC_GCAP; k += 64) { gmeta[k] = make_uint4(0u, 0u, 0u, 0u); grhs[k] = 0.0; }
+        for (int k = tid; k < OC_GCOEF; k += 64) gcoef[k] = 0.0;
+        for (int k = tid; k < OC_GCAP + 64; k += 64) cand[k] = 0;
+      }
+      __syncthreads();
+      if (which == 0) {
+#define OC_DECODE_POLICY AsDecode<C>
+#include "oc_decode_body.inc"
+#undef OC_DECODE_POLICY
+        res_ngen[0] = ngen; res_ovf[0] = overflow ? 1 : 0; res_ncoef[0] = ncoef;
+      } else {
+#define OC_DECODE_POLICY AsDecode<C>
+#include "as_decode_body.inc"
+#undef OC_DECODE_POLICY
+        res_ngen[1] = ngen; res_ovf[1] = overflow ? 1 : 0; res_ncoef[1] = ncoef;
+      }
+      __syncthreads();
+    }
+    const char* const R0 = (const char*)lds; const char* const R1 = R0 + LL.total;
+    unsigned int mis = ~0u;
+    auto miss = [&](int kind, int index) { const unsigned int m = ((unsigned int)kind << 20) | (unsigned int)(index & 0xFFFFF); if (m < mis) mis = m; };
+    if (res_ovf[0] != res_ovf[1]) miss(DC_OVERFLOW, 0);
+    if (res_ngen[0] != res_ngen[1]) miss(DC_NGEN, 0);
+    const int NM = ((const int*)(R0 + LL.sstart))[N + 1];
+    if (!res_ovf[0] && !res_ovf[1]) {
+      const unsigned long long* k0 = (const unsigned long long*)(R0 + LL.r); const unsigned long long* k1 = (const unsigned long long*)(R1 + LL.r);
+      unsigned int nkeys = 0u;
+      for (int k = tid; k < N * 32; k += 64) { if (k0[k] != k1[k]) miss(DC_BKEY, k); if (k0[k] != ~0ull) ++nkeys; }
+      if (nkeys) atomicAdd(&sh_cnt[8], nkeys);
+      const int* s0 = (const int*)(R0 + LL.sstart); const int* s1 = (const int*)(R1 + LL.sstart);
+      for (int k = tid; k <= N + 1; k += 64) if (s0[k] != s1[k]) miss(DC_SSTART, k);
+      if (res_ncoef[0] != res_ncoef[1]) miss(DC_NCOEF, 0);
+      const uint4* m0 = (const uint4*)(R0 + LL.gmeta); const uint4* m1 = (const uint4*)(R1 + LL.gmeta);
+      const unsigned long long* h0 = (const unsigned long long*)(R0 + LL.grhs); const unsigned long long* h1 = (const unsigned long long*)(R1 + LL.grhs);
+      const unsigned short* c0_ = (const unsigned short*)(R0 + LL.cand); const unsigned short* c1_ = (const unsigned short*)(R1 + LL.cand);
+      const int cls_off[8] = {0, 7, 11, 16, 16 + Y.EL, 16 + 5 * Y.EL, C * Y.SC, C * Y.SC + 8 * Y.NP};
+      for (int k = tid; k < NM && k < OC_GCAP; k += 64) {
+        const uint4 a = m0[k], b = m1[k];
+        if (a.x != b.x || a.y != b.y || a.z != b.z || a.w != b.w) miss(DC_GMETA, k);
+        if (h0[k] != h1[k]) miss(DC_GRHS, k);
+        if (c0_[k] != c1_[k]) miss(DC_CAND, k);
+        const int pc = (int)c0_[k], slot = pc % NSLOT;
+        int cl;
+        if (slot >= C * Y.SC) cl = slot >= cls_off[7] ? 7 : 6;
+        else { const int rr = slot % Y.SC; cl = 0; for (int q = 1; q < 6; ++q) if (rr >= cls_off[q]) cl = q; }
+        atomicAdd(&sh_cnt[cl], 1u);
+      }
+      const unsigned long long* g0 = (const unsigned long long*)(R0 + LL.gcoef); const unsigned long long* g1 = (const unsigned long long*)(R1 + LL.gcoef);
+      for (int k = tid; k < res_ncoef[0] && k < OC_GCOEF; k += 64) if (g0[k] != g1[k]) miss(DC_GCOEF, k);
+    }
+    {
+      const signed char* const fix0 = (const signed char*)(R0 + LL.fix);
+      unsigned int nb = 0u;
+      for (int k = tid; k < C * (N - 1) * 5; k += 64) {
+        const int c = k / ((N - 1) * 5), r_ = k - c * (N - 1) * 5, i = 1 + r_ / 5, slot = c * Y.SC + 11 + r_ % 5;
+        int col; double sg, rh;
+        if (decode_row<C, false>(Y, D, T, fix0, i, slot, nullptr).active && box_of_slot<C>(Y, D, T, fix0, i, slot, col, sg, rh)) ++nb;
+      }
+      if (nb) atomicAdd(&sh_cnt[9], nb);
+    }
+    if (mis != ~0u) atomicMin(&sh_mis, mis);
+    __syncthreads();
+    if (tid == 0) {
+      int* o = A.out + (size_t)rec * DC_WORDS;
+      const unsigned int m = sh_mis;
+      o[0] = m == ~0u ? 0 : (int)(m >> 20); o[1] = m == ~0u ? 0 : (int)(m & 0xFFFFFu);
+      o[2] = res_ngen[0]; o[3] = res_ovf[0] ? 0 : NM; o[4] = res_ovf[0] ? 0 : res_ncoef[0]; o[5] = res_ovf[0]; o[6] = (int)sh_cnt[8];
+      for (int q = 0; q < 8; ++q) o[7 + q] = (int)sh_cnt[q];
+      o[15] = (int)sh_cnt[9];
+    }
+  }
+}
+
+namespace {
+
+bool dc_record_ok(const Layout& Y, const int* T, const signed char* f) {
+  const int C = Y.C, N = Y.N;
+  for (int c = 0; c < C; ++c) for (int i = 0; i < N; ++i) { const int code = f[Y.f_reg + c * N + i]; if (code < -1 || (code >= 0 && (code >> 2) >= std::min(Y.P, T[Y.i_nposs + c]))) return false; }
+  for (int k = Y.f_env; k < Y.f_obs; ++k) if (f[k] < -1 || f[k] >= std::max(Y.E, 1)) return false;
+  for (int k = Y.f_obs; k < Y.f_c2c; ++k) if (f[k] < -1) return false;
+  for (int k = Y.f_c2c; k < Y.f_c2n; ++k) if (f[k] < -1 || f[k] > 3) return false;
+  for (int k = Y.f_c2n; k < Y.f_rmask; ++k) if (f[k] < -1 || f[k] > 15) return false;
+  return true;
+}
+
+template <int C, int GCAP>
+bool dc_launch(const DecodeCompareArgs& A, hipStream_t st) {
+  const OcLds LL = oc_lds_layout(A.Y.N, A.Y.fixlen, GCAP, GCAP <= 128);
+  const size_t lds = 2 * (size_t)LL.total;
+  if (lds > 160 * 1024) return false;
+  HIP_OK(hipFuncSetAttribute((const void*)decode_compare_kernel<C, GCAP>, hipFuncAttributeMaxDynamicSharedMemorySize, (int)lds));
+  hipLaunchKernelGGL((decode_compare_kernel<C, GCAP>), dim3(std::min(A.n, 1024)), dim3(64), lds, st, A);
+  HIP_OK(hipGetLastError());
+  return true;
+}
+
+bool dc_run(DevCtx& X, const Layout& Y, const std::vector<double>& D, const std::vector<int>& T, const std::vector<signed char>& fix, int n, int gcap, int* out) {
+  double* dD = nullptr; int* dT = nullptr; signed char* dF = nullptr; int* dO = nullptr;
+  struct Free { double*& a; int*& b; signed char*& c; int*& d; ~Free() { (void)hipFree(a); (void)hipFree(b); (void)hipFree(c); (void)hipFree(d); } } fr{dD, dT, dF, dO};
+  HIP_OK(hipSetDevice(X.device));
+  HIP_OK(hipMalloc((void**)&dD, D.size() * 8)); HIP_OK(hipMalloc((void**)&dT, T.size() * 4));
+  HIP_OK(hipMalloc((void**)&dF, fix.size())); HIP_OK(hipMalloc((void**)&dO, (size_t)n * DC_WORDS * 4));
+  HIP_OK(hipMemcpy(dD, D.data(), D.size() * 8, hipMemcpyHostToDevice)); HIP_OK(hipMemcpy(dT, T.data(), T.size() * 4, hipMemcpyHostToDevice));
+  HIP_OK(hipMemcpy(dF, fix.data(), fix.size(), hipMemcpyHostToDevice)); HIP_OK(hipMemset(dO, 0xFF, (size_t)n * DC_WORDS * 4));
+  DecodeCompareArgs A; A.Y = Y; A.D = dD; A.T = dT; A.fix = dF; A.n = n; A.out = dO;
+  bool ok;
+  if (Y.C == 1) ok = gcap == OC_GCAP ? dc_launch<1, OC_GCAP>(A, nullptr) : dc_launch<1, OC_GCAP_BIG>(A, nullptr);
+  else ok = gcap == OC_GCAP ? dc_launch<2, OC_GCAP>(A, nullptr) : dc_launch<2, OC_GCAP_BIG>(A, nullptr);
+  if (!ok) return false;
+  HIP_OK(hipDeviceSynchronize());
+  HIP_OK(hipMemcpy(out, dO, (size_t)n * DC_WORDS * 4, hipMemcpyDeviceToHost));
+  return true;
+}
+
+}
+}
+
+extern "C" {
+
+int miqp_gpu_decode_compare_words(void) { return miqp::DC_WORDS; }
+
+int miqp_solver_decode_compare(miqp_solver_t* s, const signed char* fix, int n, int gcap, int* out, int* layout16, signed char* fix_out) {
+  using namespace miqp;
+  if (!s || !s->has_inst || n < 0 || (n > 0 && !out)) return -1;
+  if (!as_shape_ok(s->inst.C, s->inst.N) || (gcap != OC_GCAP && gcap != OC_GCAP_BIG)) return -2;
+  miqp_solver_t* one[1] = {s};
+  const BatchShape bs = batch_layout(one, 1);
+  if (!bs.ok) return -2;
+  const Layout& Y = bs.Y;
+  if (layout16) { const int v[16] = {Y.fixlen, Y.f_reg, Y.f_env, Y.f_obs, Y.f_c2c, Y.f_c2n, Y.f_rmask, Y.C, Y.N, Y.E, Y.EL, Y.O, Y.L, Y.NP, Y.SC, Y.NSLOT}; std::memcpy(layout16, v, sizeof(v)); }
+  if (n == 0) return 0;
+  std::vector<double> D(Y.dstride); std::vector<int> T(Y.istride);
+  compile_instance(s->inst, Y, D.data(), T.data());
+  const size_t fl = (size_t)Y.fixlen;
+  DevCtx* Xp = ctx_for_device(s->opts.device);
+  if (!Xp) return -3;
+  DevCtx& X = *Xp;
+  std::lock_guard<std::mutex> ctx_lock(X.mu);
+  std::vector<signed char> recs;
+  int m = 0;
+  if (fix) {
+    for (int k = 0; k < n; ++k) if (!dc_record_ok(Y, T.data(), fix + (size_t)k * fl)) return -4;
+    recs.assign(fix, fix + (size_t)n * fl); m = n;
+  } else {
+    if (!X.ready || !same_layout(X.Y, Y) || !X.B.pool_fix || !X.B.pool_count) return -5;
+    int cnt = 0;
+    if (hipSetDevice(X.device) != hipSuccess || hipMemcpy(&cnt, X.B.pool_count, 4, hipMemcpyDeviceToHost) != hipSuccess) return -3;
+    const int take = std::max(0, std::min({n, cnt, X.pool_cap}));
+    std::vector<signed char> raw((size_t)take * fl);
+    if (take > 0 && hipMemcpy(raw.data(), X.B.pool_fix, raw.size(), hipMemcpyDeviceToHost) != hipSuccess) return -3;
+    recs.reserve(raw.size());
+    for (int k = 0; k < take; ++k) if (dc_record_ok(Y, T.data(), raw.data() + (size_t)k * fl)) { recs.insert(recs.end(), raw.begin() + (size_t)k * fl, raw.begin() + (size_t)(k + 1) * fl); ++m; }
+  }
+  if (m == 0) return 0;
+  if (!dc_run(X, Y, D, T, recs, m, gcap, out)) { (void)hipDeviceSynchronize(); return -3; }
+  if (fix_out) std::memcpy(fix_out, recs.data(), recs.size());
+  return m;
+}
+
+}
diff --git a/planner_miqp_amd/csrc/miqp_gpu.hip b/planner_miqp_amd/csrc/miqp_gpu.hip
--- a/planner_miqp_amd/csrc/miqp_gpu.hip
+++ b/planner_miqp_amd/csrc/miqp_gpu.hip
@@ -1448,6 +1448,7 @@
 #include "fixed_batch.hip"
 #include "solution_pool.hip"
 #include "fixed_multi.hip"
+#include "decode_compare.hip"
 
 extern "C" {
 
diff --git a/planner_miqp_amd/csrc/oc_decode.hip b/planner_miqp_amd/csrc/oc_decode.hip
--- a/planner_miqp_amd/csrc/oc_decode.hip
+++ b/planner_miqp_amd/csrc/oc_decode.hip
@@ -116,4 +116,187 @@
   return m > 0 && ((m >> alt) & 1);
 }
 
-}
+__device__ inline unsigned int oc_magic16(int d) { return 0xFFFFFFFFu / (unsigned int)d + 1u; }
+__device__ inline int oc_div16(int n, unsigned int magic) { return (int)__umulhi((unsigned int)n, magic); }
+
+template <int C>
+__device__ inline int as_classify(const Layout& Y, const double* D, const int* T, const signed char* fix, int i, int slot, int& col, double& sgn, double& rhs) {
+  static_assert(C == 1 || C == 2, "the car of a slot is found by one comparison");
+  const int N = Y.N;
+  const double* G = D + Y.d_glob;
+  if (slot < C * Y.SC) {
+    const int c = (C == 2 && slot >= Y.SC) ? 1 : 0, rr = slot - c * Y.SC;
+    const int code = (int)fix[Y.f_reg + c * N + i];
+    if (rr < 16) {
+      const int k = rr - 11;
+      if (code < 0) return (k > 1 || D[Y.d_hull + (c * N + i) * HULLSZ + 14] == 0.0) ? 0 : 2;
+      const int h = code & 3;
+      if (h == 3) {
+        if (k > 3) return 0;
+        col = 6 * c + (k < 2 ? 1 : 4); sgn = (k & 1) ? -1.0 : 1.0; rhs = G[6];
+        return 1;
+      }
+      if (k != 2) return 2;
+      const int* hs = T + Y.i_hs + ((c * Y.P + (code >> 2)) * 2 + h) * 2;
+      col = 6 * c + (hs[0] == 0 ? 1 : 4); sgn = -(double)hs[1]; rhs = -G[6];
+      return 1;
+    }
+    int q = rr - 16;
+    const double* ed;
+    int pt;
+    if (q < 5 * Y.EL) {
+      if (Y.E < 1) return 0;
+      const int EL = Y.EL;
+      pt = (q >= EL ? 1 : 0) + (q >= 2 * EL ? 1 : 0) + (q >= 3 * EL ? 1 : 0) + (q >= 4 * EL ? 1 : 0);
+      const int k = q - pt * EL;
+      const signed char* fe = fix + Y.f_env + (c * N + i) * 5;
+      const int e = Y.E == 1 ? 0 : (int)fe[pt];
+      if (e < 0 || k >= T[Y.i_envn + e] || (pt > 0 && code < 0)) return 0;
+      ed = D + Y.d_env + (e * EL + k) * 3;
+      if (pt > 0) {
+        int txs, tys;
+        if (corner_dominated(ENV_PT_D[pt][0], ENV_PT_D[pt][1], ed[0], ed[1], T[Y.i_dom + (c * Y.P + (code >> 2)) * 4 + (code & 3)], txs, tys)) {
+          const int es = Y.E == 1 ? 0 : (int)fe[env_corner(txs, tys)];
+          if (es == e) return 0;
+        }
+      }
+    } else {
+      q -= 5 * Y.EL;
+      const int o = q / 5; pt = q - o * 5;
+      const signed char* fo = fix + Y.f_obs + ((c * Y.O + o) * N + i) * 5;
+      const int kk = (int)fo[pt];
+      if (kk < 0 || kk >= Y.L || (pt > 0 && code < 0)) return 0;
+      ed = D + Y.d_obs + ((o * N + i) * Y.L + kk) * 3;
+      if (pt > 0) {
+        int txs, tys;
+        if (corner_dominated(OBS_PT_D[pt][0], OBS_PT_D[pt][1], ed[0], ed[1], T[Y.i_dom + (c * Y.P + (code >> 2)) * 4 + (code & 3)], txs, tys)) {
+          if ((int)fo[obs_corner(txs, tys)] == kk) return 0;
+        }
+      }
+    }
+    if (pt != 0) return 2;
+    if (ed[1] == 0.0 && fabs(ed[0]) == 1.0) { col = 6 * c; sgn = ed[0]; rhs = ed[2]; return 1; }
+    if (ed[0] == 0.0 && fabs(ed[1]) == 1.0) { col = 6 * c + 3; sgn = ed[1]; rhs = ed[2]; return 1; }
+    return 2;
+  }
+  if (C < 2) return 0;
+  const int q = slot - C * Y.SC;
+  const bool excl = q >= Y.NP * 8;
+  int p, grp, which;
+  if (!excl) { p = q >> 3; grp = (q & 7) >> 1; which = q & 1; if ((int)fix[Y.f_c2c + (p * N + i) * 4 + grp] < 0) return 0; }
+  else {
+    const int q2 = q - Y.NP * 8; p = q2 >> 4; grp = (q2 >> 2) & 3; which = 1;
+    const int m = (int)fix[Y.f_c2n + (p * N + i) * 4 + grp];
+    if (m <= 0 || !((m >> (q2 & 3)) & 1)) return 0;
+  }
+  int c1, c2; pair_cars(p, C, c1, c2);
+  const bool need1 = grp >= 2, need2 = (grp == 1 || grp == 3);
+  if (need1 && (int)fix[Y.f_reg + c1 * N + i] < 0) { if (excl || Y.relax_front_off) return 0; if (!region_fpk(Y, D, T, fix, c1, i)) return 0; }
+  if (need2 && (int)fix[Y.f_reg + c2 * N + i] < 0) { if (excl || Y.relax_front_off) return 0; if (!region_fpk(Y, D, T, fix, c2, i)) return 0; }
+  if (!excl && which == 1) {
+    const bool soft = (grp == 0 || grp == 3);
+    if (!soft) return 0;
+    if (!(D[Y.d_smax + i] > 0 && D[Y.d_misc + 0] > 0)) return 0;
+  }
+  return 2;
+}
+
+__device__ inline void add_point_sp(double& g0, double& g1, double& g3, double& g4, double& rhs, const double* rt, int tx, int ty, double al, double be, const double* K = nullptr) {
+  g0 += al;
+  if (tx != PT_R) {
+    if (rt) { const double* p = rt + 19 + (tx == PT_U ? 0 : 3); rhs -= al * p[0]; g1 += al * p[1]; g4 += al * p[2]; }
+    else if (al != 0.0) rhs -= al * K[(tx == PT_U ? 0 : 2) + (al > 0.0 ? 0 : 1)];
+  }
+  g3 += be;
+  if (ty != PT_R) {
+    if (rt) { const double* p = rt + 25 + (ty == PT_U ? 0 : 3); rhs -= be * p[0]; g1 += be * p[1]; g4 += be * p[2]; }
+    else if (be != 0.0) rhs -= be * K[(ty == PT_U ? 4 : 6) + (be > 0.0 ? 0 : 1)];
+  }
+}
+
+template <int C>
+__device__ inline RowOut as_sparse_row(const Layout& Y, const double* D, const int* T, const signed char* fix, int i, int slot, double (&v)[8], int& car0, int& car1, bool& regpat) {
+  static_assert(C == 1 || C == 2, "the car of a slot is found by one comparison");
+  RowOut r; r.rhs = 0; r.aq = 0; r.active = true;
+#pragma unroll
+  for (int k = 0; k < 8; ++k) v[k] = 0.0;
+  const int N = Y.N;
+  car1 = 0; regpat = false;
+  if (slot < C * Y.SC) {
+    const int c = (C == 2 && slot >= Y.SC) ? 1 : 0, rr = slot - c * Y.SC;
+    const int code = (int)fix[Y.f_reg + c * N + i];
+    const double* rt = code >= 0 ? D + Y.d_reg + (c * Y.P + (code >> 2)) * REGSZ : nullptr;
+    car0 = c;
+    if (rr < 16) {
+      regpat = true;
+      const int k = rr - 11;
+      if (code < 0) { const double* Hc = D + Y.d_hull + (c * N + i) * HULLSZ; r.rhs = Hc[10 + 3 * k]; v[0] = Hc[8 + 3 * k]; v[2] = Hc[9 + 3 * k]; return r; }
+      switch (k) {
+        case 0: v[0] = rt[0]; v[2] = rt[1]; break;
+        case 1: v[0] = rt[2]; v[2] = rt[3]; break;
+        case 3: v[3] = 1; v[1] = -rt[4]; v[0] = -rt[6]; v[2] = -rt[7]; r.rhs = rt[5]; break;
+        default: v[3] = -1; v[1] = rt[4]; v[0] = rt[9]; v[2] = rt[10]; r.rhs = -rt[8]; break;
+      }
+      return r;
+    }
+    int q = rr - 16;
+    if (q < 5 * Y.EL) {
+      const int EL = Y.EL;
+      const int pt = (q >= EL ? 1 : 0) + (q >= 2 * EL ? 1 : 0) + (q >= 3 * EL ? 1 : 0) + (q >= 4 * EL ? 1 : 0), k = q - pt * EL;
+      const int e = Y.E == 1 ? 0 : (int)fix[Y.f_env + (c * N + i) * 5 + pt];
+      const double* ed = D + Y.d_env + (e * EL + k) * 3;
+      r.rhs = ed[2];
+      add_point_sp(v[0], v[1], v[2], v[3], r.rhs, rt, ENV_PT_D[pt][0], ENV_PT_D[pt][1], ed[0], ed[1]);
+      return r;
+    }
+    q -= 5 * Y.EL;
+    const int o = q / 5, pt = q - o * 5;
+    const int kk = (int)fix[Y.f_obs + ((c * Y.O + o) * N + i) * 5 + pt];
+    const double* ed = D + Y.d_obs + ((o * N + i) * Y.L + kk) * 3;
+    r.rhs = ed[2];
+    add_point_sp(v[0], v[1], v[2], v[3], r.rhs, rt, OBS_PT_D[pt][0], OBS_PT_D[pt][1], ed[0], ed[1]);
+    return r;
+  }
+  car0 = 0;
+  if constexpr (C == 2) {
+    const int q = slot - C * Y.SC;
+    const bool excl = q >= Y.NP * 8;
+    int p, grp, which, alt;
+    if (!excl) { p = q >> 3; grp = (q & 7) >> 1; which = q & 1; alt = (int)fix[Y.f_c2c + (p * N + i) * 4 + grp]; }
+    else { const int q2 = q - Y.NP * 8; p = q2 >> 4; grp = (q2 >> 2) & 3; alt = q2 & 3; which = 1; }
+    int c1, c2; pair_cars(p, C, c1, c2);
+    car0 = c1; car1 = c2;
+    const int code1 = (int)fix[Y.f_reg + c1 * N + i], code2 = (int)fix[Y.f_reg + c2 * N + i];
+    const bool need1 = grp >= 2, need2 = (grp == 1 || grp == 3);
+    const double* K1 = nullptr; const double* K2 = nullptr;
+    if (need1 && code1 < 0) K1 = region_fpk(Y, D, T, fix, c1, i);
+    if (need2 && code2 < 0) K2 = region_fpk(Y, D, T, fix, c2, i);
+    const double* rt1 = code1 >= 0 ? D + Y.d_reg + (c1 * Y.P + (code1 >> 2)) * REGSZ : nullptr;
+    const double* rt2 = code2 >= 0 ? D + Y.d_reg + (c2 * Y.P + (code2 >> 2)) * REGSZ : nullptr;
+    const double Dsep = D[Y.d_dsep + p * N + i], S = D[Y.d_ssl + i], smax = D[Y.d_smax + i], wsl = D[Y.d_misc + 0];
+    const bool soft = (grp == 0 || grp == 3);
+    const bool isx = alt < 2, lo = (alt == 0 || alt == 2);
+    int ca, cb, ta, tb;
+    if (grp == 0) { ta = tb = PT_R; ca = lo ? c1 : c2; cb = lo ? c2 : c1; }
+    else if (grp == 1) { if (lo) { ca = c1; ta = PT_R; cb = c2; tb = PT_L; } else { ca = c2; ta = PT_U; cb = c1; tb = PT_R; } }
+    else if (grp == 2) { if (lo) { ca = c2; ta = PT_R; cb = c1; tb = PT_L; } else { ca = c1; ta = PT_U; cb = c2; tb = PT_R; } }
+    else { if (lo) { ca = c2; ta = PT_U; cb = c1; tb = PT_L; } else { ca = c1; ta = PT_U; cb = c2; tb = PT_L; } }
+    const double al = isx ? 1.0 : 0.0, be = isx ? 0.0 : 1.0;
+    r.rhs = soft ? (which == 0 ? -(Dsep + S) + smax : -(Dsep + S)) : -Dsep;
+    r.aq = (!excl && soft && which == 1) ? 2.0 * wsl : 0.0;
+    double a0 = 0.0, a1 = 0.0, a3 = 0.0, a4 = 0.0, b0 = 0.0, b1 = 0.0, b3 = 0.0, b4 = 0.0;
+    add_point_sp(a0, a1, a3, a4, r.rhs, ca == c1 ? rt1 : rt2, ta, ta, al, be, ca == c1 ? K1 : K2);
+    add_point_sp(b0, b1, b3, b4, r.rhs, cb == c1 ? rt1 : rt2, tb, tb, -al, -be, cb == c1 ? K1 : K2);
+    const bool afirst = ca == c1;
+    v[0] = afirst ? a0 : b0; v[1] = afirst ? a1 : b1; v[2] = afirst ? a3 : b3; v[3] = afirst ? a4 : b4;
+    v[4] = afirst ? b0 : a0; v[5] = afirst ? b1 : a1; v[6] = afirst ? b3 : a3; v[7] = afirst ? b4 : a4;
+    if (excl) {
+#pragma unroll
+      for (int k = 0; k < 8; ++k) v[k] = -v[k];
+      r.rhs = -r.rhs;
+    }
+  }
+  return r;
+}
+
+}
diff --git a/planner_miqp_amd/csrc/solve_diag.hpp b/planner_miqp_amd/csrc/solve_diag.hpp
--- a/planner_miqp_amd/csrc/solve_diag.hpp
+++ b/planner_miqp_amd/csrc/solve_diag.hpp
@@ -137,12 +137,16 @@
     std::fprintf(stderr, "[miqp_gpu profile] on-chip nodes %llu iters %llu cycles/node-iter %.0f :", pf[11], pf[10], tot / std::max(1ull, pf[10]));
     for (int q = 0; q < 10; ++q) std::fprintf(stderr, " %s %.1f%% (%.0f)", nm[q], 100.0 * pf[q] / tot, (double)pf[q] / std::max(1ull, pf[10]));
     std::fprintf(stderr, "\n");
-    { unsigned long long pa[14]; HIP_OK(hipMemcpy(pa, B.prof + 80, 14 * 8, hipMemcpyDeviceToHost));
+    { unsigned long long pa[20]; HIP_OK(hipMemcpy(pa, B.prof + 80, 20 * 8, hipMemcpyDeviceToHost));
       const char* na[9] = {"decode", "gains + first iterate", "scan", "response of the row", "q", "directions + ratio test + M update", "iterate refresh", "results", "warm start"};
       double ta = 0; for (int q = 0; q < 9; ++q) ta += (double)pa[q];
       if (pa[10]) { std::fprintf(stderr, "[miqp_gpu profile] active-set kernel nodes %llu steps %llu cycles/node %.0f :", pa[10], pa[11], ta / (double)pa[10]);
         for (int q = 0; q < 9; ++q) std::fprintf(stderr, " %s %.1f%% (%.0f)", na[q], 100.0 * pa[q] / ta, (double)pa[q] / (double)pa[10]);
         std::fprintf(stderr, "; inside the decode: bound classes %.0f, general-row pass %.0f", (double)pa[12] / (double)pa[10], (double)pa[13] / (double)pa[10]);
+        {
+          const double n_ = (double)pa[10], sparse = (double)pa[0] - (double)pa[12] - (double)pa[13];
+          std::fprintf(stderr, "; sparse classes %.0f = enumeration %.0f + classification %.0f + prefix and candidate list %.0f; general-row pass = build %.0f + pack %.0f",
+                       sparse / n_, (sparse - (double)pa[17] - (double)pa[18]) / n_, (double)pa[17] / n_, (double)pa[18] / n_, (double)pa[19] / n_, ((double)pa[13] - (double)pa[19]) / n_); }
         std::fprintf(stderr, "\n");
         unsigned long long pw[3], pl[6]; HIP_OK(hipMemcpy(pw, B.prof + 94, 3 * 8, hipMemcpyDeviceToHost)); HIP_OK(hipMemcpy(pl, B.prof + 120, 6 * 8, hipMemcpyDeviceToHost));
         if (pw[2] && pw[1] && pl[5]) std::fprintf(stderr, "[miqp_gpu profile] standard active-set launches: %llu wavefronts resident %.0f shader cycles = %.1f us each (shader clock %.0f MHz); per launch (%llu folded): span %.3f ms, from the first wavefront out of work to the last end %.3f ms, wavefronts %.0f, resident wavefront time / (span x wavefronts) %.3f\n",
diff --git a/planner_miqp_amd/wrapper.py b/planner_miqp_amd/wrapper.py
--- a/planner_miqp_amd/wrapper.py
+++ b/planner_miqp_amd/wrapper.py
@@ -105,6 +105,9 @@
     L.miqp_solver_solve_fixed_multi.argtypes = [C.POINTER(vp), C.c_int, C.POINTER(C.POINTER(RawResultsC)), C.POINTER(C.c_int), C.POINTER(FixedResultC), C.POINTER(C.c_int)]
     L.miqp_solver_pool_solve_multi.restype = C.c_int
     L.miqp_solver_pool_solve_multi.argtypes = [C.POINTER(vp), C.c_int, C.POINTER(FixedResultC), C.c_int, C.POINTER(C.c_int)]
+    L.miqp_solver_decode_compare.restype = C.c_int
+    L.miqp_solver_decode_compare.argtypes = [vp, C.c_void_p, C.c_int, C.c_int, C.POINTER(C.c_int), C.POINTER(C.c_int), C.c_void_p]
+    L.miqp_gpu_decode_compare_words.restype = C.c_int; L.miqp_gpu_decode_compare_words.argtypes = []
     if L.miqp_gpu_fixed_result_size() != C.sizeof(FixedResultC):
         raise RuntimeError("libmiqp_gpu.so and ctypes_types.FixedResultC disagree on miqp_fixed_result_c (%d / %d bytes): rebuild the library"
                            % (L.miqp_gpu_fixed_result_size(), C.sizeof(FixedResultC)))
@@ -130,10 +133,16 @@
                     "miqp_solver_solve_fixed_batch", "miqp_solver_fixed_batch_record", "miqp_gpu_fixed_result_size", "miqp_gpu_fixed_batch_chunk",
                     "miqp_solver_set_pool", "miqp_solver_pool_count", "miqp_solver_pool_found", "miqp_solver_pool_solve", "miqp_solver_pool_record", "miqp_gpu_pool_max",
                     "miqp_solver_solve_fixed_multi", "miqp_solver_pool_solve_multi",
-                    "miqp_solver_set_pool_filter", "miqp_gpu_pool_signature", "miqp_solver_pool_signature", "miqp_solver_pool_found_decisions"]
+                    "miqp_solver_set_pool_filter", "miqp_gpu_pool_signature", "miqp_solver_pool_signature", "miqp_solver_pool_found_decisions",
+                    "miqp_solver_decode_compare", "miqp_gpu_decode_compare_words"]
 
 
 LAUNCH_PLAN_FIELDS = ("kernel", "stream", "grid", "lds", "ovf_mode", "cls_take", "as_split", "skip_probes", "bounce", "work", "from_ovf2", "bufs", "zero")
+
+
+DECODE_COMPARE_FIELDS = ("mismatch", "index", "ngen", "rows", "ncoef", "overflow", "box_keys", "cls0", "cls1", "cls2", "cls3", "cls4", "cls5", "cls6", "cls7", "cls2_box")
+DECODE_LAYOUT_FIELDS = ("fixlen", "f_reg", "f_env", "f_obs", "f_c2c", "f_c2n", "f_rmask", "C", "N", "E", "EL", "O", "L", "NP", "SC", "NSLOT")
+DECODE_MISMATCH = ("none", "overflow", "ngen", "box key", "rows packed", "ncoef", "gmeta", "grhs", "cand", "gcoef")
 
 
 _FIXED_RESULT_DTYPE = np.dtype([("status", "<i4"), ("route", "<i4"), ("iterations", "<i4"), ("reserved", "<i4"), ("objective", "<f8"), ("violation", "<f8")])
@@ -420,6 +429,32 @@
             raise RuntimeError("miqp_solver_launch_plan failed (%d)" % n)
         k = len(LAUNCH_PLAN_FIELDS)
         return [tuple(out[i * k:(i + 1) * k]) for i in range(n)]
+
+    def decodeLayout(self):
+        if self._push_inputs() != 0:
+            raise RuntimeError("invalid parameters")
+        lay = (C.c_int * 16)()
+        rc = self._L.miqp_solver_decode_compare(self._h, None, 0, 128, None, lay, None)
+        if rc < 0:
+            raise RuntimeError("miqp_solver_decode_compare refused the handle (%d)" % rc)
+        return dict(zip(DECODE_LAYOUT_FIELDS, list(lay)))
+
+    def decodeCompare(self, records=None, n=4096, gcap=128):
+        if self._push_inputs() != 0:
+            raise RuntimeError("invalid parameters")
+        fl = self.decodeLayout()["fixlen"]
+        w = int(self._L.miqp_gpu_decode_compare_words())
+        if records is not None:
+            records = np.ascontiguousarray(records, dtype=np.int8).reshape(-1, fl)
+            n = records.shape[0]
+        n = int(n)
+        out = np.zeros((max(n, 1), w), dtype=np.int32)
+        back = np.zeros((max(n, 1), fl), dtype=np.int8)
+        m = self._L.miqp_solver_decode_compare(self._h, records.ctypes.data if records is not None else None, n, int(gcap),
+                                               out.ctypes.data_as(C.POINTER(C.c_int)), None, back.ctypes.data)
+        if m < 0:
+            raise RuntimeError("miqp_solver_decode_compare failed (%d)" % m)
+        return out[:m], back[:m]
 
     def solveFixedBatch(self, records):
         if self._push_inputs() != 0:
```

Result: no change. 1085 (-0.6%).
